# apple/ml-stable-diffusion

Measured on AMD Instinct MI355X. Metric: diffusion iter/s (UNet steps/s), SD2.1-base 512x512 fp16, higher is better.
Workload: dtype fp16; 1 GPU; BASELINE config 2: SD2.1-base (865.9 M-parameter UNet), random-init, denoising iteration at 512x512 (64x64 latents), CFG batch 2 per prompt, DDIM, device-resident loop; unet=sd21-base, latent=64, attention=ORIGINAL, prompts_per_gpu=1, global_batch=2, hip_graph=True, parallelism=dp1 (independent prompts per rank, no data-path collective)

## Files before the change

include/sd_mi355x.h:

```cpp
#ifndef SD_MI355X_H
#define SD_MI355X_H

#include <stddef.h>
#include <stdint.h>

#ifdef __cplusplus
extern "C" {
#endif

typedef enum sd_status {
  SD_OK = 0,
  SD_ERR_INVALID_ARGUMENT = -1,
  SD_ERR_NOT_FOUND = -2,
  SD_ERR_HIP = -3,
  SD_ERR_UNSUPPORTED = -4,
  SD_ERR_INTERNAL = -5
} sd_status;

typedef enum sd_dtype { SD_F16 = 0, SD_F32 = 1 } sd_dtype;

typedef enum sd_attention_impl {
  SD_ATTN_ORIGINAL = 0,
  SD_ATTN_SPLIT_EINSUM = 1,
  SD_ATTN_SPLIT_EINSUM_V2 = 2
// ... 62 lines not shown
int sd_unet_set_attention(sd_unet* u, int impl);
int sd_unet_reload_weights(sd_unet* u, const sd_weights* w, const char* const* names, int n_names);
int sd_unet_num_residuals(const sd_unet* u);
size_t sd_unet_device_bytes(const sd_unet* u);
size_t sd_unet_arena_used_bytes(const sd_unet* u);
int sd_unet_palette_info(const sd_unet* u, int* n_palettized, int* n_streamed, size_t* stream_bytes);
int sd_unet_w8a8_info(const sd_unet* u, int* n_marked, int* n_applied, size_t* bytes);
int sd_unet_w8a8_layer(const sd_unet* u, int index, char* name, int name_bytes);
int sd_unet_activation_ranges(sd_unet* u, int index, char* name, int name_bytes, float* absmax);

#define SD_FLAG_DEVICE_PTRS 1

typedef struct sd_unet_io {
  const void* sample;
  const void* timestep;
  const void* encoder_hidden_states;
  const void* time_ids;
  const void* text_embeds;
  const void* controlnet_cond;
  const void* const* additional_residuals;
  int32_t num_additional_residuals;
  void* noise_pred;
  void* const* residual_outputs;
  int32_t flags;
  const float* step_noise;
} sd_unet_io;

int sd_unet_forward(sd_unet* u, const sd_unet_io* io);

int sd_unet_time_forward(sd_unet* u, int warmup, int iters, float* ms_per_iter);

int sd_unet_profile(sd_unet* u, int iters, int cap, float* ms, double* flop, char* labels, int label_bytes,
                    int* n_ops);

int sd_tune_set_candidate(int tile, int staging, int splitk);
int sd_tune_set_plan_table(const char* rows, sd_unet* u, int* n_plans);

int sd_unet_denoise_loop(sd_unet* u, const sd_unet_io* io, float* latents, int n_images, int n_steps,
                         const float* timesteps, const float* coef, const float* sample_scale, int history,
                         float guidance_scale, float* history_io, float* ms_per_step);

typedef int (*sd_progress_fn)(void* user, int step, int n_steps, const float* latents, const float* denoised);
int sd_unet_denoise_loop_progress(sd_unet* u, const sd_unet_io* io, float* latents, int n_images, int n_steps,
                                  const float* timesteps, const float* coef, const float* sample_scale, int history,
                                  float guidance_scale, float* history_io, float* ms_per_step,
                                  const float* pred , int every,
                                  sd_progress_fn fn, void* user, int* steps_done);

int sd_unet_attach_controlnets(sd_unet* u, sd_unet* const* controlnets, int n);
int sd_controlnet_set_cond(sd_unet* controlnet, const void* controlnet_cond, int flags);

int sd_vae_decoder_create(const sd_unet_config* cfg, const sd_weights* w, int device, sd_unet** out);
int sd_vae_decode(sd_unet* vae, const void* z, sd_dtype z_dtype, float* image, int flags);
int sd_vae_encoder_create(const sd_unet_config* cfg, const sd_weights* w, int device, sd_unet** out);
int sd_vae_encode(sd_unet* vae, const void* x, sd_dtype x_dtype, float* moments, int flags);
int sd_vae_encode_latents(sd_unet* vae_encoder, const void* x, sd_dtype x_dtype, const float* eps, const float* noise, int n_images,
                          float scale_factor, float sa, float sb, float* latents, int flags);
int sd_op_vae_attention(const void* q, const void* k, const void* v, void* out, int B, int S, int C, int iters, float* ms);

typedef struct sd_text_encoder_config {
  int32_t vocab_size, hidden_size, intermediate_size, num_hidden_layers, num_attention_heads;
  int32_t max_position_embeddings;
  int32_t hidden_act;
  int32_t projection_dim;
  float layer_norm_eps;
  int32_t use_graph;
} sd_text_encoder_config;
typedef struct sd_text_encoder sd_text_encoder;
int sd_text_encoder_create(const sd_text_encoder_config* cfg, const sd_weights* w, int device, sd_text_encoder** out);
void sd_text_encoder_destroy(sd_text_encoder* t);
size_t sd_text_encoder_device_bytes(const sd_text_encoder* t);
int sd_text_encoder_encode(sd_text_encoder* t, const int32_t* input_ids, int eos_index, float* last_hidden_state,
                           float* hidden_embeds, float* pooled);

int sd_op_attention(int impl, const void* q, const void* k, const void* v, void* out, int B, int heads, int d,
                    int Sq, int Sk, int variant, int iters, float* ms);
int sd_op_layernorm(const void* x, const float* weight, const float* bias, void* out, int B, int C, int S, float eps,
                    int iters, float* ms);
int sd_op_groupnorm(const void* x, const float* weight, const float* bias, void* out, int B, int C, int H, int W,
                    int groups, float eps, int silu, int iters, float* ms);
int sd_op_groupnorm_shortcut(const void* x0, const void* x1, const float* gn_weight, const float* gn_bias, const void* w, const float* bias,
                             void* out_gn, void* out_sc, int B, int C0, int C1, int H, int W, int N, int groups, float eps, int silu,
                             int side, int iters, float* ms);
int sd_op_conv2d(const void* x, const void* w, const float* bias, const void* res, void* out, int B, int Cin, int H,
                 int W, int Cout, int ksize, int stride, int upsample, int tile, int splitk, int force_generic,
                 int iters, float* ms);
int sd_op_conv2d_ex(const void* x, const void* x1, const void* w, const float* bias, const float* temb, const void* res, void* out, int B,
                    int Cin, int C1, int H, int W, int Cout, int ksize, int stride, int upsample, int pad_mode, int twin_groups,
                    const float* twin_gamma, const float* twin_beta, float twin_eps, int twin_silu, void* out_twin, int tile, int splitk,
                    int force_generic, int* plan_out, int iters, float* ms);
int sd_op_conv2d_palettized(const void* x, const void* x1, const void* lut, int nbits, const uint8_t* indices, const float* bias,
                            const void* res, void* out, int B, int Cin, int C1, int H, int W, int Cout, int ksize, int upsample, int nw,
                            int* plan_out, int iters, float* ms);
int sd_op_palette_pack(const uint8_t* indices, int Cout, int Ctot, int ksize, int nbits, uint8_t* stream, size_t* bytes);
int sd_op_conv2d_w8a8(const void* x, const void* x1, const int8_t* wq, const float* w_scale, float act_absmax, const float* bias,
                      const void* res, void* out, int B, int Cin, int C1, int H, int W, int Cout, int ksize, int upsample, int nw,
                      int* plan_out, int iters, float* ms);
int sd_op_w8a8_pack(const int8_t* wq, int Cout, int Ctot, int ksize, int8_t* stream, size_t* bytes);
int sd_op_conv2d_w8a8_halo(const void* x, const void* x1, const int8_t* wq, const float* w_scale, float act_absmax, const float* bias,
                           const float* temb, const void* res, void* out, int B, int Cin, int C1, int H, int W, int Cout, int upsample,
                           int staging, int splitk, int* plan_out, int iters, float* ms);
int sd_op_w8a8_pack_halo(const int8_t* wq, int Cout, int Ctot, int8_t* packed, size_t* bytes);
int sd_op_subpixel_fold(const void* w, int w_f32, int Cout, int Cin, void* folded, size_t* halves);
int sd_op_subpixel_refusal(int ksize, int stride, int up, int C0, int C1, int N, int B, int Hi, int Wi, int out_mode, char* text, int text_bytes);
int sd_op_conv2d_subpixel(const void* x, const void* w, const float* bias, const void* res, void* out, int B, int Cin, int H, int W, int Cout,
                          int splitk, int staging, int* plan_out, int iters, float* ms);
int sd_op_gemm_w8a8(const void* x, const int8_t* wq, const float* w_scale, float act_absmax, const float* bias, const void* res, void* out, int B,
                    int Cin, int H, int W, int Cout, int bm, int* plan_out, int iters, float* ms);
int sd_op_w8a8_pack_gemm(const int8_t* wq, int Cout, int K, int8_t* packed, size_t* bytes);
int sd_op_layernorm_q8(const void* x, const float* ln_weight, const float* ln_bias, float act_absmax, float eps, int8_t* xq, int M, int C,
                       int iters, float* ms);
int sd_op_geglu_w8a8(const int8_t* xq, const int8_t* wq, const float* w_scale, float act_absmax, const float* bias, void* out, int M, int C,
                     int N2, int bm, int* plan_out, int iters, float* ms);
int sd_op_w8a8_pack_geglu(const int8_t* wq, int N2, int K, int8_t* packed, size_t* bytes);
int sd_op_geglu_w8a8_q8(const int8_t* xq, const int8_t* wq, const float* w_scale, float act_absmax, const float* bias, float out_absmax,
                        int8_t* out_q, int M, int C, int N2, int bm, int* plan_out, int iters, float* ms);
int sd_op_gemm_q8(const int8_t* xq, const int8_t* wq, const float* w_scale, float act_absmax, const float* bias, const void* res, void* out,
                  int M, int K, int N, int bm, int* plan_out, int iters, float* ms);
int sd_op_qkv_w8a8(const int8_t* xq, const int8_t* wq, const float* w_scale, float act_absmax, const float* bias, void* out_qk, void* out_vt,
                   int B, int HW, int C, float q_scale, int vt_perm, int bm, int* plan_out, int iters, float* ms);
int sd_op_w8a8_pack_qkv(const int8_t* wq, int C, int8_t* packed, size_t* bytes);
int sd_op_quantize_weight(const float* w, int Cout, size_t per_row, int8_t* q, float* w_scale, double* sq_err);
int sd_op_absmax(const void* x, size_t n, float* absmax);
int sd_op_gemm_palettized(const void* x, const void* lut, int nbits, const uint8_t* indices, const float* bias, const void* res, void* out,
                          int B, int Cin, int H, int W, int Cout, int bm, int* plan_out, int iters, float* ms);
int sd_op_palette_pack_gemm(const uint8_t* indices, int Cout, int K, int nbits, uint8_t* stream, size_t* bytes);
int sd_op_geglu_palettized(const void* x, const float* ln_weight, const float* ln_bias, const void* lut, int nbits, const uint8_t* indices,
                           const float* bias, void* out, int M, int C, int N2, float eps, int bm, int* plan_out, int iters, float* ms);
int sd_op_palette_pack_geglu(const uint8_t* indices, int N2, int K, int nbits, uint8_t* stream, size_t* bytes);
int sd_op_conv2d_groupnorm(const void* x, const void* w, const float* bias, const void* res, const float* gn_weight,
                           const float* gn_bias, void* conv_out, void* out, int B, int Cin, int H, int W, int Cout, int ksize,
                           int groups, float eps, int silu, int tile, int producer_stats, int* entries, int iters, float* ms);
int sd_op_conv2d_groupnorm_proj(const void* x, const void* w, const float* bias, const void* res, const float* gn_weight,
                                const float* gn_bias, const void* proj_w, const float* proj_bias, void* conv_out, void* out, int B,
                                int Cin, int H, int W, int Cout, int ksize, int Nproj, int groups, float eps, int fold, int tile,
                                int* entries, int iters, float* ms);
int sd_op_conv2d_groupnorm_conv3x3(const void* x, const void* w, const float* bias, const void* res, const float* gn_weight,
                                   const float* gn_bias, const void* w2, const float* bias2, const void* res2, void* conv_out, void* out,
                                   int B, int Cin, int H, int W, int Cout, int ksize, int N2, int groups, float eps, int silu, int fold,
                                   int tile, int staging2, int* entries, int iters, float* ms);
int sd_op_ffn_out_proj(const void* g, const void* w1, const float* b1, const void* res1, const void* w2, const float* b2, const void* res2,
                       void* out, float* gn_sums, int B, int C, int S, int groups, int fused, int iters, float* ms);
int sd_op_fold_linear(const void* wp, const float* bp, const void* w2, const float* b2, void* wm_out, float* bm_out, int N, int J, int K);
int sd_op_cross_attention_fused(const void* x, const float* ln_weight, const float* ln_bias, const void* wq, const void* k,
                                const void* v, void* out, int B, int heads, int Sq, int Sk, float eps, int nst, int iters,
                                float* ms);
int sd_op_cross_attention_block(const void* x, const float* ln_weight, const float* ln_bias, const void* wq, const void* k, const void* v,
                                const void* wo, const float* bo, const void* a1, const void* wo1, const float* bo1, void* out, int B, int heads,
                                int Sq, int Sk, float eps, int fused, int iters, float* ms);
int sd_op_geglu(const void* x, const void* w, const float* bias, void* out, int M, int C, int N2, int iters, float* ms);
int sd_op_geglu_ln(const void* x, const float* ln_weight, const float* ln_bias, const void* w, const float* bias, void* out, int M, int C,
                   int N2, float eps, int kernel, int iters, float* ms);
int sd_op_qkv_ln(const void* x, const float* ln_weight, const float* ln_bias, const void* w, void* out_qk, void* out_vt, int B, int HW, int C,
                 float eps, float q_scale, int vt_perm, int kernel, int iters, float* ms);
int sd_op_gn_proj_qkv(const void* x_in, const void* conv_w, const float* gn_weight, const float* gn_bias, const void* proj_w,
                      const float* proj_bias, const float* ln_weight, const float* ln_bias, const void* wqkv, void* out_h, void* out_qk,
                      void* out_vt, int B, int H, int W, int C, int groups, float gn_eps, float ln_eps, float q_scale, int vt_perm, int fused,
                      int* entries, int iters, float* ms);
int sd_op_timestep_embedding(const float* t, float* out, int n, int dim, int flip_sin_to_cos, float freq_shift);
int sd_op_posterior_noise(const float* moments, const float* eps, const float* noise, float* out, int Cz, int h, int w, int n_images,
                          float scale_factor, float sa, float sb, int iters, float* ms);
int sd_op_sched_step(const float* noise_pred, float* latents, float* hist, const float* coef, const float* pred, const float* step_noise,
                     float guidance, int cfg, int history, int n_images, int n, float* denoised, int* step_after);
int sd_op_conv_plan(int ksize, int stride, int up, int C0, int C1, int N, int B, int Ho, int Wo, int out_mode, int flags, int n_trans,
                    int n_twins, int gnf_groups, int tile, int staging, int splitk, int copies, int* plan, unsigned long long* workspace_bytes);
int sd_op_conv_plan_kernel(int ksize, int stride, int up, int C0, int C1, int N, int B, int Ho, int Wo, int out_mode, int flags, int n_trans,
// ... 58 lines not shown
```

ml-stable-diffusion_amd/csrc/capi_ops.cpp:

```cpp
#include <algorithm>
#include <climits>
#include <cmath>
#include <cstring>
#include <initializer_list>

#include "capi_util.h"
#include "conv_plan.h"
#include "weight_prep.h"

namespace sd {
namespace {

const half_t* f16(const void* p) { return reinterpret_cast<const half_t*>(p); }

half_t* upload_nhwc(Scratch& sc, const void* x, int B, int C, int H, int W) {
  const half_t* src = f16(x);
  std::vector<half_t> t((size_t)B * C * H * W);
  for (int b = 0; b < B; ++b)
    for (int c = 0; c < C; ++c)
      for (int p = 0; p < H * W; ++p) t[((size_t)b * H * W + p) * C + c] = src[((size_t)b * C + c) * H * W + p];
  return sc.dev<half_t>(t.size(), t.data());
}
half_t* upload_tokens(Scratch& sc, const void* x, int B, int C, int S) { return upload_nhwc(sc, x, B, C, 1, S); }

// ... 326 lines not shown
      a.variant = 0;
      a.sk_force = 1;
      a.sk_upw = variant - 100;
    }
    {
      size_t pb = 0;
      int nc = 0;
      if (perm && attention8_sk_scratch(a, &pb, &nc)) {
        a.sk_part = reinterpret_cast<float*>(sc.out<char>(pb, "sk_part"));
        a.sk_part_bytes = pb;
        a.sk_cnt = sc.zeroed<unsigned>(nc, "sk_cnt");
        a.sk_cnt_n = nc;
      } else {
        SD_REQUIRE(variant < 100, kInvalidArgument, "attention variant %d: the balanced form cannot run this shape", variant);
      }
    }
    sc.timed(iters, ms, [&] { launch_attention(a, sc.stream); });
    download_tokens(o, out, B, C, Sq);
  });
}

int sd_op_layernorm(const void* x, const float* weight, const float* bias, void* out, int B, int C, int S, float eps,
                    int iters, float* ms) {
  return guarded([&] {
    SD_REQUIRE(x && weight && bias && out, kInvalidArgument, "NULL argument");
    Scratch sc("layernorm");
    half_t* dx = upload_tokens(sc, x, B, C, S);
    half_t* dy = sc.out<half_t>((size_t)B * S * C, "out");
    float* dw = sc.dev<float>(C, weight);
    float* db = sc.dev<float>(C, bias);
    sc.timed(iters, ms, [&] { launch_layernorm(dx, dw, db, dy, B * S, C, eps, sc.stream); });
    download_tokens(dy, out, B, C, S);
  });
}

int sd_op_groupnorm(const void* x, const float* weight, const float* bias, void* out, int B, int C, int H, int W,
                    int groups, float eps, int silu, int iters, float* ms) {
  return guarded([&] {
    SD_REQUIRE(x && weight && bias && out, kInvalidArgument, "NULL argument");
    Scratch sc("groupnorm");
    half_t* dx = upload_nhwc(sc, x, B, C, H, W);
    half_t* dy = sc.out<half_t>((size_t)B * H * W * C, "out");
    float* dw = sc.dev<float>(C, weight);
    float* db = sc.dev<float>(C, bias);
    float* partial = poisoned_gn_partial(sc, B, H * W, groups);
    sc.timed(iters, ms, [&] {
      launch_groupnorm(dx, C, nullptr, 0, partial, dw, db, dy, B, H * W, groups, eps, silu, sc.stream);
    });
    download_nchw(dy, out, B, C, H, W);
  });
}

int sd_op_groupnorm_shortcut(const void* x0, const void* x1, const float* gn_weight, const float* gn_bias, const void* w, const float* bias,
                             void* out_gn, void* out_sc, int B, int C0, int C1, int H, int W, int N, int groups, float eps, int silu,
                             int side, int iters, float* ms) {
  return guarded([&] {
    SD_REQUIRE(x0 && gn_weight && gn_bias && w && out_gn && out_sc, kInvalidArgument, "NULL argument");
    if (!x1) C1 = 0;
    const int C = C0 + C1;
    Scratch sc("groupnorm_shortcut");
    half_t* d0 = upload_nhwc(sc, x0, B, C0, H, W);
    half_t* d1 = x1 ? upload_nhwc(sc, x1, B, C1, H, W) : nullptr;
    half_t* dy = sc.out<half_t>((size_t)B * H * W * C, "out_gn");
    half_t* ds = sc.out<half_t>((size_t)B * H * W * N, "out_sc");
    float* dgw = sc.dev<float>(C, gn_weight);
    float* dgb = sc.dev<float>(C, gn_bias);
    float* partial = poisoned_gn_partial(sc, B, H * W, groups);
    ConvDesc d = conv_desc(d0, C0, sc.dev<half_t>((size_t)N * C, f16(w)), bias ? sc.dev<float>(N, bias) : nullptr, nullptr, ds, B, H, W, N);
    d.x1 = d1;
    d.C1 = C1;
    SD_REQUIRE(conv_fast_path_ok(d), kInvalidArgument, "groupnorm_shortcut: C0=%d C1=%d N=%d not MFMA-tileable", C0, C1, N);
    SD_REQUIRE(!side || gn_side_gemm_ok(d), kUnsupported, "groupnorm_shortcut: the GEMM cannot ride in the GroupNorm launch (M=%d)", B * H * W);
    ConvWorkspace ws = workspace_for(sc, {d});
    sc.timed(iters, ms, [&] {
      if (side) {
        launch_groupnorm(d0, C0, d1, C1, partial, dgw, dgb, dy, B, H * W, groups, eps, silu, sc.stream, 0, &d);
      } else {
        launch_groupnorm(d0, C0, d1, C1, partial, dgw, dgb, dy, B, H * W, groups, eps, silu, sc.stream);
        launch_conv(d, ws, sc.stream);
      }
    });
    download_nchw(dy, out_gn, B, C, H, W);
    download_nchw(ds, out_sc, B, N, H, W);
  });
}

int sd_op_conv2d(const void* x, const void* w, const float* bias, const void* res, void* out, int B, int Cin, int H,
                 int W, int Cout, int ksize, int stride, int upsample, int tile, int splitk, int force_generic,
                 int iters, float* ms) {
  return guarded([&] { conv2d_op(x, w, bias, res, out, B, Cin, H, W, Cout, ksize, stride, upsample, tile, splitk, force_generic, iters, ms, ConvOpExtra{}); });
}

int sd_op_conv2d_ex(const void* x, const void* x1, const void* w, const float* bias, const float* temb, const void* res, void* out, int B,
                    int Cin, int C1, int H, int W, int Cout, int ksize, int stride, int upsample, int pad_mode, int twin_groups,
                    const float* twin_gamma, const float* twin_beta, float twin_eps, int twin_silu, void* out_twin, int tile, int splitk,
                    int force_generic, int* plan_out, int iters, float* ms) {
  return guarded([&] {
    SD_REQUIRE(plan_out, kInvalidArgument, "NULL argument");
    ConvOpExtra e;
    e.entry = "conv2d_ex";
    e.x1 = x1; e.C1 = C1; e.temb = temb; e.pad_mode = pad_mode;
    e.twin_groups = twin_groups; e.twin_gamma = twin_gamma; e.twin_beta = twin_beta; e.twin_eps = twin_eps; e.twin_silu = twin_silu;
    e.out_twin = out_twin;
    e.plan_out = plan_out;
    conv2d_op(x, w, bias, res, out, B, Cin, H, W, Cout, ksize, stride, upsample, tile, splitk, force_generic, iters, ms, e);
  });
}

int sd_op_conv2d_palettized(const void* x, const void* x1, const void* lut, int nbits, const uint8_t* indices, const float* bias,
                            const void* res, void* out, int B, int Cin, int C1, int H, int W, int Cout, int ksize, int upsample, int nw,
                            int* plan_out, int iters, float* ms) {
  return guarded([&] {
    SD_REQUIRE(lut && indices, kInvalidArgument, "NULL argument");
    SD_REQUIRE(palette_bits_ok(nbits), kInvalidArgument, "conv2d_palettized: nbits = %d, not one of 1, 2, 4, 6, 8", nbits);
    SD_REQUIRE(nw == 0 || nw == 4 || nw == 8, kInvalidArgument, "conv2d_palettized: nw = %d, not 0, 4 or 8", nw);
    SD_REQUIRE(B > 0 && Cin > 0 && C1 >= 0 && Cout > 0 && H > 0 && W > 0, kInvalidArgument, "conv2d_palettized: empty problem");
    ConvOpExtra e;
    e.entry = "conv2d_palettized";
    e.x1 = x1; e.C1 = C1;
    e.plan_out = plan_out;
    e.cw.kind = WeightSource::PalWstream; e.cw.lut = lut; e.cw.indices = indices; e.cw.bits = nbits;
    e.nw = nw;
    conv2d_op(x, nullptr, bias, res, out, B, Cin, H, W, Cout, ksize, 1, upsample, 0, 0, 0, iters, ms, e);
  });
}

int sd_op_conv2d_w8a8(const void* x, const void* x1, const int8_t* wq, const float* w_scale, float act_absmax, const float* bias,
                      const void* res, void* out, int B, int Cin, int C1, int H, int W, int Cout, int ksize, int upsample, int nw,
                      int* plan_out, int iters, float* ms) {
  return guarded([&] {
    SD_REQUIRE(x && wq && w_scale && out, kInvalidArgument, "NULL argument");
    SD_REQUIRE(nw == 0 || nw == 4 || nw == 8, kInvalidArgument, "conv2d_w8a8: nw = %d, not 0, 4 or 8", nw);
    SD_REQUIRE(B > 0 && Cin > 0 && C1 >= 0 && Cout > 0 && H > 0 && W > 0 && (C1 == 0 || x1), kInvalidArgument, "conv2d_w8a8: empty problem");
    SD_REQUIRE((ksize == 1 || ksize == 3) && (upsample == 0 || upsample == 1), kInvalidArgument, "conv2d_w8a8: ksize %d upsample %d", ksize, upsample);
    ConvDesc d;
    d.C0 = Cin;
    if (C1 > 0) d.x1 = f16(x1), d.C1 = C1;
    d.B = B; d.Hi = H; d.Wi = W; d.Ho = H * (upsample ? 2 : 1); d.Wo = W * (upsample ? 2 : 1);
    d.ksize = ksize; d.up = upsample ? 2 : 1; d.N = Cout;
    SD_REQUIRE(conv_fast_path_ok(d) && wstream_shape_ok(d), kInvalidArgument,
               "conv2d_w8a8: shape not eligible for plan tile 17 (wstream.hip: k=%d C0=%d C1=%d N=%d %dx%d)", ksize, Cin, C1, Cout, d.Ho, d.Wo);
    (void)w8a8_host_copy("conv2d_w8a8", wq, w_scale, act_absmax, Cout, Cin + C1, ksize);
    ConvOpExtra e;
    e.entry = "conv2d_w8a8";
    e.x1 = x1; e.C1 = C1;
    e.plan_out = plan_out;
    e.cw.kind = WeightSource::I8Wstream; e.cw.q = wq; e.cw.w_scale = w_scale; e.cw.act_absmax = act_absmax;
    e.nw = nw;
    conv2d_op(x, nullptr, bias, res, out, B, Cin, H, W, Cout, ksize, 1, upsample, 0, 0, 0, iters, ms, e);
  });
}

int sd_op_conv2d_w8a8_halo(const void* x, const void* x1, const int8_t* wq, const float* w_scale, float act_absmax, const float* bias, const float* temb,
                           const void* res, void* out, int B, int Cin, int C1, int H, int W, int Cout, int upsample, int staging, int splitk, int* plan_out,
                           int iters, float* ms) {
  return guarded([&] {
    SD_REQUIRE(x && wq && w_scale && out, kInvalidArgument, "NULL argument");
    SD_REQUIRE(B > 0 && Cin > 0 && C1 >= 0 && Cout > 0 && H > 0 && W > 0 && (C1 == 0 || x1), kInvalidArgument, "conv2d_w8a8_halo: empty problem");
    SD_REQUIRE((upsample == 0 || upsample == 1) && staging >= 0 && staging <= 5 && staging != 1 && splitk >= 0, kInvalidArgument,
               "conv2d_w8a8_halo: upsample %d staging %d (plan tile 7's ring codes 0, 2-5) splitk %d", upsample, staging, splitk);
    ConvDesc d;
    d.C0 = Cin;
    if (C1 > 0) d.x1 = f16(x1), d.C1 = C1;
    d.B = B; d.Hi = H; d.Wi = W; d.Ho = H * (upsample ? 2 : 1); d.Wo = W * (upsample ? 2 : 1);
    d.ksize = 3; d.up = upsample ? 2 : 1; d.N = Cout;
    SD_REQUIRE(conv_fast_path_ok(d) && halo_ks_ok(d), kInvalidArgument,
// ... 1506 lines not shown
```

ml-stable-diffusion_amd/csrc/conv_plan.cpp:

```cpp
#include "conv_plan.h"

#include <algorithm>
#include <cstring>

namespace sd {

namespace {

constexpr int BK = kConvBK;

struct Dims {
  int Ctot, M, N, K, HoWo, nk_total, tiles_x, tiles_y;
};
Dims dims_of(const ConvDesc& d) {
  Dims a;
  a.Ctot = d.C0 + (d.x1 ? d.C1 : 0);
  a.M = d.B * d.Ho * d.Wo;
  a.N = d.N;
  a.K = d.ksize * d.ksize * a.Ctot;
  a.HoWo = d.Ho * d.Wo;
  a.nk_total = a.K / BK;
  a.tiles_x = cdiv(d.Wo, 16);
  a.tiles_y = cdiv(d.Ho, 8);
  return a;
// ... 317 lines not shown
    r.workspace_bytes = slab_bytes(a, r.splitk, r.slab);
    return r;
  }
  if (!conv_fast_path_ok(d)) return ConvPlan{-1, 0, 1, false, 0};
  switch (cw.kind) {
    case WeightSource::Fp16: break;
    case WeightSource::PalWstream:
    case WeightSource::I8Wstream: {
      const bool i8 = i8_stream(d);
      SD_REQUIRE(cw.stream && (i8 ? cw.scale != nullptr : cw.lut != nullptr) && can_split(d) && wstream_shape_ok(d), kInvalidArgument, "%s",
                 i8 ? "plan tile 17 (wstream.hip, int8) needs the int8 stream, the scales and a shape of the weight stream"
                    : "plan tile 14 (wstream.hip, palettized) needs the index stream, the LUT and a shape of the weight stream");
      ConvPlan r{i8 ? 17 : 14, d.staging, 1, true, 0};
      r.splitk = wstream_splits(d, wstream_waves(d.staging));
      r.workspace_bytes = slab_bytes(dims_of(d), r.splitk, true);
      return r;
    }
    case WeightSource::I8Halo: {
      const Dims a = dims_of(d);
      const Plan p = choose_plan(d, a);
      ConvPlan r{18, p.staging, 1, true, 0};
      const int steps = a.Ctot / BK;
      r.splitk = cdiv(steps, cdiv(steps, p.splitk));
      r.slab = r.splitk > 1 || d.n_twins > 0;
      r.workspace_bytes = slab_bytes(a, r.splitk, r.slab);
      return r;
    }
    case WeightSource::PalGemm:
      SD_REQUIRE(cw.stream && cw.lut && palette_bits_ok(cw.bits) && !d.x1 && d.staging >= 0 && d.staging <= 2 && smgemm_shape_ok(d, d.staging), kInvalidArgument,
                 "plan tile 15 (smgemm.hip, palettized) needs the index stream, the LUT and a single-source shape of the small-M GEMM");
      return ConvPlan{15, smgemm_bm(d, d.staging) == 32 ? 1 : 2, 1, false, 0};
    case WeightSource::I8Gemm:
      return ConvPlan{19, smgemm_bm(d, d.staging) == 32 ? 1 : 2, 1, false, 0};
    case WeightSource::PalGeglu:
      SD_REQUIRE(cw.stream && cw.lut && palette_bits_ok(cw.bits) && (cw.ln_gamma != nullptr) == (d.ln_colsum != nullptr) && smgeglu_pal_shape_ok(d, d.staging),
                 kInvalidArgument,
                 "plan tile 16 (smgeglu.hip, palettized) needs the index stream, the LUT, the norm weight with the LayerNorm fold and a shape of "
                 "the GEGLU kernel with 128-row tiles");
      return ConvPlan{16, 1, 1, false, 0};
    case WeightSource::I8Geglu:
      return ConvPlan{20, smgeglu_bm(d, d.staging) == 128 ? 1 : 2, 1, false, 0};
    case WeightSource::I8Qkv:
      return ConvPlan{22, smqkv_i8_bm(d, d.staging) == 128 ? 1 : 2, 1, false, 0};
    case WeightSource::I8GemmQ:
      return ConvPlan{24, smgemm_bm(d, d.staging) == 32 ? 1 : 2, 1, false, 0};
  }
  const Switches& sw = switches();
  const bool free_choice = d.tile == 0 && d.splitk == 0 && d.staging == 0 && g_tune.tile == 0;
  if (d.w_ws && wsgemm_shape_ok(d) && (d.tile == 10 || (sw.wsgemm && free_choice && wsgemm_wanted(d)))) return ConvPlan{10, 0, 1, false, 0};
  SD_REQUIRE(d.tile != 10, kInvalidArgument, "plan tile 10 (wsgemm.hip) needs the pre-tiled weights and an eligible GEGLU shape");
  if (sw.bvgemm && d.w_bv && free_choice && bvgemm_wanted(d)) return ConvPlan{11, 0, 1, false, 0};
  if (d.tile == 11) {
    SD_REQUIRE(d.w_bv && bvgemm_shape_ok(d), kInvalidArgument, "plan tile 11 (bvgemm.hip) needs the pre-tiled weights and an eligible 1x1 shape");
    return ConvPlan{11, d.staging, 1, false, 0};
  }
  if (d.tile == 12 || (sw.smgemm && free_choice && smgemm_wanted(d))) return ConvPlan{12, d.tile == 12 ? d.staging : 0, 1, false, 0};
  if (d.tile == 13 || (sw.smgeglu && free_choice && smgeglu_wanted(d))) return ConvPlan{13, d.tile == 13 ? d.staging : 0, 1, false, 0};

  const Dims a = dims_of(d);
  Plan p = choose_plan(d, a);
  const bool twins = d.n_twins > 0;
  if (d.gnf_partial && d.ksize == 3) {
    SD_REQUIRE(conv_gn_loader_ok(d) && d.gnf_silu == 1 && d.gnf_gamma && d.gnf_beta && d.gnf_entries >= 1 && d.gnf_entries <= 128 && !twins, kInvalidArgument,
               "GroupNorm in the conv loader: Ctot=%d groups=%d entries=%d up=%d", a.Ctot, d.gnf_groups, d.gnf_entries, d.up);
    p.tile = 7;
    if (p.staging != 2 && p.staging != 3) p.staging = 3;
    p.splitk = 1;
  } else if (d.gnf_partial) {
    SD_REQUIRE(d.ksize == 1 && d.stride == 1 && !d.x1 && d.out_mode == kOutHalf && !d.ln_colsum && !d.out_t && !twins &&
                   gemm_pipe_ok(d.ksize, d.stride, d.up, a.M, a.N, a.K, d.C0, 0) &&
                   d.gnf_gamma && d.gnf_beta && d.gnf_groups >= 1 && d.gnf_groups <= 32 && a.K % d.gnf_groups == 0 && a.K <= 2048 &&
                   d.gnf_entries >= 1 && d.gnf_entries <= 128 && a.HoWo % 64 == 0,
               kInvalidArgument, "GroupNorm fold: K=%d groups=%d entries=%d HoWo=%d", a.K, d.gnf_groups, d.gnf_entries, a.HoWo);
    p.tile = 3;
    if (p.staging != 6 && p.staging != 7 && p.staging != 8) p.staging = 6;
    p.splitk = 1;
  }
  ConvPlan r{p.tile, p.staging, 1, true, 0};
  if (p.tile == 9) {
    r.splitk = wstream_splits(d, wstream_waves(p.staging));
  } else {
    const int steps = p.tile == 7 ? a.Ctot / BK : a.nk_total;
    r.splitk = cdiv(steps, cdiv(steps, p.splitk));
    r.slab = r.splitk > 1 || twins;
  }
  r.workspace_bytes = slab_bytes(a, r.splitk, r.slab);
  return r;
}

void decode_plan(const ConvDesc& d, ConvPlan& p) {
  const Dims a = dims_of(d);
  int code = p.staging;
  switch (p.tile) {
    case -1: p.kernel = ConvKernel::Generic; return;
    case 9: case 14: case 17:
      p.kernel = p.tile == 9 ? ConvKernel::Wstream : p.tile == 14 ? ConvKernel::WstreamPal : ConvKernel::WstreamI8;
      p.waves = wstream_waves(code);
      return;
    case 10: p.kernel = ConvKernel::Wsgemm; return;
    case 11:
      p.kernel = ConvKernel::Bvgemm;
      p.variant = code >= 1 && code <= 6 ? code : bvgemm_auto_variant(d);
      return;
    case 12: case 15: case 19: case 24:
      p.kernel = p.tile == 12 ? ConvKernel::Smgemm : p.tile == 15 ? ConvKernel::SmgemmPal : p.tile == 19 ? ConvKernel::SmgemmI8 : ConvKernel::SmgemmQ8;
      p.bm = code >= 0 && code <= 2 ? smgemm_bm(d, code) : 0;
      return;
    case 13: case 16: case 20:
      p.kernel = p.tile == 13 ? ConvKernel::Smgeglu : p.tile == 16 ? ConvKernel::SmgegluPal : ConvKernel::SmgegluI8;
      p.bm = code >= 0 && code <= 2 ? smgeglu_bm(d, code) : 0;
      return;
    case 22:
      p.kernel = ConvKernel::SmqkvI8;
      p.bm = code >= 0 && code <= 2 ? smqkv_i8_bm(d, code) : 0;
      return;
    default: break;
  }
  if (p.tile == 18) {
    tile_dims(7, p.bm, p.bn);
    p.kernel = ConvKernel::HaloI8;
    p.stages = code >= 3 ? 4 : code == 2 ? 3 : 2;
    return;
  }
  if (p.tile == 21) {
    tile_dims(7, p.bm, p.bn);
    p.kernel = ConvKernel::HaloSubpix;
    p.stages = code == 2 ? 3 : 4;
    return;
  }
  tile_dims(p.tile, p.bm, p.bn);
  if (p.tile == 7) {
    p.kernel = ConvKernel::HaloKs;
    if (d.gnf_partial) p.stages = code >= 3 && halo_gnl_lds_bytes(4, a.Ctot) <= kLdsBudget ? 4 : 3;
    else p.stages = code >= 5 ? 8 : code == 4 ? 6 : code == 3 ? 4 : code == 2 ? 3 : 2;
    return;
  }
  p.kernel = ConvKernel::Igemm;
  p.stages = 2;
  const bool lnf = d.ln_colsum != nullptr;
  auto fits = [&](int nst, int kgroups = 1) { return ring_fits(p.bm, p.bn, nst, kgroups); };
  if (lnf && code == 1) code = 0;
  if (code == 1) {
    p.reg_staged = true;
    return;
  }
  if (!lnf && d.out_mode == kOutHalfT) {
    if (code >= 2) p.stages = 3;
    return;
  }
  if (code == 12 || code == 13) {
    const bool two_groups = !lnf && cdiv(a.nk_total, p.splitk) >= 4;
    if (two_groups && code == 13 && fits(4, 2)) p.stages = 4, p.kgroups = 2;
    else if (two_groups && fits(3, 2)) p.stages = 3, p.kgroups = 2;
    if (p.kgroups == 2) return;
    code -= 10;
  }
  if (code >= 6 && code <= 8 && gemm_pipe_ok(d.ksize, d.stride, d.up, a.M, a.N, a.K, d.C0, d.x1 ? d.C1 : 0)) {
    p.kernel = ConvKernel::GemmPipe;
    p.stages = code == 8 ? 2 : (code == 7 && fits(4)) ? 4 : 3;
    return;
  }
  if (code >= 6) code = 3;
  const int asked = code >= 5 ? 8 : code == 4 ? 6 : code == 3 ? 4 : code == 2 ? 3 : 2;
  for (int nst : {8, 6, 4, 3, 2})
    if (nst <= asked && fits(nst)) {
      p.stages = nst;
      return;
    }
}

}

ConvPlan conv_plan(const ConvDesc& d) {
  ConvPlan p = plan_codes(d);
  decode_plan(d, p);
  return p;
}

std::string conv_plan_kernel_name(const ConvPlan& p) {
  const std::string tile = std::to_string(p.bm) + "x" + std::to_string(p.bn), ring = " ring" + std::to_string(p.stages);
  switch (p.kernel) {
    case ConvKernel::Igemm: return "igemm " + tile + ring + (p.kgroups == 2 ? " kg2" : "") + (p.reg_staged ? " regs" : "");
    case ConvKernel::GemmPipe: return "gemm_pipe " + tile + ring;
    case ConvKernel::HaloKs: return "halo_ks" + ring;
    case ConvKernel::HaloI8: return "halo_i8" + ring;
    case ConvKernel::HaloSubpix: return "conv3x3_halo_sp" + ring;
    case ConvKernel::Wstream: return "wstream waves" + std::to_string(p.waves);
    case ConvKernel::WstreamPal: return "wstream_pal waves" + std::to_string(p.waves);
    case ConvKernel::WstreamI8: return "wstream_i8 waves" + std::to_string(p.waves);
    case ConvKernel::Wsgemm: return "wsgemm";
    case ConvKernel::Bvgemm: return "bvgemm v" + std::to_string(p.variant);
    case ConvKernel::Smgemm: return "smgemm bm" + std::to_string(p.bm);
    case ConvKernel::SmgemmPal: return "smgemm_pal bm" + std::to_string(p.bm);
    case ConvKernel::SmgemmI8: return "smgemm_i8 bm" + std::to_string(p.bm);
    case ConvKernel::SmgemmQ8: return "smgemm_q8 bm" + std::to_string(p.bm);
    case ConvKernel::Smgeglu: return "smgeglu bm" + std::to_string(p.bm);
    case ConvKernel::SmgegluPal: return "smgeglu_pal bm" + std::to_string(p.bm);
    case ConvKernel::SmgegluI8: return "smgeglu_i8 bm" + std::to_string(p.bm);
    case ConvKernel::SmqkvI8: return "smqkv_i8 bm" + std::to_string(p.bm);
    default: return "generic";
  }
}

size_t conv_workspace_bytes(const ConvDesc& d) {
  if (!conv_fast_path_ok(d) || pal_gemm(d) || pal_geglu(d) || i8_gemm(d) || i8_geglu(d) || i8_qkv(d) || i8_gemm_q(d)) return 0;
  const Dims a = dims_of(d);
  if (d.subpix) return halo_sp_ok(d) ? slab_bytes(a, subpix_splits(d, a), false) : 0;
  const Plan p = choose_plan(d, a);
  int splits = (switches().tuning && can_split(d)) ? std::max(p.splitk, 16) : p.splitk;
  const bool stream = can_stream(d) || ((pal_stream(d) || i8_stream(d)) && can_split(d) && wstream_shape_ok(d));
  if (stream) splits = std::max(splits, wstream_splits(d, 4));
  return slab_bytes(a, splits, d.n_twins > 0 || stream);
}

ConvWeightCopies conv_plan_copies(const ConvDesc& d0) {
  ConvWeightCopies c{false, false, false};
  if (!conv_fast_path_ok(d0) || d0.subpix) return c;
  ConvDesc d = d0;
  d.w_tiled = d.w_ws = d.w_bv = nullptr;
  const Switches& sw = switches();
  const int k = d.ksize, M = d.B * d.Ho * d.Wo;
  const bool ws_candidate = sw.tuning ? ((k == 3 && M <= 512) || (k == 1 && M <= 128)) : plan_is_wstream(d);
  c.wstream = sw.wstream && wstream_shape_ok(d) && ws_candidate;
  c.wsgemm = sw.wsgemm && wsgemm_wanted(d);
  c.bvgemm = sw.bvgemm && !c.wsgemm && bvgemm_wanted(d);
  return c;
}

namespace {
ConvPlan fp16_plan(const ConvDesc& d0, const ConvWeightCopies& c) {
  static const half_t present = 0;
  ConvDesc d = d0;
  d.cw = CompressedWeights{};
  d.w_tiled = c.wstream ? &present : nullptr;
  d.w_ws = c.wsgemm ? &present : nullptr;
  d.w_bv = c.bvgemm ? &present : nullptr;
  return conv_plan(d);
}
}

WeightPin conv_plan_pin(WeightSource kind, int n) {
  switch (kind) {
    case WeightSource::PalWstream: return {kind, 14, n == 4 ? 4 : 0};
    case WeightSource::I8Wstream: return {kind, 17, n == 4 ? 4 : 0};
    case WeightSource::I8Halo: return {kind, 18, n};
    case WeightSource::PalGemm: return {kind, 15, n == 32 ? 1 : n == 64 ? 2 : 0};
    case WeightSource::I8Gemm: return {kind, 19, n == 32 ? 1 : n == 64 ? 2 : 0};
    case WeightSource::PalGeglu: return {kind, 16, n == 128 ? 1 : n == 256 ? 2 : 0};
    case WeightSource::I8Geglu: return {kind, 20, n == 128 ? 1 : n == 256 ? 2 : 0};
    case WeightSource::I8Qkv: return {kind, 22, n == 128 ? 1 : n == 256 ? 2 : 0};
    case WeightSource::I8GemmQ: return {kind, 24, n == 32 ? 1 : n == 64 ? 2 : 0};
    default: return {};
  }
}

WeightPin conv_plan_weights(const ConvDesc& d, StoredWeights held, bool opt_in) {
  if (held == StoredWeights::Fp16 || !conv_fast_path_ok(d)) return {};
  const Switches& sw = switches();
  const bool palette = held == StoredWeights::Palette, one_by_one = opt_in && palette && d.ksize == 1 && !d.x1;
  if (one_by_one && d.out_mode == kOutGeglu && sw.smgeglu) {
    const ConvPlan p = fp16_plan(d, conv_plan_copies(d));
    if (p.kernel == ConvKernel::Smgeglu && smgeglu_pal_shape_ok(d, 0)) return conv_plan_pin(WeightSource::PalGeglu, p.bm);
  }
  if (opt_in && held == StoredWeights::W8A8 && d.ksize == 1 && !d.x1 && d.out_mode == kOutGeglu && sw.smgeglu) {
    const ConvPlan p = fp16_plan(d, conv_plan_copies(d));
    ConvDesc plain = d;
    plain.ln_colsum = nullptr;
    if (p.kernel == ConvKernel::Smgeglu && smgeglu_i8_shape_ok(plain, p.bm == 128 ? 1 : 2)) return conv_plan_pin(WeightSource::I8Geglu, p.bm);
  }
  if (opt_in && held == StoredWeights::W8A8 && d.ksize == 1 && !d.x1 && d.out_mode == kOutHalf && d.n_trans == 0 && d.x0_i8) {
    if (sw.smgemm && !d.ln_colsum && smgemm_q8_wanted(d)) return conv_plan_pin(WeightSource::I8GemmQ, smgemm_bm(d, 0));
    return {};
  }
  if (opt_in && held == StoredWeights::W8A8 && d.ksize == 1 && !d.x1 && d.out_mode == kOutHalf && d.n_trans > 0 && sw.qkv_i8) {
    ConvDesc plain = d;
    plain.ln_colsum = nullptr;
    if (smqkv_i8_shape_ok(plain, 0)) return conv_plan_pin(WeightSource::I8Qkv, smqkv_i8_bm(plain, 0));
    return {};
  }
  if (sw.wstream && !d.ln_colsum && plan_is_wstream(d)) {
    const ConvPlan p = fp16_plan(d, {true, false, false});
    if (p.kernel == ConvKernel::Wstream) return conv_plan_pin(palette ? WeightSource::PalWstream : WeightSource::I8Wstream, p.waves);
  }
  if (one_by_one && d.out_mode == kOutHalf && sw.smgemm && !d.ln_colsum) {
    const ConvPlan p = fp16_plan(d, conv_plan_copies(d));
    if (p.kernel == ConvKernel::Smgemm) return conv_plan_pin(WeightSource::PalGemm, p.bm);
  }
  if (opt_in && held == StoredWeights::W8A8 && d.ksize == 1 && !d.x1 && d.out_mode == kOutHalf && sw.smgemm && !d.ln_colsum) {
    const ConvPlan p = fp16_plan(d, conv_plan_copies(d));
    if (p.kernel == ConvKernel::Smgemm && smgemm_i8_shape_ok(d, 0)) return conv_plan_pin(WeightSource::I8Gemm, p.bm);
  }
  if (held == StoredWeights::W8A8 && halo_i8_ok(d)) {
    const ConvPlan p = fp16_plan(d, conv_plan_copies(d));
    if (p.kernel == ConvKernel::HaloKs) {
      WeightPin pin = conv_plan_pin(WeightSource::I8Halo, p.staging);
// ... 79 lines not shown
```

ml-stable-diffusion_amd/csrc/conv_plan.h:

```cpp
#pragma once
#include <string>

#include "kernels.h"

namespace sd {

enum class ConvKernel { Generic, Igemm, GemmPipe, HaloKs, HaloI8, HaloSubpix, Wstream, WstreamPal, WstreamI8, Wsgemm, Bvgemm, Smgemm, SmgemmPal, SmgemmI8, Smgeglu, SmgegluPal, SmgegluI8, SmqkvI8, SmgemmQ8 };

struct ConvPlan {
  int tile;
  int staging;
  int splitk;
  bool slab;
  size_t workspace_bytes;
  ConvKernel kernel = ConvKernel::Generic;
  int bm = 0, bn = 0;
  int stages = 0;
  int kgroups = 1;
  bool reg_staged = false;
  int waves = 0;
  int variant = 0;
};
ConvPlan conv_plan(const ConvDesc& d);

struct ConvWeightCopies {
  bool wstream, wsgemm, bvgemm;
};
ConvWeightCopies conv_plan_copies(const ConvDesc& d);

enum class StoredWeights { Fp16, Palette, W8A8 };
struct WeightPin {
  WeightSource kind = WeightSource::Fp16;
  int tile = 0, staging = 0;
  int splitk = 0;
};
WeightPin conv_plan_weights(const ConvDesc& d, StoredWeights held, bool opt_in);
WeightPin conv_plan_pin(WeightSource kind, int n);

void conv_plan_log(const ConvDesc& d, const ConvPlan& p, int n_fast = 0);

std::string conv_plan_kernel_name(const ConvPlan& p);

bool choose_tile_order(double a_bytes, double w_bytes, double nbm, double nbn, bool ab_switch);

bool conv_reduce_stats_on();

constexpr int kConvBK = 64;
bool halo_ks_ok(const ConvDesc& d);
const char* halo_sp_refusal(const ConvDesc& d);
inline bool halo_sp_ok(const ConvDesc& d) { return halo_sp_refusal(d) == nullptr; }
bool subpixel_wanted(const ConvDesc& d);
bool gemm_pipe_ok(int ksize, int stride, int up, int M, int N, int K, int C0, int C1);

constexpr size_t kLdsBudget = 160 * 1024;
constexpr size_t ring_bytes(int bm, int bn, int nst) { return (size_t)nst * (bm + bn) * kConvBK * sizeof(half_t); }
constexpr bool ring_fits(int bm, int bn, int nst, int kgroups = 1) { return kgroups * ring_bytes(bm, bn, nst) + 2 * bn * sizeof(float) <= kLdsBudget; }
constexpr int kHaloLdsRows = 184;
constexpr size_t halo_lds_bytes(int bn, int d) {
  return ((size_t)2 * kHaloLdsRows * kConvBK + (size_t)d * bn * kConvBK) * sizeof(half_t) + bn * sizeof(float);
}
constexpr size_t halo_gnl_lds_bytes(int d, int ctot) {
  const size_t k_loop = halo_lds_bytes(64, d) - 64 * sizeof(float) + (((size_t)6 * ctot + 15) & ~(size_t)15);
  const size_t epilogue = 32 * 1024 + 128 * (64 + 8) * 2 + 64 * sizeof(float);
  return k_loop > epilogue ? k_loop : epilogue;
}
constexpr int kHaloI8Pitch = 20, kHaloI8Rows = 204;
constexpr size_t halo_i8_lds_bytes(int d) {
  return (size_t)kHaloLdsRows * kConvBK * sizeof(half_t) + (size_t)2 * kHaloI8Rows * kConvBK + (size_t)d * 64 * kConvBK + 2 * 64 * sizeof(float);
}
constexpr int kHaloI8MaxCtot = 14784;
static_assert(127LL * 127 * 9 * kHaloI8MaxCtot < (1LL << 31) && 127LL * 127 * 9 * (kHaloI8MaxCtot + 64) >= (1LL << 31), "int32 bound of plan tile 18");
constexpr int kSmI8MaxK = 133120;
static_assert(127LL * 127 * kSmI8MaxK < (1LL << 31) && 127LL * 127 * (kSmI8MaxK + 64) >= (1LL << 31), "int32 bound of plan tile 19");

bool smgemm_q8_wanted(const ConvDesc& d);
constexpr int kSmQkvCols = 160;
bool smqkv_i8_shape_ok(const ConvDesc& d, int variant);
bool smqkv_i8_tiles(const ConvDesc& d, int variant);
int smqkv_i8_bm(const ConvDesc& d, int variant);

}
```

ml-stable-diffusion_amd/csrc/igemm.hip:

```cpp
#include "igemm_device.h"

namespace sd {

namespace {

template <int BM, int BN, int WGM, int WGN, bool TRANS_OUT, bool GLDS, int NST, int DBG = 0, bool LNF = false, int KG = 1>
__global__ __launch_bounds__(256 * KG) void igemm_kernel(IgemmArgs a) {
  static_assert(WGM * WGN == 4, "4 waves");
  static_assert(KG == 1 || (KG == 2 && GLDS && NST >= 3 && !LNF && !TRANS_OUT && DBG == 0), "in-workgroup split-K: ring variants of the plain epilogue");
  static_assert(!(LNF && TRANS_OUT), "LayerNorm fold uses the in-lane row layout of the non-transposed tile");
  constexpr int TM = BM / WGM / 32;
  constexpr int TN = BN / WGN / 32;
  constexpr int XR = BM / 32;
  constexpr int WR = BN / 32;
  constexpr int ROW = GLDS ? BK : LDS_ROW;

  const bool prof = (DBG & 4) && blockIdx.x == 0 && blockIdx.y == 0 && threadIdx.x == 0;
  long long prof_t[4];
  long long prof_w0 = 0;
  if (prof) { prof_t[0] = clock64(); prof_w0 = wall_clock64(); }
  extern __shared__ __attribute__((aligned(16))) char smem[];
  const int kg = KG > 1 ? __builtin_amdgcn_readfirstlane((int)threadIdx.x >> 8) : 0;
  half_t* Xs = reinterpret_cast<half_t*>(smem) + (size_t)kg * NST * (BM + BN) * ROW;
  half_t* Ws = Xs + NST * BM * ROW;
// ... 618 lines not shown
  int rd_stage = 0;
  auto body = [&](Frags& cur, Frags& nxt, auto last) {
    constexpr bool LAST = decltype(last)::value;
    if constexpr (LAST) {
      asm volatile("s_waitcnt lgkmcnt(0)" ::: "memory");
      mfma_step(cur);
    } else {
      asm volatile("s_waitcnt lgkmcnt(0)" ::: "memory");
      wait_vmcnt_barrier<(D - 2) * PER>();
      const int nstage = (rd_stage + 1 == D) ? 0 : rd_stage + 1;
      read_step(nxt, nstage);
      issue_tile();
      mfma_step(cur);
      rd_stage = nstage;
      if constexpr (!LNF && !GNF) {
        constexpr int NM = KK * TM * TN, NR = KK * (TM + TN);
        constexpr int RPM = (NR + NM / 2 - 1) / (NM / 2);
#pragma unroll
        for (int g = 0; g < NM / 2; ++g) {
          __builtin_amdgcn_sched_group_barrier(0x008, 1, 0);
          __builtin_amdgcn_sched_group_barrier(0x100, RPM, 0);
        }
#pragma unroll
        for (int g = 0; g < NM - NM / 2; ++g) {
          __builtin_amdgcn_sched_group_barrier(0x008, 1, 0);
          __builtin_amdgcn_sched_group_barrier(0x010, (PER + NM - NM / 2 - 1) / (NM - NM / 2), 0);
        }
      }
    }
    __builtin_amdgcn_sched_barrier(0);
  };
  {
    using Tt = std::true_type;
    using Ff = std::false_type;
    int st = 0;
    for (; st + 2 < T; st += 2) {
      body(fA, fB, Ff{});
      body(fB, fA, Ff{});
    }
    if (T - st == 2) {
      body(fA, fB, Ff{});
      body(fB, fA, Tt{});
    } else {
      body(fA, fB, Tt{});
    }
  }
  asm volatile("s_waitcnt vmcnt(0) lgkmcnt(0)" ::: "memory");

  float ln_a[TM] = {}, ln_b[TM] = {};
  if constexpr (LNF) {
    const float inv_k = 1.0f / (float)a.K;
#pragma unroll
    for (int i = 0; i < TM; ++i) {
      const float s1 = xor32_sum(ln_s1[i]), s2 = xor32_sum(ln_s2[i]);
      const float mean = s1 * inv_k;
      const float var = fmaxf(s2 * inv_k - mean * mean, 0.f);
      ln_a[i] = rsqrtf(var + a.ln_eps);
      ln_b[i] = -ln_a[i] * mean;
    }
  }
  tile_epilogue<BM, BN, WGM, WGN, TM, TN, LNF, (RES_PRE ? RIT : 0)>(a, acc, ln_a, ln_b, smem, sconst, const_b, const_t, const_c, m_blk,
                                                                    n_blk, wave, split, temb_uniform, resv, use_resv);
}

template <int BM, int BN, int WGM, int WGN, int D, bool LNF, int DBG = 0, bool GNF = false>
__global__ __launch_bounds__(256, D == 2 ? 2 : 1) void gemm_pipe_kernel(IgemmArgs a) {
  gemm_pipe_body<BM, BN, WGM, WGN, D, LNF, DBG, GNF>(a, blockIdx.x, blockIdx.y);
}

struct GnSideArgs {
  const half_t* x0;
  const half_t* x1;
  int C0, C1;
  const float* partial;
  int slabs;
  const float* gamma;
  const float* beta;
  half_t* y;
  int HW, G;
  float eps;
  int silu, pix_per_block;
  int gx, gy;
  int n_gn_pad;
};

template <int D>
__global__ __launch_bounds__(256) void gn_apply_side_kernel(GnSideArgs g, IgemmArgs a) {
  const int v = blockIdx.x;
  if (v < g.gx * g.gy) {
    groupnorm_apply_body(g.x0, g.C0, g.x1, g.C1, g.partial, g.slabs, g.gamma, g.beta, g.y, g.HW, g.G, g.eps, g.silu, g.pix_per_block,
                         v % g.gx, v / g.gx);
  } else if (v >= g.n_gn_pad) {
    gemm_pipe_body<64, 64, 2, 2, D, false>(a, v - g.n_gn_pad, 0);
  }
}

template <int VW, int D>
__global__ __launch_bounds__(256) void gn_fused_side_kernel(GnSideArgs g, IgemmArgs a) {
  const int v = blockIdx.x;
  if (v < g.gx * g.gy) {
    groupnorm_fused_body<VW, 256>(g.x0, g.C0, g.x1, g.C1, g.gamma, g.beta, g.y, g.HW, g.G, g.eps, g.silu, v % g.gx, v / g.gx);
  } else if (v >= g.n_gn_pad) {
    gemm_pipe_body<64, 64, 2, 2, D, false>(a, v - g.n_gn_pad, 0);
  }
}

__global__ __launch_bounds__(256) void splitk_reduce_kernel(IgemmArgs a) {
  constexpr int SB = 8;
  const size_t total4 = (size_t)a.M * a.N / 4;
  const size_t slab = (size_t)a.M * a.N;
  const floatx4 z4 = {0.f, 0.f, 0.f, 0.f};
  for (size_t idx = (size_t)blockIdx.x * blockDim.x + threadIdx.x; idx < total4;
       idx += (size_t)gridDim.x * blockDim.x) {
    const size_t e0 = idx * 4;
    const int m = (int)(e0 / a.N);
    const int n = (int)(e0 - (size_t)m * a.N);
    floatx4 p[SB];
#pragma unroll
    for (int z = 0; z < SB; ++z) p[z] = (z < a.splitk) ? *reinterpret_cast<const floatx4*>(a.partial + (size_t)z * slab + e0) : z4;
    const floatx4 bv = a.bias ? *reinterpret_cast<const floatx4*>(a.bias + n) : z4;
    const floatx4 tv = a.temb ? *reinterpret_cast<const floatx4*>(a.temb + (size_t)(m / a.HoWo) * a.temb_stride + n) : z4;
    const half4 hz = {0, 0, 0, 0};
    const half4 rr = a.res ? *reinterpret_cast<const half4*>(a.res + e0) : hz;
    floatx4 s = z4;
#pragma unroll
    for (int z = 0; z < SB; ++z)
      if (z < a.splitk) s += p[z];
    for (int z = SB; z < a.splitk; ++z) s += *reinterpret_cast<const floatx4*>(a.partial + (size_t)z * slab + e0);
    if (a.bias) s += bv;
    if (a.temb) s += tv;
    if (a.res) {
      s[0] += (float)rr[0];
      s[1] += (float)rr[1];
      s[2] += (float)rr[2];
      s[3] += (float)rr[3];
    }
    half4 o = {(half_t)s[0], (half_t)s[1], (half_t)s[2], (half_t)s[3]};
    out_store(reinterpret_cast<half4*>(a.out + e0), o);
  }
}

__global__ __launch_bounds__(256) void splitk_reduce_stats_kernel(IgemmArgs a, int ppb) {
  extern __shared__ __attribute__((aligned(16))) char smem[];
  float* qs = reinterpret_cast<float*>(smem);
  const int NQ = a.N >> 2, t = threadIdx.x, b = blockIdx.y;
  const int p0 = blockIdx.x * ppb;
  const int items = ppb * NQ;
  for (int id = t; id < items; id += 256) {
    const int pl = id / NQ, qd = id - pl * NQ;
    const int p = p0 + pl;
    float fs = 0.f, fq = 0.f;
    if (p < a.HoWo) {
      const int m = b * a.HoWo + p, n = 4 * qd;
      const size_t e0 = (size_t)m * a.N + n;
      floatx4 s = {0.f, 0.f, 0.f, 0.f};
      for (int z = 0; z < a.splitk; ++z) s += *reinterpret_cast<const floatx4*>(a.partial + (size_t)z * a.M * a.N + e0);
      if (a.bias) s += *reinterpret_cast<const floatx4*>(a.bias + n);
      if (a.temb) s += *reinterpret_cast<const floatx4*>(a.temb + (size_t)b * a.temb_stride + n);
      if (a.res) {
        const half4 rr = *reinterpret_cast<const half4*>(a.res + e0);
        s[0] += (float)rr[0];
        s[1] += (float)rr[1];
        s[2] += (float)rr[2];
        s[3] += (float)rr[3];
      }
      const half4 o = {(half_t)s[0], (half_t)s[1], (half_t)s[2], (half_t)s[3]};
      out_store(reinterpret_cast<half4*>(a.out + e0), o);
      const float f0 = (float)o[0], f1 = (float)o[1], f2 = (float)o[2], f3 = (float)o[3];
      fs = (f0 + f1) + (f2 + f3);
      fq = fmaf(f0, f0, fmaf(f1, f1, fmaf(f2, f2, f3 * f3)));
    }
    qs[2 * id] = fs;
    qs[2 * id + 1] = fq;
  }
  __syncthreads();
  if (t < a.gn_G) {
    const int q0 = t * (a.gn_cpg >> 2), q1 = q0 + (a.gn_cpg >> 2);
    float s = 0.f, q = 0.f;
    for (int pl = 0; pl < ppb; ++pl)
      for (int qd = q0; qd < q1; ++qd) {
        s += qs[2 * (pl * NQ + qd)];
        q += qs[2 * (pl * NQ + qd) + 1];
      }
    float* dst = a.gn_partial + (((size_t)b * a.gn_G + t) * kGnMaxSlabs + blockIdx.x) * 2;
    dst[0] = s;
    dst[1] = q;
  }
}


template <int BM, int BN, int WGM, int WGN, bool TRANS, bool GLDS, int NST, bool LNF = false, int KG = 1>
void launch_variant(const IgemmArgs& a, hipStream_t s) {
  const size_t lds = (size_t)KG * NST * (BM + BN) * (GLDS ? BK : LDS_ROW) * sizeof(half_t) + 2 * BN * sizeof(float);
  static_assert(ring_fits(BM, BN, NST, KG), "LDS");
  static_assert((size_t)BN * (BM + 8) <= (size_t)NST * (BM + BN) * (GLDS ? BK : LDS_ROW), "transposed staging fits");
  static_assert((size_t)BM * (BN + 8) * 2 + 16 + (kGnScratchFloats + 2 * BN) * sizeof(float) <=
                    (size_t)NST * (BM + BN) * (GLDS ? BK : LDS_ROW) * sizeof(half_t),
                "GroupNorm statistics scratch fits behind the staged tile");
  dim3 grid(cdiv(a.M, BM) * cdiv(a.N, BN), a.splitk);
  auto k = igemm_kernel<BM, BN, WGM, WGN, TRANS, GLDS, NST, 0, LNF, KG>;
  static DynLdsOnce once;
  once.set(k, lds);
  hipLaunchKernelGGL(k, grid, dim3(256 * KG), lds, s, a);
}

template <int BM, int BN, int DBG>
void launch_debug(const IgemmArgs& a, hipStream_t s) {
  const size_t lds = (size_t)2 * (BM + BN) * BK * sizeof(half_t) + 2 * BN * sizeof(float);
  dim3 grid(cdiv(a.M, BM) * cdiv(a.N, BN), a.splitk);
  auto k = igemm_kernel<BM, BN, 2, 2, false, true, 2, DBG>;
  SD_HIP(hipFuncSetAttribute((const void*)k, hipFuncAttributeMaxDynamicSharedMemorySize, (int)lds));
  hipLaunchKernelGGL(k, grid, dim3(256), lds, s, a);
}
template <int BM, int BN>
bool launch_debug_mode(const IgemmArgs& a, int dbg, hipStream_t s) {
  switch (dbg) {
    case 4: launch_debug<BM, BN, 4>(a, s); return true;
    case 5: launch_debug<BM, BN, 5>(a, s); return true;
    case 6: launch_debug<BM, BN, 6>(a, s); return true;
    case 14: launch_debug<BM, BN, 14>(a, s); return true;
    case 22: launch_debug<BM, BN, 22>(a, s); return true;
    case 30: launch_debug<BM, BN, 30>(a, s); return true;
    default: return false;
  }
}

template <int BM, int BN, int WGM, int WGN, int D, bool LNF>
void launch_pipe_dbg(const IgemmArgs& a, hipStream_t s) {
  constexpr size_t lds = (size_t)D * (BM + BN) * BK * sizeof(half_t) + 2 * BN * sizeof(float);
  dim3 grid(cdiv(a.M, BM) * cdiv(a.N, BN), a.splitk);
  if (a.debug == 65) {
    auto k = gemm_pipe_kernel<BM, BN, WGM, WGN, D, LNF, 1>;
    SD_HIP(hipFuncSetAttribute((const void*)k, hipFuncAttributeMaxDynamicSharedMemorySize, (int)lds));
    hipLaunchKernelGGL(k, grid, dim3(256), lds, s, a);
  } else {
    auto k = gemm_pipe_kernel<BM, BN, WGM, WGN, D, LNF, 2>;
    SD_HIP(hipFuncSetAttribute((const void*)k, hipFuncAttributeMaxDynamicSharedMemorySize, (int)lds));
    hipLaunchKernelGGL(k, grid, dim3(256), lds, s, a);
  }
// ... 37 lines not shown
      if constexpr (!LNF && (NST == 3 || NST == 4) && ring_fits(BM, BN, NST, 2)) { launch_variant<BM, BN, 2, 2, false, true, NST, false, 2>(a, s); return true; }
    } else {
      launch_variant<BM, BN, 2, 2, false, true, NST, LNF>(a, s);
      return true;
    }
  }
  return false;
}
template <int BM, int BN, bool LNF>
bool launch_ring(const IgemmArgs& a, const ConvPlan& p, hipStream_t s) {
  switch (p.stages) {
    case 2: return launch_ring_depth<BM, BN, LNF, 2>(a, p, s);
    case 3: return launch_ring_depth<BM, BN, LNF, 3>(a, p, s);
    case 4: return launch_ring_depth<BM, BN, LNF, 4>(a, p, s);
    case 6: return launch_ring_depth<BM, BN, LNF, 6>(a, p, s);
    case 8: return launch_ring_depth<BM, BN, LNF, 8>(a, p, s);
    default: return false;
  }
}

template <int BM, int BN>
void launch_tile(const IgemmArgs& a, const ConvPlan& p, bool trans, hipStream_t s) {
  bool ok = true;
  if (a.ln_colsum) ok = !p.reg_staged && launch_ring<BM, BN, true>(a, p, s);
  else if (trans && p.reg_staged) launch_variant<BM, BN, 2, 2, true, false, 2>(a, s);
  else if (trans && p.stages == 3) launch_variant<BM, BN, 2, 2, true, true, 3>(a, s);
  else if (trans) launch_variant<BM, BN, 2, 2, true, true, 2>(a, s);
  else if (p.reg_staged) launch_variant<BM, BN, 2, 2, false, false, 2>(a, s);
  else ok = launch_ring<BM, BN, false>(a, p, s);
  SD_REQUIRE(ok, kInternal, "no %dx%d kernel for plan '%s'", BM, BN, conv_plan_kernel_name(p).c_str());
}

int launch_slab_combine(const ConvDesc& d, IgemmArgs& a, hipStream_t s) {
  a.gn_partial = nullptr;
  if (conv_reduce_stats_on() && d.gn_partial && d.gn_groups >= 1 && d.gn_groups <= 256 && a.N % d.gn_groups == 0 && (a.N / d.gn_groups) % 4 == 0 &&
      a.HoWo <= 256 && d.out_mode == kOutHalf && !d.out_t) {
    int ppb = std::max(1, a.B * a.HoWo / 512);
    const int slabs = cdiv(a.HoWo, ppb);
    const size_t lds = (size_t)ppb * (a.N / 4) * 2 * sizeof(float);
    if (slabs <= kGnMaxSlabs && lds <= 64 * 1024) {
      a.gn_partial = d.gn_partial;
      a.gn_G = d.gn_groups;
      a.gn_cpg = a.N / d.gn_groups;
      a.gn_T = slabs;
      hipLaunchKernelGGL(splitk_reduce_stats_kernel, dim3(slabs, a.B), dim3(256), lds, s, a, ppb);
      return slabs;
    }
  }
  const size_t total4 = (size_t)a.M * a.N / 4;
  const int blocks = (int)std::min<size_t>((total4 + 255) / 256, 2048);
  hipLaunchKernelGGL(splitk_reduce_kernel, dim3(blocks), dim3(256), 0, s, a);
  return 0;
}

half_t* g_zero_chunk = nullptr;

}

const half_t* device_zero_chunk() {
  if (!g_zero_chunk) {
    SD_HIP(hipMalloc(reinterpret_cast<void**>(&g_zero_chunk), 256));
    SD_HIP(hipMemset(g_zero_chunk, 0, 256));
    SD_HIP(hipDeviceSynchronize());
  }
  return g_zero_chunk;
}

const half_t* zero_chunk() {
  SD_REQUIRE(g_zero_chunk, kInternal, "conv launch before any handle allocated the zero chunk (device_zero_chunk)");
  return g_zero_chunk;
}

int launch_conv(const ConvDesc& d, const ConvWorkspace& ws, hipStream_t s) {
  SD_REQUIRE(conv_fast_path_ok(d), kInvalidArgument, "launch_conv: shape not MFMA-tileable (C0=%d C1=%d N=%d k=%d)",
             d.C0, d.C1, d.N, d.ksize);
  SD_REQUIRE(!d.ln_colsum || (d.ksize == 1 && !d.x1 && d.bias && d.out_mode != kOutHalfT), kInvalidArgument,
             "LayerNorm fold needs a 1x1 single-source GEMM with a (folded) bias");
  SD_REQUIRE(!d.out_t || (d.out_mode == kOutHalf && d.n_trans % 64 == 0 && d.n_trans < d.N && (d.Ho * d.Wo) % 8 == 0 &&
                          d.ldT % 8 == 0 && !d.res && !d.temb),
             kInvalidArgument, "fused q|k|v: n_trans %d N %d HoWo %d ldT %d", d.n_trans, d.N, d.Ho * d.Wo, d.ldT);
  SD_REQUIRE(!d.vt_perm || (d.out_t && (d.Ho * d.Wo) % 16 == 0), kInvalidArgument, "permuted V^T needs the fused q|k|v epilogue and HoWo %% 16 == 0");
  SD_REQUIRE(d.q_cols == 0 || (d.out_t && d.q_cols % 4 == 0 && d.q_cols <= d.n_trans), kInvalidArgument, "pre-scaled queries need the fused q|k|v epilogue (q_cols %d)", d.q_cols);
  const ConvPlan p = conv_plan(d);
  switch (p.kernel) {
    case ConvKernel::Wsgemm: launch_wsgemm(d, s); return 0;
    case ConvKernel::Bvgemm: launch_bvgemm(d, p, s); return 0;
    case ConvKernel::Smgemm: launch_smgemm(d, p, s); return 0;
    case ConvKernel::Smgeglu: launch_smgeglu(d, p, s); return 0;
    case ConvKernel::SmgegluPal: launch_smgeglu_pal(d, p, s); return 0;
    case ConvKernel::SmgemmPal: launch_smgemm_pal(d, p, s); return 0;
    case ConvKernel::SmgemmI8: launch_smgemm_i8(d, p, s); return 0;
    case ConvKernel::SmgegluI8: launch_smgeglu_i8(d, p, s); return 0;
    case ConvKernel::SmgemmQ8: launch_smgemm_q8(d, p, s); return 0;
    case ConvKernel::SmqkvI8: launch_smqkv_i8(d, p, s); return 0;
    default: break;
  }
  IgemmArgs a = planned_args(d, p, ws.partial);
  const bool twins = d.n_twins > 0;
  SD_REQUIRE(!twins || (d.out_mode == kOutHalf && !d.ln_colsum && !d.out_t && !d.debug && reduce_twin_ok(a.HoWo, a.N, d.n_twins, d.twin)),
             kInvalidArgument, "GroupNorm twins need a plain fp16 output and whole (sample, group) slices (HoWo=%d N=%d)", a.HoWo, a.N);
  const bool have_ws = !p.slab || (ws.partial && ws.partial_bytes >= p.workspace_bytes);
  if (p.kernel == ConvKernel::Wstream || p.kernel == ConvKernel::WstreamPal || p.kernel == ConvKernel::WstreamI8) SD_REQUIRE(have_ws, kInternal, "wstream workspace too small (%zu < %zu)", ws.partial_bytes, p.workspace_bytes);
  SD_REQUIRE(have_ws, kInternal, "split-K workspace too small (%zu < %zu)", ws.partial_bytes, p.workspace_bytes);
  conv_plan_log(d, p);
  int gn_entries = 0;
  switch (p.kernel) {
    case ConvKernel::Wstream:
      launch_wstream(d, ws.partial, p.waves, s);
      break;
    case ConvKernel::WstreamPal:
      launch_wstream_pal(d, ws.partial, p.waves, s);
      break;
    case ConvKernel::WstreamI8:
      launch_wstream_i8(d, ws.partial, p.waves, s);
      break;
    case ConvKernel::HaloKs: gn_entries = launch_halo_ks(d, p, ws.partial, s); break;
    case ConvKernel::HaloI8: gn_entries = launch_halo_i8(d, p, ws.partial, s); break;
    case ConvKernel::HaloSubpix: gn_entries = launch_halo_sp(d, p, ws.partial, s); break;
    case ConvKernel::Igemm:
    case ConvKernel::GemmPipe: {
      const bool trans = d.out_mode == kOutHalfT;
      set_tile_order(a, p.bm, p.bn);
      if (d.debug && d.debug < 64) {
        const bool ok = p.bm == 128 && p.bn == 128 ? launch_debug_mode<128, 128>(a, d.debug, s) : launch_debug_mode<64, 64>(a, d.debug, s);
        SD_REQUIRE(ok && !trans, kInvalidArgument, "no ablation kernel for debug mode %d", d.debug);
        return 0;
      }
      if (!trans) gn_entries = setup_gn_stats(d, a, p.bm);
      if (p.bm == 128 && p.bn == 128) launch_tile<128, 128>(a, p, trans, s);
      else if (p.bm == 128) launch_tile<128, 64>(a, p, trans, s);
      else if (p.bn == 64) launch_tile<64, 64>(a, p, trans, s);
      else launch_tile<64, 128>(a, p, trans, s);
      break;
    }
    default: SD_REQUIRE(false, kInternal, "launch_conv: plan '%s' has no launcher here", conv_plan_kernel_name(p).c_str());
  }
  if (twins) {
    launch_reduce_twin(a.partial, a.splitk, a.M, a.N, a.HoWo, a.bias, a.temb, a.temb_stride, a.res, a.out, d.n_twins, d.twin, s);
  } else if (a.slab) {
    gn_entries = launch_slab_combine(d, a, s);
  }
  SD_HIP(hipGetLastError());
  return gn_entries;
}

bool gn_side_gemm_ok(const ConvDesc& d) {
  if (!(d.ksize == 1 && d.stride == 1 && d.up == 1 && d.out_mode == kOutHalf && !d.ln_colsum && !d.out_t && d.n_twins == 0 && !d.gnf_partial &&
        !d.gn_partial && !d.temb && !d.debug && conv_fast_path_ok(d)))
    return false;
  const int M = d.B * d.Ho * d.Wo, c1 = d.x1 ? d.C1 : 0;
  return gemm_pipe_ok(d.ksize, d.stride, d.up, M, d.N, d.C0 + c1, d.C0, c1) && M >= 256;
}

namespace {
constexpr int kSideD = 4;
IgemmArgs side_args(const ConvDesc& d) {
  SD_REQUIRE(gn_side_gemm_ok(d), kInvalidArgument, "side GEMM: not a plain 1x1 GEMM of the pipelined kernel (C0=%d C1=%d N=%d)", d.C0, d.C1, d.N);
  IgemmArgs a = make_args(d);
  a.splitk = 1;
  a.slab = 0;
  set_tile_order(a, 64, 64);
  return a;
}
constexpr size_t kSideLds = (size_t)kSideD * (64 + 64) * BK * sizeof(half_t) + 2 * 64 * sizeof(float);
}

void launch_gn_apply_side(const half_t* x0, int C0, const half_t* x1, int C1, const float* partial, int entries, const float* gamma,
                          const float* beta, half_t* y, int B, int HW, int G, float eps, int silu, int slabs, int ppb, const ConvDesc& side,
                          hipStream_t s) {
  IgemmArgs a = side_args(side);
  GnSideArgs g{x0, x1, C0, x1 ? C1 : 0, partial, entries, gamma, beta, y, HW, G, eps, silu, ppb, slabs, B, 0};
  g.n_gn_pad = (slabs * B + 7) / 8 * 8;
  auto k = gn_apply_side_kernel<kSideD>;
  static DynLdsOnce once;
  once.set(k, kSideLds);
  hipLaunchKernelGGL(k, dim3(g.n_gn_pad + cdiv(a.M, 64) * cdiv(a.N, 64)), dim3(256), kSideLds, s, g, a);
  SD_HIP(hipGetLastError());
}

void launch_gn_fused_side(int vw, const half_t* x0, int C0, const half_t* x1, int C1, const float* gamma, const float* beta, half_t* y, int B,
                          int HW, int G, float eps, int silu, const ConvDesc& side, hipStream_t s) {
  IgemmArgs a = side_args(side);
  GnSideArgs g{x0, x1, C0, x1 ? C1 : 0, nullptr, 0, gamma, beta, y, HW, G, eps, silu, 0, G, B, 0};
  g.n_gn_pad = (G * B + 7) / 8 * 8;
  const dim3 grid(g.n_gn_pad + cdiv(a.M, 64) * cdiv(a.N, 64));
  static DynLdsOnce o8, o4, o2;
  if (vw == 8) {
    auto k = gn_fused_side_kernel<8, kSideD>;
    o8.set(k, kSideLds);
    hipLaunchKernelGGL(k, grid, dim3(256), kSideLds, s, g, a);
  } else if (vw == 4) {
    auto k = gn_fused_side_kernel<4, kSideD>;
    o4.set(k, kSideLds);
    hipLaunchKernelGGL(k, grid, dim3(256), kSideLds, s, g, a);
  } else {
    auto k = gn_fused_side_kernel<2, kSideD>;
    o2.set(k, kSideLds);
    hipLaunchKernelGGL(k, grid, dim3(256), kSideLds, s, g, a);
  }
  SD_HIP(hipGetLastError());
}

}
```

ml-stable-diffusion_amd/csrc/igemm_device.h:

```cpp
#pragma once
#include <cstdio>
#include <cstdlib>
#include <cstring>
#include <string>
#include <type_traits>

#include "conv_plan.h"

namespace sd {

const half_t* zero_chunk();

int launch_halo_ks(const ConvDesc& d, const ConvPlan& p, float* partial, hipStream_t s);
int launch_halo_i8(const ConvDesc& d, const ConvPlan& p, float* partial, hipStream_t s);
int launch_halo_sp(const ConvDesc& d, const ConvPlan& p, float* partial, hipStream_t s);

namespace {

constexpr int BK = kConvBK;
constexpr int LDS_ROW = BK + 8;

struct IgemmArgs {
  const half_t* x0;
  const half_t* x1;
  const half_t* w;
  const float* bias;
  const float* temb;
  const half_t* res;
  half_t* out;
  float* partial;
  int C0, C1, Ctot;
  int B, Hi, Wi, Ho, Wo, HoWo;
  int ksize, stride, up, pad;
  int M, N, K;
  int temb_stride;
  int nk_total, nk_per_split, splitk;
  int slab;
  int out_mode, ldT;
  int debug;
  long long* prof;
  const half_t* zeros;
  int tiles_x, tiles_y;
  const float* ln_colsum;
  float ln_eps;
  int n_trans, ldo;
  half_t* out_t;
  int vt_perm;
  int res_pre;
  float* gn_partial;
  int gn_G, gn_cpg, gn_T;
  int n_fast;
  const float* gnf_partial;
  const float* gnf_gamma;
  const float* gnf_beta;
  float gnf_eps;
  int gnf_G, gnf_entries;
  float q_scale;
  int q_cols;
};

constexpr int kGnScratchFloats = 256 * 17;

template <int BN>
__device__ __forceinline__ void tile_gn_stats(const IgemmArgs& a, float* scratch, const float (&fs)[8], const float (&fq)[8],
                                              int n_blk, int b, int mt) {
  constexpr int OWC = BN / 8;
  const int tid = threadIdx.x;
  float* chan = scratch + kGnScratchFloats;
#pragma unroll
  for (int e = 0; e < 8; ++e) {
    scratch[tid * 17 + e] = fs[e];
    scratch[tid * 17 + 8 + e] = fq[e];
  }
  __syncthreads();
  for (int cc = tid; cc < 2 * BN; cc += 256) {
    const int which = cc / BN, ch = cc - which * BN;
    const int cl = ch >> 3, e = ch & 7;
    float s = 0.f;
#pragma unroll 4
    for (int k = 0; k < 256 / OWC; ++k) s += scratch[(k * OWC + cl) * 17 + which * 8 + e];
    chan[cc] = s;
  }
  __syncthreads();
  const int g0 = n_blk / a.gn_cpg;
  const int g = g0 + tid;
  const int n_end = min(n_blk + BN, a.N);
  if (tid < BN && g < a.gn_G && g * a.gn_cpg < n_end) {
    const int gs = g * a.gn_cpg, ge = gs + a.gn_cpg;
    const int lo = max(gs, n_blk), hi = min(ge, n_end);
    float s = 0.f, q = 0.f;
    for (int c = lo; c < hi; ++c) {
      s += chan[c - n_blk];
      q += chan[BN + c - n_blk];
    }
    float* dst = a.gn_partial + (((size_t)b * a.gn_G + g) * kGnMaxSlabs + (size_t)mt * 2) * 2;
    if (gs < n_blk) {
      dst[2] = s;
      dst[3] = q;
    } else {
      dst[0] = s;
      dst[1] = q;
      if (ge <= n_end) {
        dst[2] = 0.f;
        dst[3] = 0.f;
      }
    }
  }
}

__device__ __forceinline__ float gelu_erf(float x) {
  const float z = x * 0.70710678118654752f;
  const float az = fabsf(z);
  const float t = __builtin_amdgcn_rcpf(fmaf(0.3275911f, az, 1.0f));
  float p = 1.061405429f;
  p = fmaf(p, t, -1.453152027f);
  p = fmaf(p, t, 1.421413741f);
  p = fmaf(p, t, -0.284496736f);
  p = fmaf(p, t, 0.254829592f);
  const float e = __builtin_amdgcn_exp2f(-az * az * 1.4426950408889634f);
  const float erf_abs = fmaf(-p * t, e, 1.0f);
  return 0.5f * x * (1.0f + copysignf(erf_abs, z));
}

__device__ __forceinline__ float xor32_sum(float v) {
  const unsigned u = __float_as_uint(v);
  const auto r = __builtin_amdgcn_permlane32_swap(u, u, false, false);
  const unsigned r0 = r[0], r1 = r[1];
  return __uint_as_float(r0) + __uint_as_float(r1);
}

__device__ __forceinline__ float wave_sum(float v) {
#pragma unroll
  for (int o = 32; o > 0; o >>= 1) v += __shfl_xor(v, o);
  return v;
}
#include "gn_body.inc"

__device__ __forceinline__ void dma16_to_lds(const __amdgpu_buffer_rsrc_t& rs, char* lds, unsigned voffset, int soffset) {
#if defined(__HIP_DEVICE_COMPILE__)
  __builtin_amdgcn_raw_ptr_buffer_load_lds(rs, (__attribute__((address_space(3))) void*)lds, 16, voffset, soffset, 0, 0);
#endif
// ... 309 lines not shown
```

ml-stable-diffusion_amd/csrc/kernels.h:

```cpp
#pragma once
#include "sd_common.h"

namespace sd {

enum OutMode : int {
  kOutHalf = 0,
  kOutHalfT = 1,
  kOutGeglu = 2,
};

struct GnTwin {
  half_t* y = nullptr;
  int ld = 0, c_off = 0;
  int cpg = 0;
  const float* gamma = nullptr;
  const float* beta = nullptr;
  float eps = 1e-5f;
  int silu = 0;
};

enum class WeightSource { Fp16, PalWstream, PalGemm, PalGeglu, I8Wstream, I8Halo, I8Gemm, I8Geglu, I8Qkv, I8GemmQ };
struct CompressedWeights {
  WeightSource kind = WeightSource::Fp16;
  const void* stream = nullptr;
  const half_t* lut = nullptr;
  int bits = 0;
  const float* ln_gamma = nullptr;
  const float* scale = nullptr;
  float inv_s = 0.f;
  bool palettized() const { return kind == WeightSource::PalWstream || kind == WeightSource::PalGemm || kind == WeightSource::PalGeglu; }
  const uint8_t* pal() const { return palettized() ? static_cast<const uint8_t*>(stream) : nullptr; }
  bool int8() const { return kind == WeightSource::I8Wstream || kind == WeightSource::I8Halo || kind == WeightSource::I8Gemm || kind == WeightSource::I8Geglu || kind == WeightSource::I8Qkv || kind == WeightSource::I8GemmQ; }
  const int8_t* i8() const { return int8() ? static_cast<const int8_t*>(stream) : nullptr; }
};

struct ConvDesc {
  const half_t* x0 = nullptr;
  const half_t* x1 = nullptr;
  const int8_t* x0_i8 = nullptr;
  int C0 = 0, C1 = 0;
  const half_t* w = nullptr;
  const float* bias = nullptr;
  const float* temb = nullptr;
  int temb_stride = 0;
  const half_t* res = nullptr;
  half_t* out = nullptr;
  int8_t* out_q8 = nullptr;
  float out_inv_s = 0.f;
  int B = 1, Hi = 1, Wi = 1;
  int Ho = 1, Wo = 1;
  int ksize = 1, stride = 1, up = 1;
  int pad = -1;
  int N = 0;
  int out_mode = kOutHalf;
  int ldT = 0;
  int tile = 0;
  int splitk = 0;
  long long* prof = nullptr;
  int debug = 0;
  int staging = 0;
  const float* ln_colsum = nullptr;
  float ln_eps = 1e-5f;
  half_t* out_t = nullptr;
  int n_trans = 0;
  int vt_perm = 0;
  float q_scale = 1.f;
  int q_cols = 0;
  float* gn_partial = nullptr;
  int gn_groups = 0;
  const float* gnf_partial = nullptr;
  const float* gnf_gamma = nullptr;
  const float* gnf_beta = nullptr;
  float gnf_eps = 1e-6f;
  int gnf_groups = 0, gnf_entries = 0;
  int gnf_silu = 0;
  const half_t* w_tiled = nullptr;
  CompressedWeights cw;
  const half_t* w_ws = nullptr;
  const half_t* w_bv = nullptr;
  GnTwin twin[2];
  int n_twins = 0;
  bool subpix = false;
};

constexpr int kGnMaxSlabs = 256;

struct ConvWorkspace {
  float* partial = nullptr;
  size_t partial_bytes = 0;
};

size_t conv_workspace_bytes(const ConvDesc& d);
const half_t* device_zero_chunk();
int launch_conv(const ConvDesc& d, const ConvWorkspace& ws, hipStream_t s);
struct ConvPlan;
bool conv_fast_path_ok(const ConvDesc& d);
bool conv_gn_loader_ok(const ConvDesc& d);
void conv_tune_set_candidate(int tile, int staging, int splitk);
bool conv_plan_is_tuned(const ConvDesc& d);
int conv_plan_table_set(const char* text);

bool wstream_shape_ok(const ConvDesc& d);
int wstream_splits(const ConvDesc& d, int nw);
size_t wstream_tiled_halves(int N, int Ctot, int ksize);
void launch_wstream_retile(const half_t* w, half_t* wt, int N, int Ctot, int ksize, hipStream_t s);
int launch_wstream(const ConvDesc& d, float* partial, int nw, hipStream_t s);
int launch_wstream_pal(const ConvDesc& d, float* partial, int nw, hipStream_t s);
int launch_wstream_i8(const ConvDesc& d, float* partial, int nw, hipStream_t s);
bool reduce_twin_ok(int HW, int N, int n_twins, const GnTwin* tw);
void launch_reduce_twin(const float* partial, int S, int M, int N, int HW, const float* bias, const float* temb, int temb_stride,
                        const half_t* res, half_t* out, int n_twins, const GnTwin* tw, hipStream_t s);

bool wsgemm_shape_ok(const ConvDesc& d);
bool wsgemm_wanted(const ConvDesc& d);
size_t wsgemm_tiled_halves(int N);
void launch_wsgemm_retile(const half_t* w, half_t* wt, int N, bool geglu, hipStream_t s);
void launch_wsgemm(const ConvDesc& d, hipStream_t s);

bool bvgemm_shape_ok(const ConvDesc& d);
size_t bvgemm_tiled_halves(int N, int K);
void launch_bvgemm_retile(const half_t* w, half_t* wt, int N, int K, bool geglu, hipStream_t s);
void launch_bvgemm(const ConvDesc& d, const ConvPlan& p, hipStream_t s);
int bvgemm_auto_variant(const ConvDesc& d);
bool bvgemm_wanted(const ConvDesc& d);

bool smgemm_shape_ok(const ConvDesc& d, int variant);
bool smgemm_wanted(const ConvDesc& d);
void launch_smgemm(const ConvDesc& d, const ConvPlan& p, hipStream_t s);
int smgemm_bm(const ConvDesc& d, int variant);
void launch_smgemm_pal(const ConvDesc& d, const ConvPlan& p, hipStream_t s);
bool smgemm_i8_shape_ok(const ConvDesc& d, int variant);
void launch_smgemm_i8(const ConvDesc& d, const ConvPlan& p, hipStream_t s);
bool smgemm_q8_shape_ok(const ConvDesc& d, int variant);
void launch_smgemm_q8(const ConvDesc& d, const ConvPlan& p, hipStream_t s);

void launch_wfold(const half_t* wp, const float* bp, const half_t* w2, const float* b2, half_t* merged, float* bm, int N, int J, int K,
                  hipStream_t s);

bool smgeglu_shape_ok(const ConvDesc& d, int variant);
bool smgeglu_wanted(const ConvDesc& d);
int smgeglu_bm(const ConvDesc& d, int variant);
void launch_smgeglu(const ConvDesc& d, const ConvPlan& p, hipStream_t s);
size_t smgeglu_prof_entries(const ConvDesc& d, int variant);
bool smgeglu_pal_shape_ok(const ConvDesc& d, int variant);
void launch_smgeglu_pal(const ConvDesc& d, const ConvPlan& p, hipStream_t s);
bool smgeglu_i8_shape_ok(const ConvDesc& d, int variant);
void launch_smgeglu_i8(const ConvDesc& d, const ConvPlan& p, hipStream_t s);
void launch_smqkv_i8(const ConvDesc& d, const ConvPlan& p, hipStream_t s);

void run_calibration(int device, float* out);

int launch_conv_generic(const ConvDesc& d, int act_silu_out, hipStream_t s);

void launch_conv_small_n(const ConvDesc& d, float* out_nchw_f32, hipStream_t s);

enum AttnImpl : int { kAttnOriginal = 0, kAttnSplitEinsum = 1, kAttnSplitEinsumV2 = 2 };

struct AttnDesc {
  const half_t* q = nullptr;
  const half_t* k = nullptr;
  const half_t* vt = nullptr;
  half_t* out = nullptr;
  int B = 1, heads = 1, d = 64, Sq = 0, Sk = 0;
  int ldq = 0, ldk = 0, ldv = 0, ldo = 0;
  int impl = kAttnOriginal;
// ... 202 lines not shown
```

ml-stable-diffusion_amd/csrc/net.cpp:

```cpp
#include "net.h"

#include <algorithm>
#include <type_traits>

#include "conv_plan.h"
#include "weight_prep.h"

namespace sd {

Net::Net(const sd_unet_config& cfg, const WeightStore& ws, int device)
    : cfg_(cfg), ws_(&ws), f32_(cfg.compute_fp32 != 0), pal_tensors_((int)ws.palettes()), i8_marked_((int)ws.w8a8_marks()),
      observing_(ws.observe() != 0) {
  SD_REQUIRE(cfg.n_levels >= 1 && cfg.n_levels <= SD_MAX_LEVELS, kInvalidArgument, "n_levels=%d", cfg.n_levels);
  SD_REQUIRE(cfg.batch >= 1 && cfg.height >= 1 && cfg.width >= 1, kInvalidArgument, "bad batch/size");
  SD_REQUIRE(cfg.norm_num_groups >= 1 && cfg.norm_num_groups <= 64, kUnsupported, "norm_num_groups=%d",
             cfg.norm_num_groups);
  open(device);
}

void Net::seal() {
  ll_.seal();
  ws_ = nullptr;
}

// ... 40 lines not shown
  refill({name + ".weight"}, d, [=](const WeightStore& ws) {
    const HostTensor& t = ws.get(name + ".weight");
    SD_REQUIRE(t.numel() == expect, kInvalidArgument, "%s.weight has %zu elements, expected %zu (%d,%d,%d,%d)", name.c_str(), t.numel(), expect,
               cout, cin, k, k);
    std::vector<float> host(expect);
    retile_ohwi(t.data.data(), cout, cin, k, false, host.data());
    SD_HIP(hipMemcpy(d, host.data(), expect * sizeof(float), hipMemcpyHostToDevice));
  });
  return d;
}

float* Net::upload_vec(const std::string& name, int n, bool geglu) {
  SD_REQUIRE((int)ws_->get(name).numel() == n, kInvalidArgument, "%s has %zu elements, expected %d", name.c_str(), ws_->get(name).numel(), n);
  float* d = ll_.arena.alloc_n<float>(n);
  refill({name}, d, [=](const WeightStore& ws) {
    const HostTensor& t = ws.get(name);
    SD_REQUIRE((int)t.numel() == n, kInvalidArgument, "%s has %zu elements, expected %d", name.c_str(), t.numel(), n);
    std::vector<float> host(t.data);
    if (geglu)
      for (int o = 0; o < n; ++o) host[geglu_row(o, n)] = t.data[o];
    SD_HIP(hipMemcpy(d, host.data(), (size_t)n * sizeof(float), hipMemcpyHostToDevice));
  });
  return d;
}

void Net::refill(const std::vector<std::string>& sources, const void* made, Fill fill) {
  for (const std::string& s : sources) source_shape_[s] = ws_->get(s).shape;
  fill(*ws_);
  if (made) made_from_[made] = sources;
  refills_.push_back({sources, std::move(fill)});
}

void Net::derive(const void* from, std::function<void()> launch) {
  auto it = made_from_.find(from);
  SD_REQUIRE(it != made_from_.end(), kInternal, "a derived weight copy of a matrix no refill record made");
  launch();
  refills_.push_back({it->second, [launch](const WeightStore&) { launch(); }});
}

void Net::reload_weights(const WeightStore& ws, const std::vector<std::string>& names) {
  SD_REQUIRE(!observing_, kUnsupported, "reload_weights: the handle was built from an observing store (its observers' ranges belong to the weights it was built with)");
  const std::set<std::string> wanted(names.begin(), names.end());
  for (const std::string& n : wanted) {
    const HostTensor* t = ws.find(n);
    if (!t) fail(kNotFound, "reload_weights: the store has no tensor '%s'", n.c_str());
    SD_REQUIRE(!compressed_.count(n), kUnsupported, "reload_weights: the handle holds '%s' compressed on the device (a palette stream or int8); only fp16 / fp32 tensors reload",
               n.c_str());
  }
  std::vector<const Refill*> run;
  for (const Refill& r : refills_)
    if (std::any_of(r.sources.begin(), r.sources.end(), [&](const std::string& s) { return wanted.count(s) != 0; })) run.push_back(&r);
  for (const Refill* r : run)
    for (const std::string& s : r->sources) {
      const HostTensor* t = ws.find(s);
      if (!t) fail(kNotFound, "reload_weights: the store has no tensor '%s' (read together with a named one)", s.c_str());
      SD_REQUIRE(t->shape == source_shape_.at(s), kInvalidArgument, "reload_weights: '%s' has another shape than the tensor the handle was built with", s.c_str());
    }
  if (run.empty()) return;
  SD_HIP(hipSetDevice(ll_.device));
  SD_HIP(hipStreamSynchronize(ll_.stream));
  for (const Refill* r : run) r->fill(ws);
  after_reload();
  SD_HIP(hipStreamSynchronize(ll_.stream));
}

namespace {
struct ConvGeom {
  int Ho, Wo, pad;
};
ConvGeom conv_geom(const std::string& name, const Tensor& x, const ConvArgs& a) {
  const int Hup = x.H * a.up, Wup = x.W * a.up, pad = a.k / 2;
  if (a.pad >= 0) {
    SD_REQUIRE(a.pad == 0 && a.stride == 2 && a.k == 3, kUnsupported, "%s: explicit padding %d", name.c_str(), a.pad);
    return {(Hup + 1 - a.k) / a.stride + 1, (Wup + 1 - a.k) / a.stride + 1, 0};
  }
  return {(Hup + 2 * pad - a.k) / a.stride + 1, (Wup + 2 * pad - a.k) / a.stride + 1, -1};
}
}

Tensor Net::conv(std::vector<Op>& ops, const std::string& name, const Tensor& x, const ConvArgs& a) {
  if (f32_) return conv_f32(ops, name, x, a);
  const int cin = x.C + (a.x2 ? a.x2->C : 0);
  const bool geglu = a.out_mode == kOutGeglu;
  const float* b = a.bias ? upload_vec(name + ".bias", a.cout, geglu) : nullptr;
  const WeightPin pin = weight_plan(name, x, a, false);
  const WeightSource could = ws_->observe() && !ws_->palette(name + ".weight") && !a.silu_out
                                 ? conv_plan_weights(conv_shape(name, x, a), StoredWeights::W8A8, ws_->observe_gemms() && a.keep_compressed).kind
                                 : WeightSource::Fp16;
  if (could == WeightSource::I8Wstream || (could == WeightSource::I8Halo && ws_->observe() >= 2) || could == WeightSource::I8Gemm) {
    float* slot = ll_.arena.alloc_n<float>(1);
    observed_.push_back({name + ".weight", slot});
    const half_t *p0 = x.p, *p1 = a.x2 ? a.x2->p : nullptr;
    const size_t n0 = x.numel(), n1 = a.x2 ? a.x2->numel() : 0;
    ops.push_back([=](hipStream_t s) { launch_absmax_half(p0, n0, p1, n1, slot, s); });
    ops.back().label = "absmax " + name;
  }
  if (pin.kind != WeightSource::Fp16) return conv_w(ops, name, upload_compressed(name, pin, cin, a), b, x, a);
  if (a.subpix && !a.silu_out && subpixel_wanted(conv_shape(name, x, a))) return conv_w(ops, name, ConvWeights(upload_subpixel_weight(name, a.cout, cin), true), b, x, a);
  return conv_w(ops, name, upload_conv_weight(name, a.cout, cin, a.k, geglu), b, x, a);
}

WeightPin Net::weight_plan(const std::string& name, const Tensor& x, const ConvArgs& a, bool ln) const {
  if (f32_ || a.silu_out) return {};
  const StoredWeights held = ws_->palette(name + ".weight") ? StoredWeights::Palette
                             : ws_->w8a8(name + ".weight")  ? StoredWeights::W8A8
                                                            : StoredWeights::Fp16;
  ConvDesc d = conv_shape(name, x, a);
  static const float present = 0.f;
  if (ln) d.ln_colsum = d.bias = &present;
  return conv_plan_weights(d, held, a.keep_compressed);
}

bool Net::observes_geglu(const std::string& name, const Tensor& x, const ConvArgs& a, bool ln) const {
  if (f32_ || !ws_->observe() || !ws_->observe_geglus() || ws_->palette(name + ".weight") || a.out_mode != kOutGeglu) return false;
  ConvDesc d = conv_shape(name, x, a);
  static const float present = 0.f;
  if (ln) d.ln_colsum = d.bias = &present;
  return conv_plan_weights(d, StoredWeights::W8A8, a.keep_compressed).kind == WeightSource::I8Geglu;
}

bool Net::observes_tail(const std::string& name, const Tensor& x, const ConvArgs& a) const {
  if (f32_ || !ws_->observe() || !ws_->observe_tails() || ws_->palette(name + ".weight") || a.out_mode != kOutHalf) return false;
  const WeightSource could = conv_plan_weights(conv_shape(name, x, a), StoredWeights::W8A8, a.keep_compressed).kind;
  return could == (a.x_i8 ? WeightSource::I8GemmQ : WeightSource::I8Gemm);
}

void Net::observe_tensor(std::vector<Op>& ops, const std::string& name, const Tensor& t, const std::vector<std::string>& report_as) {
  float* slot = ll_.arena.alloc_n<float>(1);
  if (report_as.empty()) observed_.push_back({name + ".weight", slot});
  for (const std::string& n : report_as) observed_.push_back({n + ".weight", slot});
  const half_t* p0 = t.p;
  const size_t n0 = t.numel();
  ops.push_back([=](hipStream_t s) { launch_absmax_half(p0, n0, nullptr, 0, slot, s); });
  ops.back().label = "absmax " + name;
}

ConvDesc Net::qkv_shape(const std::string& name, const Tensor& x, const ConvArgs& a) const {
  ConvArgs plain = a;
  plain.ln_colsum = nullptr;
  plain.x_i8 = nullptr;
  ConvDesc d = conv_shape(name, x, plain);
  static const half_t present = 0;
  d.out_t = const_cast<half_t*>(&present);
  d.n_trans = a.n_trans;
  d.vt_perm = a.vt_perm ? 1 : 0;
  d.q_scale = a.q_scale;
  d.q_cols = a.q_cols;
  return d;
}

WeightPin Net::qkv_plan(const std::string& name, const std::vector<std::string>& parts, const Tensor& x, const ConvArgs& a) const {
  if (f32_ || a.silu_out || parts.empty()) return {};
  const W8A8Mark* first = nullptr;
  for (const std::string& p : parts) {
    const W8A8Mark* m = ws_->w8a8(p + ".weight");
    if (!m || ws_->palette(p + ".weight")) return {};
    if (!first) first = m;
    if (m->act_absmax != first->act_absmax) return {};
  }
  return conv_plan_weights(qkv_shape(name, x, a), StoredWeights::W8A8, true);
}

bool Net::observes_qkv(const std::string& name, const std::vector<std::string>& parts, const Tensor& x, const ConvArgs& a) const {
  if (f32_ || !ws_->observe() || !ws_->observe_qkv()) return false;
  for (const std::string& p : parts)
    if (ws_->palette(p + ".weight")) return false;
  return conv_plan_weights(qkv_shape(name, x, a), StoredWeights::W8A8, true).kind == WeightSource::I8Qkv;
}

ConvWeights Net::upload_qkv_i8(const std::vector<std::string>& parts, const WeightPin& pin, int cin, int cout_each) {
  const size_t per = (size_t)cout_each * cin;
  std::vector<int8_t> q(parts.size() * per);
  std::vector<float> w_scale(parts.size() * cout_each);
  float act_absmax = 0.f;
  for (size_t i = 0; i < parts.size(); ++i) {
    const std::string wname = parts[i] + ".weight";
    const W8A8Mark* i8 = ws_->w8a8(wname);
    SD_REQUIRE(i8 && ws_->get(wname).numel() == per && i8->q.size() == per && i8->w_scale.size() == (size_t)cout_each, kInvalidArgument,
               "%s: expected %zu W8A8 values (%d,%d,1,1)", wname.c_str(), per, cout_each, cin);
    std::copy(i8->q.begin(), i8->q.end(), q.begin() + i * per);
    std::copy(i8->w_scale.begin(), i8->w_scale.end(), w_scale.begin() + i * cout_each);
    act_absmax = i8->act_absmax;
// ... 29 lines not shown
               "%s: expected %zu W8A8 values (%d,%d,%d,%d)", wname.c_str(), expect, a.cout, cin, a.k, a.k);
    cw = upload_w8a8(up, pin.kind, wname.c_str(), i8->q.data(), i8->w_scale.data(), i8->act_absmax, a.cout, cin, a.k, &bytes);
    ++i8_applied_;
    i8_bytes_ += bytes;
    i8_names_.push_back(wname);
  } else {
    const Palette* pal = ws_->palette(wname);
    SD_REQUIRE(pal && ws_->get(wname).numel() == expect && pal->indices.size() == expect, kInvalidArgument,
               "%s has %zu elements, expected %zu (%d,%d,%d,%d)", wname.c_str(), ws_->get(wname).numel(), expect, a.cout, cin, a.k, a.k);
    SD_REQUIRE(palette_bits_ok(pal->nbits) && pal->lut.size() == (size_t)1 << pal->nbits, kInternal, "%s: a palette of %zu entries for %d bits",
               wname.c_str(), pal->lut.size(), pal->nbits);
    cw = upload_palettized(up, pin.kind, wname.c_str(), reinterpret_cast<const half_t*>(pal->lut.data()), pal->nbits, pal->indices.data(), a.cout,
                           cin, a.k, &bytes);
    if (!ln_name.empty()) cw.ln_gamma = upload_vec(ln_name + ".weight", cin);
    ++pal_streamed_;
    pal_stream_bytes_ += bytes;
  }
  holds_compressed(wname);
  return ConvWeights(cw, pin);
}

int Net::activation_range(int index, std::string* name, float* absmax) {
  if (index < 0 || index >= (int)observed_.size()) return (int)observed_.size();
  SD_HIP(hipSetDevice(ll_.device));
  SD_HIP(hipStreamSynchronize(ll_.stream));
  SD_HIP(hipMemcpy(absmax, observed_[(size_t)index].second, sizeof(float), hipMemcpyDeviceToHost));
  *name = observed_[(size_t)index].first;
  return (int)observed_.size();
}

Tensor Net::conv_f32(std::vector<Op>& ops, const std::string& name, const Tensor& x, const ConvArgs& a) {
  const int cout = a.cout, k = a.k;
  const float* b = a.bias ? upload_vec(name + ".bias", cout) : nullptr;
  SD_REQUIRE(!a.x2 && !a.temb && !a.ln_colsum && a.out_mode == kOutHalf && !a.silu_out, kInternal, "%s: not a VAE conv", name.c_str());
  const float* w = upload_conv_weight_f32(name, cout, x.C, k);
  const ConvGeom g = conv_geom(name, x, a);
  Tensor out = new_tensor(x.B, g.Ho, g.Wo, cout);
  ConvF32Desc fd;
  fd.x = x.f();
  fd.w = w;
  fd.w_kind = 1;
  fd.bias = b;
  fd.res = reinterpret_cast<const float*>(a.res);
  fd.out = out.f();
  fd.B = x.B; fd.Hi = x.H; fd.Wi = x.W; fd.Cin = x.C; fd.Ho = g.Ho; fd.Wo = g.Wo; fd.N = cout;
  fd.ksize = k; fd.stride = a.stride; fd.up = a.up; fd.pad = g.pad;
  ops.push_back([fd](hipStream_t s) { launch_conv_f32(fd, s); });
  char buf[256];
  snprintf(buf, sizeof(buf), "conv%dx%d fp32 %d->%d @%dx%d %s", k, k, x.C, cout, g.Ho, g.Wo, name.c_str());
  ops.back().label = buf;
  ops.back().flop = 2.0 * x.B * g.Ho * g.Wo * (double)cout * x.C * k * k;
  return out;
}

ConvDesc Net::conv_shape(const std::string& name, const Tensor& x, const ConvArgs& a) const {
  const Tensor* x2 = a.x2;
  const bool ln = a.ln_colsum != nullptr;
  ConvDesc d;
  d.x0 = x.p;
  d.C0 = x.C;
  if (x2) {
    SD_REQUIRE(x2->B == x.B && x2->H == x.H && x2->W == x.W, kInternal, "%s: concat shape mismatch", name.c_str());
    d.x1 = x2->p;
    d.C1 = x2->C;
  }
  d.temb = a.temb;
  d.temb_stride = kTembCap;
  d.res = a.res;
  d.B = x.B;
  d.Hi = x.H;
  d.Wi = x.W;
  const ConvGeom g = conv_geom(name, x, a);
  d.Ho = g.Ho;
  d.Wo = g.Wo;
  d.pad = g.pad;
  d.ksize = a.k;
  d.stride = a.stride;
  d.up = a.up;
  d.N = a.cout;
  d.out_mode = a.out_mode;
  d.ldT = a.ldT;
  d.ln_colsum = a.ln_colsum;
  d.x0_i8 = a.x_i8;
  if (ln || a.x_i8) {
    d.vt_perm = a.vt_perm ? 1 : 0;
    d.q_scale = a.q_scale;
    d.q_cols = a.q_cols;
  }
  return d;
}

Tensor Net::conv_w(std::vector<Op>& ops, const std::string& name, const ConvWeights& weights, const float* bias, const Tensor& x, const ConvArgs& a) {
  const Tensor* x2 = a.x2;
  const int cout = a.cout, k = a.k;
  const bool geglu = a.out_mode == kOutGeglu, ln = a.ln_colsum != nullptr;
  const half_t* w = weights.w;
  ConvDesc d = conv_shape(name, x, a);
  d.w = w;
  d.bias = bias;
  d.cw = weights.cw;
  d.tile = weights.pin.tile;
  d.staging = weights.pin.staging;
  d.splitk = weights.pin.splitk;
  d.subpix = weights.subpix;
  Tensor out;
  const bool qkv = (ln || a.x_i8) && a.n_trans > 0;
  if (qkv) {
    out = new_tensor(x.B, d.Ho, d.Wo, a.n_trans);
    *a.vt_out = ll_.arena.alloc_n<half_t>((size_t)x.B * (cout - a.n_trans) * a.ldT);
    d.out_t = *a.vt_out;
    d.n_trans = a.n_trans;
  } else if (a.out_mode == kOutHalfT) {
    out.B = x.B; out.H = 1; out.W = a.ldT; out.C = cout;
    out.p = ll_.arena.alloc_n<half_t>((size_t)x.B * cout * a.ldT);
  } else if (a.out_q8) {
    SD_REQUIRE(geglu && d.cw.kind == WeightSource::I8Geglu && a.out_inv_s > 0.f, kInternal, "%s: an int8 output needs the int8 GEGLU kernel", name.c_str());
    out.B = x.B; out.H = d.Ho; out.W = d.Wo; out.C = cout / 2;
    d.out_q8 = a.out_q8;
    d.out_inv_s = a.out_inv_s;
  } else {
    out = new_tensor(x.B, d.Ho, d.Wo, geglu ? cout / 2 : cout);
  }
  d.out = out.p;
  SD_REQUIRE(!ln || (conv_fast_path_ok(d) && !a.silu_out), kInternal, "%s: LayerNorm fold / fused q|k|v off the MFMA path",
             name.c_str());
  std::shared_ptr<GnHook> hook;
  if (a.out_mode == kOutHalf && !qkv) {
    hook = std::make_shared<GnHook>();
    out.gn = hook;
    hook->ops_pos = (int)ops.size();
    hook->ops_list = &ops;
  }
  auto with_hook = [hook](const ConvDesc& d0) {
    ConvDesc dd = d0;
    if (hook) {
      dd.gn_partial = hook->partial;
      dd.gn_groups = hook->groups;
    }
    return dd;
  };
  const int cin = x.C + (x2 ? x2->C : 0);
  if (conv_fast_path_ok(d) && !a.silu_out) {
    const ConvWeightCopies copies = d.cw.kind != WeightSource::Fp16 ? ConvWeightCopies{false, false, false} : conv_plan_copies(d);
    if (copies.wstream && !ln) {
      half_t* wt = ll_.arena.alloc_n<half_t>(wstream_tiled_halves(cout, cin, k));
      derive(w, [=] { launch_wstream_retile(w, wt, cout, cin, k, ll_.stream); });
      d.w_tiled = wt;
    }
    if (copies.wsgemm) {
      half_t* wt = ll_.arena.alloc_n<half_t>(wsgemm_tiled_halves(cout));
      derive(w, [=] { launch_wsgemm_retile(w, wt, cout, geglu, ll_.stream); });
      d.w_ws = wt;
    }
    if (copies.bvgemm) {
      half_t* wt = ll_.arena.alloc_n<half_t>(bvgemm_tiled_halves(cout, x.C));
      const int c0 = x.C;
      derive(w, [=] { launch_bvgemm_retile(w, wt, cout, c0, geglu, ll_.stream); });
      d.w_bv = wt;
    }
    ll_.ws_need = std::max(ll_.ws_need, conv_workspace_bytes(d));
    ops.push_back([this, d, hook, with_hook](hipStream_t s) {
      const int n = launch_conv(with_hook(d), ll_.ws_conv, s);
      if (hook) hook->produced(n);
    });
  } else {
    const int so = a.silu_out ? 1 : 0;
    ops.push_back([d, so, hook, with_hook](hipStream_t s) {
      const int n = launch_conv_generic(with_hook(d), so, s);
      if (hook) hook->produced(n);
    });
  }
  char buf[320];
  const int kind = d.out_t ? 3 : (geglu ? 2 : (ln ? 1 : 0));
  const WeightSource src = d.cw.kind;
  const std::string lnmark = ln ? "+ln" : "", palmark = "+pal" + std::to_string(d.cw.bits);
  const std::string mark = d.subpix ? "+subpix" : src == WeightSource::PalGeglu ? palmark + lnmark : lnmark + (d.cw.i8() ? (d.out_q8 ? "+q8out+w8a8" : "+w8a8") : src != WeightSource::Fp16 ? palmark : "");
  snprintf(buf, sizeof(buf), "%s%s %d->%d @%dx%d M=%d K=%d %s #%d,%d,%d,%d,%d,%d,%d",
           k == 3 ? "conv3x3" : (geglu ? (src == WeightSource::PalGeglu ? "geglu" : "geglu1x1") : "gemm1x1"), mark.c_str(), cin, cout, d.Ho, d.Wo,
           x.B * d.Ho * d.Wo, cin * k * k, name.c_str(), kind, k, a.stride, a.up, cin, cout, x.B * d.Ho * d.Wo);
  ops.back().label = buf;
  ops.back().flop = 2.0 * x.B * d.Ho * d.Wo * (double)cout * cin * k * k;
  return out;
}

void Net::conv_small_n(std::vector<Op>& ops, const std::string& name, const Tensor& x, int cout, half_t* out_nhwc, float* out_nchw) {
  if (f32_) {
    ConvF32Desc fd;
    fd.x = x.f(); fd.w = upload_conv_weight_f32(name, cout, x.C, 3); fd.w_kind = 1; fd.bias = upload_vec(name + ".bias", cout);
    fd.out = out_nhwc ? reinterpret_cast<float*>(out_nhwc) : new_tensor(x.B, x.H, x.W, cout).f();
    fd.B = x.B; fd.Hi = x.H; fd.Wi = x.W; fd.Cin = x.C; fd.Ho = x.H; fd.Wo = x.W; fd.N = cout; fd.ksize = 3;
    ops.push_back([=](hipStream_t s) {
      launch_conv_f32(fd, s);
      if (out_nchw) launch_nhwc_to_nchw_f32f32(fd.out, out_nchw, fd.B, fd.N, fd.Ho, fd.Wo, s);
    });
  } else {
    ConvDesc d;
    d.x0 = x.p;
    d.C0 = x.C;
    d.w = upload_conv_weight(name, cout, x.C, 3, false);
    d.bias = upload_vec(name + ".bias", cout);
    d.out = out_nhwc;
    d.B = x.B; d.Hi = x.H; d.Wi = x.W; d.Ho = x.H; d.Wo = x.W;
    d.ksize = 3; d.stride = 1; d.up = 1; d.N = cout;
    ops.push_back([=](hipStream_t s) { launch_conv_small_n(d, out_nchw, s); });
  }
  ops.back().label = "conv3x3 small-N " + name + (out_nchw ? " -> fp32 NCHW" : "");
  ops.back().flop = 2.0 * x.M() * (double)cout * x.C * 9;
}

Tensor Net::group_norm_f32(std::vector<Op>& ops, const std::string& name, const Tensor& x, float eps, bool silu) {
  const int C = x.C, G = cfg_.norm_num_groups;
  void* scratch = ll_.arena.alloc(groupnorm_f32_scratch_bytes(x.B, G));
  const float* gamma = upload_vec(name + ".weight", C);
  const float* beta = upload_vec(name + ".bias", C);
  Tensor y = new_tensor(x.B, x.H, x.W, C);
  const float* xp = x.f();
  float* yp = y.f();
  const int B = x.B, HW = x.H * x.W, si = silu ? 1 : 0;
  ops.push_back([=](hipStream_t s) { launch_groupnorm_f32(xp, scratch, gamma, beta, yp, B, HW, C, G, eps, si, s); });
  ops.back().label = "groupnorm fp32 C=" + std::to_string(C) + " @" + std::to_string(x.H) + "x" + std::to_string(x.W) + " " + name;
  return y;
}

Tensor Net::group_norm(std::vector<Op>& ops, const std::string& name, const Tensor& x, const Tensor* x2, float eps,
                       bool silu, const ConvDesc* side, const std::string& side_label, double side_flop) {
  SD_REQUIRE(!side || !f32_, kInternal, "%s: side GEMM on the fp32 path", name.c_str());
  const int C = x.C + (x2 ? x2->C : 0);
  const int G = cfg_.norm_num_groups;
  SD_REQUIRE(C % G == 0, kUnsupported, "%s: %d channels not divisible by %d groups", name.c_str(), C, G);
  if (f32_) {
    SD_REQUIRE(!x2, kInternal, "%s: concat GroupNorm on the fp32 path", name.c_str());
    return group_norm_f32(ops, name, x, eps, silu);
  }
  const float* gamma = upload_vec(name + ".weight", C);
  const float* beta = upload_vec(name + ".bias", C);
  Tensor y = new_tensor(x.B, x.H, x.W, C);
  float* partial = ll_.arena.alloc_n<float>(groupnorm_scratch_floats(x.B, x.H * x.W, G));
  const half_t* p0 = x.p;
  const half_t* p1 = x2 ? x2->p : nullptr;
  const int C0 = x.C, C1 = x2 ? x2->C : 0, B = x.B, HW = x.H * x.W, si = silu ? 1 : 0;
  half_t* yp = y.p;
  std::shared_ptr<GnHook> hook;
  if (!x2 && x.gn && !x.gn->partial && groupnorm_wants_producer_stats(HW, C, G)) {
    SD_REQUIRE(x.gn->ops_list == &ops && x.gn->ops_pos >= 0 && x.gn->ops_pos < (int)ops.size(), kInternal,
               "%s: GroupNorm producer statistics need the producing op earlier in the same launch list", name.c_str());
    hook = x.gn;
    hook->partial = partial;
    hook->groups = G;
  }
  const std::string label = "groupnorm C=" + std::to_string(C) + " @" + std::to_string(x.H) + "x" + std::to_string(x.W) + " " + name;
  if (side) {
    const ConvDesc sd = *side;
    ops.push_back([=](hipStream_t s) {
      launch_groupnorm(p0, C0, p1, C1, partial, gamma, beta, yp, B, HW, G, eps, si, s, hook ? hook->consume() : 0, &sd);
    });
    ops.back().label = label + " || " + side_label;
    ops.back().flop = side_flop;
    return y;
  }
  ops.push_back([=](hipStream_t s) {
    launch_groupnorm(p0, C0, p1, C1, partial, gamma, beta, yp, B, HW, G, eps, si, s, hook ? hook->consume() : 0);
  });
  ops.back().label = label;
  return y;
}

Tensor Net::resnet(std::vector<Op>& ops, const std::string& p, const Tensor& x, const Tensor* x2, int cout, const float* temb) {
  const int cin = x.C + (x2 ? x2->C : 0);
  static const int side_mode = tune_env_int("SD_GN_SIDE", 1);
  const half_t* side_out = nullptr;
  Tensor t0;
  if (cin != cout && side_mode != 0 && !f32_) {
    ConvDesc sd;
    sd.x0 = x.p;
    sd.C0 = x.C;
    if (x2) {
      sd.x1 = x2->p;
      sd.C1 = x2->C;
    }
    sd.B = x.B;
    sd.Hi = sd.Ho = x.H;
    sd.Wi = sd.Wo = x.W;
    sd.N = cout;
    if (gn_side_gemm_ok(sd)) {
      sd.w = upload_conv_weight(p + ".conv_shortcut", cout, cin, 1, false);
      sd.bias = upload_vec(p + ".conv_shortcut.bias", cout);
      Tensor sc = new_tensor(x.B, x.H, x.W, cout);
      sd.out = sc.p;
      side_out = sc.p;
      char buf[256];
      snprintf(buf, sizeof(buf), "gemm1x1 %d->%d @%dx%d M=%d K=%d %s.conv_shortcut", cin, cout, x.H, x.W, x.M(), cin, p.c_str());
      t0 = group_norm(ops, p + ".norm1", x, x2, cfg_.norm_eps, true, &sd, buf, 2.0 * x.M() * (double)cout * cin);
    }
  }
  if (!side_out) t0 = group_norm(ops, p + ".norm1", x, x2, cfg_.norm_eps, true);
  Tensor h = conv(ops, p + ".conv1", t0, {.cout = cout, .k = 3, .temb = temb});
  Tensor t1 = group_norm(ops, p + ".norm2", h, nullptr, cfg_.norm_eps, true);
  const half_t* shortcut;
  if (side_out) {
    shortcut = side_out;
  } else if (cin != cout) {
    shortcut = conv(ops, p + ".conv_shortcut", x, {.x2 = x2, .cout = cout}).p;
  } else {
    SD_REQUIRE(x2 == nullptr, kInternal, "%s: concat input with identity shortcut", p.c_str());
    shortcut = x.p;
  }
  return conv(ops, p + ".conv2", t1, {.cout = cout, .k = 3, .res = shortcut});
}

void Net::invalidate_graphs() {
  if (ll_.graph) { (void)hipGraphExecDestroy(ll_.graph); ll_.graph = nullptr; }
}

void Net::set_attention(int impl) {
  SD_REQUIRE(impl >= 0 && impl <= 2, kInvalidArgument, "attention impl %d", impl);
  if (impl != cfg_.attention_impl) {
    cfg_.attention_impl = impl;
    invalidate_graphs();
  }
}

void Net::run_ops_on(const std::vector<Op>& ops, hipStream_t s) {
  static const bool trace = tune_env_set("SD_NAN_TRACE");
  if (trace) {
    hipStreamCaptureStatus cs = hipStreamCaptureStatusNone;
    if (hipStreamIsCapturing(s, &cs) == hipSuccess && cs == hipStreamCaptureStatusNone) {
      unsigned long long* d = nullptr;
      SD_HIP(hipMalloc(&d, sizeof(unsigned long long)));
      auto scan = [&]() {
        SD_HIP(hipMemsetAsync(d, 0, sizeof(unsigned long long), s));
        const Arena& ar = ll_.arena;
        for (size_t i = 0; i < ar.chunks().size(); ++i) launch_count_nonfinite_half(ar.chunks()[i], ar.chunk_bytes()[i], d, s);
        unsigned long long h = 0;
        SD_HIP(hipMemcpyAsync(&h, d, sizeof(h), hipMemcpyDeviceToHost, s));
        SD_HIP(hipStreamSynchronize(s));
        return h;
      };
      unsigned long long last = scan();
      fprintf(stderr, "nan-trace: %llu non-finite fp16 patterns in the arena before the list\n", last);
      for (auto& op : ops) {
        op(s);
        const unsigned long long now = scan();
        if (now != last) fprintf(stderr, "nan-trace: %llu -> %llu after  %s\n", last, now, op.label.c_str());
        last = now;
      }
      (void)hipFree(d);
      return;
    }
  }
  static const bool poison = tune_env_set("SD_POISON_LDS");
  for (auto& op : ops) {
    if (poison) launch_lds_poison(s);
    op(s);
  }
}

void Net::run_forward() {
  if (!cfg_.use_graph) return run_eager();
  if (!ll_.graph) {
    run_eager();
    SD_HIP(hipStreamSynchronize(ll_.stream));
    ll_.graph = capture_graph(ll_.stream, [&] { run_eager(); });
  }
  SD_HIP(hipGraphLaunch(ll_.graph, ll_.stream));
}

// ... 47 lines not shown
```

ml-stable-diffusion_amd/csrc/net.h:

```cpp
#pragma once
#include "../../include/sd_mi355x.h"
#include "conv_plan.h"
#include "launch_list.h"

#include <functional>
#include <map>
#include <set>

namespace sd {

constexpr int kTembCap = 65536;
inline int round_up(int x, int a) { return (x + a - 1) / a * a; }

struct GnHook {
  float* partial = nullptr;
  int groups = 0;
  int entries = 0;
  bool fresh = false;
  void produced(int n) {
    entries = n;
    fresh = true;
  }
  int consume() {
    const int n = fresh ? entries : 0;
    fresh = false;
    return n;
  }
  int ops_pos = -1;
  const void* ops_list = nullptr;
};

struct Tensor {
  half_t* p = nullptr;
  int B = 0, H = 0, W = 0, C = 0;
  std::shared_ptr<GnHook> gn;
  int M() const { return B * H * W; }
  size_t numel() const { return (size_t)B * H * W * C; }
  float* f() const { return reinterpret_cast<float*>(p); }
};

struct OpTime {
  std::string label;
  double flop;
  float ms;
};

struct ConvArgs {
  const Tensor* x2 = nullptr;
  int cout = 0;
  int k = 1, stride = 1, up = 1;
  bool bias = true;
  const float* temb = nullptr;
  const half_t* res = nullptr;
  int out_mode = kOutHalf;
  int ldT = 0;
  bool silu_out = false;
  int pad = -1;
  const float* ln_colsum = nullptr;
  int n_trans = 0;
  half_t** vt_out = nullptr;
  bool vt_perm = false;
  float q_scale = 1.f;
  int q_cols = 0;
  bool keep_compressed = false;
  bool subpix = false;
  const int8_t* x_i8 = nullptr;
  int8_t* out_q8 = nullptr;
  float out_inv_s = 0.f;
};

struct ConvWeights {
  const half_t* w = nullptr;
  CompressedWeights cw;
  WeightPin pin;
  bool subpix = false;
  ConvWeights(const half_t* fp16, bool folded = false) : w(fp16), subpix(folded) {}
  ConvWeights(const CompressedWeights& c, const WeightPin& p) : cw(c), pin(p) {}
};

class Net {
 public:
  virtual ~Net() { close(); }
  Net(const Net&) = delete;
  float time_forward(int warmup, int iters);
  std::vector<OpTime> profile(int iters);
  virtual void set_attention(int impl);
  void drop_graphs() { invalidate_graphs(); }
  size_t device_bytes() const { return ll_.arena.bytes(); }
  size_t arena_used_bytes() const { return ll_.arena.used(); }
  void palette_info(int* n_palettized, int* n_streamed, size_t* stream_bytes) const {
    *n_palettized = pal_tensors_;
    *n_streamed = pal_streamed_;
    *stream_bytes = pal_stream_bytes_;
  }
  void w8a8_info(int* n_marked, int* n_applied, size_t* bytes) const {
    *n_marked = i8_marked_;
    *n_applied = i8_applied_;
    *bytes = i8_bytes_;
  }
  int activation_range(int index, std::string* name, float* absmax);
  const std::vector<std::string>& w8a8_applied() const { return i8_names_; }
  const sd_unet_config& config() const { return cfg_; }
  virtual void reload_weights(const WeightStore& ws, const std::vector<std::string>& names);

 protected:
  Net(const sd_unet_config& cfg, const WeightStore& ws, int device);
  void open(int device) { ll_.open(device); }
  void seal();
  void close() { ll_.close(); }

  Tensor new_tensor(int B, int H, int W, int C);
  half_t* upload_conv_weight(const std::string& name, int cout, int cin, int k, bool geglu);
  float* upload_conv_weight_f32(const std::string& name, int cout, int cin, int k);
  half_t* upload_subpixel_weight(const std::string& name, int cout, int cin);
  float* upload_vec(const std::string& name, int n, bool geglu = false);
  Tensor conv(std::vector<Op>& ops, const std::string& name, const Tensor& x, const ConvArgs& a);
  Tensor conv_w(std::vector<Op>& ops, const std::string& name, const ConvWeights& w, const float* bias, const Tensor& x, const ConvArgs& a);
  WeightPin weight_plan(const std::string& name, const Tensor& x, const ConvArgs& a, bool ln) const;
  ConvWeights upload_compressed(const std::string& name, const WeightPin& pin, int cin, const ConvArgs& a, const std::string& ln_name = std::string());
  bool observes_geglu(const std::string& name, const Tensor& x, const ConvArgs& a, bool ln) const;
  bool observes_tail(const std::string& name, const Tensor& x, const ConvArgs& a) const;
  void observe_tensor(std::vector<Op>& ops, const std::string& name, const Tensor& t, const std::vector<std::string>& report_as = {});
  WeightPin qkv_plan(const std::string& name, const std::vector<std::string>& parts, const Tensor& x, const ConvArgs& a) const;
  bool observes_qkv(const std::string& name, const std::vector<std::string>& parts, const Tensor& x, const ConvArgs& a) const;
  ConvWeights upload_qkv_i8(const std::vector<std::string>& parts, const WeightPin& pin, int cin, int cout_each);
  void conv_small_n(std::vector<Op>& ops, const std::string& name, const Tensor& x, int cout, half_t* out_nhwc, float* out_nchw);
  Tensor group_norm(std::vector<Op>& ops, const std::string& name, const Tensor& x, const Tensor* x2, float eps,
                    bool silu, const ConvDesc* side = nullptr, const std::string& side_label = std::string(), double side_flop = 0);
  Tensor resnet(std::vector<Op>& ops, const std::string& p, const Tensor& x, const Tensor* x2, int cout, const float* temb);

  using Fill = std::function<void(const WeightStore&)>;
  void refill(const std::vector<std::string>& sources, const void* made, Fill fill);
  void derive(const void* from, std::function<void()> launch);
  void holds_compressed(const std::string& wname) { compressed_.insert(wname); }
  virtual void after_reload() {}

  void run_ops(const std::vector<Op>& ops) { run_ops_on(ops, ll_.stream); }
  void run_ops_on(const std::vector<Op>& ops, hipStream_t s);
  virtual void run_eager() { run_ops(ll_.ops); }
  void run_forward();
  virtual void invalidate_graphs();
  virtual std::vector<const std::vector<Op>*> forward_lists() const { return {&ll_.ops}; }

  sd_unet_config cfg_;
  const WeightStore* ws_ = nullptr;
  bool f32_ = false;
  LaunchList ll_;
  bool have_inputs_ = false;

 private:
  ConvDesc conv_shape(const std::string& name, const Tensor& x, const ConvArgs& a) const;
  ConvDesc qkv_shape(const std::string& name, const Tensor& x, const ConvArgs& a) const;
  int pal_tensors_ = 0, pal_streamed_ = 0;
  size_t pal_stream_bytes_ = 0;
  int i8_marked_ = 0, i8_applied_ = 0;
  size_t i8_bytes_ = 0;
  std::vector<std::pair<std::string, float*>> observed_;
  std::vector<std::string> i8_names_;
  struct Refill {
    std::vector<std::string> sources;
    Fill fill;
  };
  std::vector<Refill> refills_;
  std::map<std::string, std::vector<int64_t>> source_shape_;
  std::map<const void*, std::vector<std::string>> made_from_;
  std::set<std::string> compressed_;
  bool observing_ = false;
  Tensor conv_f32(std::vector<Op>& ops, const std::string& name, const Tensor& x, const ConvArgs& a);
  Tensor group_norm_f32(std::vector<Op>& ops, const std::string& name, const Tensor& x, float eps, bool silu);
};

struct EventList {
  std::vector<hipEvent_t> ev;
  explicit EventList(size_t n) {
    ev.reserve(n);
    for (size_t i = 0; i < n; ++i) {
      hipEvent_t e = nullptr;
      SD_HIP(hipEventCreate(&e));
      ev.push_back(e);
    }
  }
  ~EventList() {
    for (hipEvent_t e : ev) (void)hipEventDestroy(e);
  }
  hipEvent_t operator[](size_t i) const { return ev[i]; }
};

}

struct sd_unet {
  std::unique_ptr<sd::Net> impl;
};
```

ml-stable-diffusion_amd/csrc/weight_prep.h:

```cpp
#pragma once
#include <algorithm>
#include <cmath>
#include <cstddef>
#include <cstdint>
#include <vector>

#include "kernels.h"

namespace sd {

inline int geglu_row(int o, int n) {
  const int half_n = n / 2;
  const bool gate = o >= half_n;
  const int j = gate ? o - half_n : o;
  return (j / 32) * 64 + (gate ? 32 : 0) + (j % 32);
}

template <typename S, typename D>
void retile_ohwi(const S* src, int cout, int cin, int k, bool geglu, D* dst) {
  const int kk = k * k;
  for (int o = 0; o < cout; ++o) {
    const int dst_o = geglu ? geglu_row(o, cout) : o;
    for (int c = 0; c < cin; ++c)
      for (int t = 0; t < kk; ++t) dst[((size_t)dst_o * kk + t) * cin + c] = (D)src[((size_t)o * cin + c) * kk + t];
  }
}

inline size_t subpixel_fold_halves(int cout, int cin) { return (size_t)16 * cout * cin; }
inline int subpixel_first(int phase_bit, int d) { return phase_bit == 0 ? d : 2 * d; }
inline int subpixel_count(int phase_bit, int d) { return (phase_bit == 0) == (d == 0) ? 1 : 2; }
template <typename S>
void subpixel_fold(const S* src, int cout, int cin, half_t* dst) {
  SD_REQUIRE(src && dst && cout > 0 && cin > 0, kInvalidArgument, "subpixel_fold: Cout %d Cin %d", cout, cin);
  for (int p = 0; p < 4; ++p) {
    const int a = p >> 1, b = p & 1;
    for (int o = 0; o < cout; ++o)
      for (int t = 0; t < 4; ++t) {
        const int dy = t >> 1, dx = t & 1;
        const int ky0 = subpixel_first(a, dy), nky = subpixel_count(a, dy), kx0 = subpixel_first(b, dx), nkx = subpixel_count(b, dx);
        half_t* row = dst + (((size_t)p * cout + o) * 4 + t) * cin;
        for (int c = 0; c < cin; ++c) {
          const S* w9 = src + ((size_t)o * cin + c) * 9;
          float s = 0.f;
          for (int ky = ky0; ky < ky0 + nky; ++ky)
            for (int kx = kx0; kx < kx0 + nkx; ++kx) s += (float)w9[ky * 3 + kx];
          SD_REQUIRE(std::fabs(s) <= 65504.0f, kInvalidArgument, "subpixel_fold: the folded weight of output %d input %d phase %d tap %d is %g, outside fp16",
                     o, c, p, t, (double)s);
          row[c] = (half_t)s;
        }
      }
  }
}

template <typename W>
void fold_layernorm_rows(const W* w, const float* bias, const float* gamma, const float* beta, int cout, int cin, int row0,
                         bool geglu, half_t* w_out, float* colsum, float* bias_out) {
  for (int o = 0; o < cout; ++o) {
    const int dst = geglu ? geglu_row(o, cout) : row0 + o;
    double cs = 0.0, bb = bias ? (double)bias[o] : 0.0;
    for (int c = 0; c < cin; ++c) {
      const float wv = (float)w[(size_t)o * cin + c];
      const half_t h = gamma ? (half_t)(wv * gamma[c]) : (half_t)w[(size_t)o * cin + c];
      w_out[(size_t)dst * cin + c] = h;
      cs += (double)(float)h;
      if (beta) bb += (double)wv * (double)beta[c];
    }
    colsum[dst] = (float)cs;
    bias_out[dst] = (float)bb;
  }
}

struct PalLaneWriter {
  int nbits;
  std::vector<uint8_t> bytes;
  uint64_t window = 0;
  int held = 0;
  size_t at = 0;
  PalLaneWriter(int nbits_, int words) : nbits(nbits_), bytes((size_t)words * 16 + 8, (uint8_t)0) {}
  void put(uint64_t index) {
    window |= index << held;
    held += nbits;
    while (held >= 8) {
      bytes[at++] = (uint8_t)window;
      window >>= 8;
      held -= 8;
    }
  }
  void flush(uint8_t* wave_block, int lane) {
    if (held) bytes[at++] = (uint8_t)window;
    for (size_t q = 0; (q + 1) * 16 + 8 <= bytes.size(); ++q)
      std::copy(bytes.begin() + q * 16, bytes.begin() + (q + 1) * 16, wave_block + (q * 64 + lane) * 16);
    std::fill(bytes.begin(), bytes.end(), (uint8_t)0);
    window = 0;
    held = 0;
    at = 0;
  }
};

inline int wstream_pal_words(int taps, int nbits) { return (2 * taps * 8 * nbits + 127) / 128; }
inline size_t wstream_pal_bytes(int N, int Ctot, int ksize, int nbits) {
  return (size_t)(N / 32) * (Ctot / 32) * wstream_pal_words(ksize * ksize, nbits) * 64 * 16;
}
inline void wstream_pal_pack(const uint8_t* indices, int N, int Ctot, int ksize, int nbits, uint8_t* dst) {
  const int taps = ksize * ksize, nslices = Ctot / 32, Q = wstream_pal_words(taps, nbits), nf = 2 * taps;
  PalLaneWriter w(nbits, Q);
  for (int strip = 0; strip < N / 32; ++strip)
    for (int slice = 0; slice < nslices; ++slice)
      for (int lane = 0; lane < 64; ++lane) {
// ... 162 lines not shown
```

ml-stable-diffusion_amd/python_hip_stable_diffusion/_lib.py:

```python
import ctypes as C
import os

import numpy as np

_HERE = os.path.dirname(os.path.abspath(__file__))
LIB_PATH = os.environ.get("SD_MI355X_LIB", os.path.join(os.path.dirname(_HERE), "lib", "libsdmi355.so"))

SD_MAX_LEVELS = 6
SD_FLAG_DEVICE_PTRS = 1
ATTENTION_IMPLEMENTATIONS = {"ORIGINAL": 0, "SPLIT_EINSUM": 1, "SPLIT_EINSUM_V2": 2}


class LibraryNotBuilt(ImportError):
    pass


class UNetConfig(C.Structure):
    _fields_ = [
        ("batch", C.c_int32), ("in_channels", C.c_int32), ("out_channels", C.c_int32),
        ("height", C.c_int32), ("width", C.c_int32), ("n_levels", C.c_int32),
        ("block_out_channels", C.c_int32 * SD_MAX_LEVELS),
        ("down_cross_attn", C.c_int32 * SD_MAX_LEVELS),
        ("up_cross_attn", C.c_int32 * SD_MAX_LEVELS),
        ("layers_per_block", C.c_int32),
# ... 39 lines not shown

ACTS = {"quick_gelu": 0, "gelu": 1}

PROGRESS_FN = C.CFUNCTYPE(C.c_int, C.c_void_p, C.c_int, C.c_int, C.POINTER(C.c_float), C.POINTER(C.c_float))

_lib = None

_P, _I, _F = C.c_void_p, C.c_int, C.c_float
_FP = C.POINTER(C.c_float)
SYMBOLS = [
    ("sd_last_error", C.c_char_p, []),
    ("sd_version", C.c_char_p, []),
    ("sd_device_count", _I, []),
    ("sd_weights_create", _I, [C.POINTER(_P)]),
    ("sd_weights_add", _I, [_P, C.c_char_p, _P, _I, C.POINTER(C.c_int64), _I]),
    ("sd_weights_load_safetensors", _I, [_P, C.c_char_p, C.c_char_p]),
    ("sd_weights_count", _I, [_P]),
    ("sd_weights_destroy", None, [_P]),
    ("sd_weights_set_values", _I, [_P, C.c_char_p, _FP, C.c_size_t]),
    ("sd_weights_tensor_info", _I, [_P, _I, C.c_char_p, _I, C.POINTER(C.c_int64), C.POINTER(_I)]),
    ("sd_weights_palettize", _I, [_P, C.c_char_p, _I, C.POINTER(C.c_double)]),
    ("sd_weights_add_palettized", _I, [_P, C.c_char_p, _P, _I, _P, C.POINTER(C.c_int64), _I]),
    ("sd_weights_palette_bits", _I, [_P, C.c_char_p]),
    ("sd_weights_read_palette", _I, [_P, C.c_char_p, _P, _P, _FP]),
    ("sd_weights_quantize_w8a8", _I, [_P, C.c_char_p, _F, C.POINTER(C.c_double)]),
    ("sd_weights_w8a8_info", _I, [_P, C.c_char_p, _FP]),
    ("sd_weights_observe_activations", _I, [_P, _I]),
    ("sd_weights_observe_gemms", _I, [_P, _I]),
    ("sd_weights_observe_geglus", _I, [_P, _I]),
    ("sd_weights_observe_qkv", _I, [_P, _I]),
    ("sd_weights_observe_tails", _I, [_P, _I]),
    ("sd_unet_w8a8_info", _I, [_P, C.POINTER(_I), C.POINTER(_I), C.POINTER(C.c_size_t)]),
    ("sd_unet_w8a8_layer", _I, [_P, _I, C.c_char_p, _I]),
    ("sd_unet_activation_ranges", _I, [_P, _I, C.c_char_p, _I, _FP]),
    ("sd_op_conv2d_w8a8", _I, [_P, _P, _P, _FP, _F, _FP, _P, _P, _I, _I, _I, _I, _I, _I, _I, _I, _I, C.POINTER(_I), _I, _FP]),
    ("sd_op_w8a8_pack", _I, [_P, _I, _I, _I, _P, C.POINTER(C.c_size_t)]),
    ("sd_op_conv2d_w8a8_halo", _I, [_P, _P, _P, _FP, _F, _FP, _FP, _P, _P, _I, _I, _I, _I, _I, _I, _I, _I, _I, C.POINTER(_I), _I, _FP]),
    ("sd_op_w8a8_pack_halo", _I, [_P, _I, _I, _P, C.POINTER(C.c_size_t)]),
    ("sd_op_subpixel_fold", _I, [_P, _I, _I, _I, _P, C.POINTER(C.c_size_t)]),
    ("sd_op_subpixel_refusal", _I, [_I, _I, _I, _I, _I, _I, _I, _I, _I, _I, C.c_char_p, _I]),
    ("sd_op_conv2d_subpixel", _I, [_P, _P, _FP, _P, _P, _I, _I, _I, _I, _I, _I, _I, C.POINTER(_I), _I, _FP]),
    ("sd_op_gemm_w8a8", _I, [_P, _P, _FP, _F, _FP, _P, _P, _I, _I, _I, _I, _I, _I, C.POINTER(_I), _I, _FP]),
    ("sd_op_w8a8_pack_gemm", _I, [_P, _I, _I, _P, C.POINTER(C.c_size_t)]),
    ("sd_op_layernorm_q8", _I, [_P, _FP, _FP, _F, _F, _P, _I, _I, _I, _FP]),
    ("sd_op_geglu_w8a8", _I, [_P, _P, _FP, _F, _FP, _P, _I, _I, _I, _I, C.POINTER(_I), _I, _FP]),
    ("sd_op_w8a8_pack_geglu", _I, [_P, _I, _I, _P, C.POINTER(C.c_size_t)]),
    ("sd_op_geglu_w8a8_q8", _I, [_P, _P, _FP, _F, _FP, _F, _P, _I, _I, _I, _I, C.POINTER(_I), _I, _FP]),
    ("sd_op_gemm_q8", _I, [_P, _P, _FP, _F, _FP, _P, _P, _I, _I, _I, _I, C.POINTER(_I), _I, _FP]),
    ("sd_op_qkv_w8a8", _I, [_P, _P, _FP, _F, _FP, _P, _P, _I, _I, _I, _F, _I, _I, C.POINTER(_I), _I, _FP]),
    ("sd_op_w8a8_pack_qkv", _I, [_P, _I, _P, C.POINTER(C.c_size_t)]),
    ("sd_op_quantize_weight", _I, [_FP, _I, C.c_size_t, _P, _FP, C.POINTER(C.c_double)]),
    ("sd_op_absmax", _I, [_P, C.c_size_t, _FP]),
    ("sd_unet_create", _I, [C.POINTER(UNetConfig), _P, _I, C.POINTER(_P)]),
    ("sd_unet_destroy", None, [_P]),
    ("sd_unet_set_attention", _I, [_P, _I]),
    ("sd_unet_reload_weights", _I, [_P, _P, C.POINTER(C.c_char_p), _I]),
    ("sd_unet_num_residuals", _I, [_P]),
    ("sd_unet_device_bytes", C.c_size_t, [_P]),
    ("sd_unet_arena_used_bytes", C.c_size_t, [_P]),
    ("sd_unet_palette_info", _I, [_P, C.POINTER(_I), C.POINTER(_I), C.POINTER(C.c_size_t)]),
    ("sd_unet_forward", _I, [_P, C.POINTER(UNetIO)]),
    ("sd_unet_time_forward", _I, [_P, _I, _I, _FP]),
    ("sd_unet_denoise_loop", _I, [_P, C.POINTER(UNetIO), _FP, _I, _I, _FP, _FP, _FP, _I, _F, _FP, _FP]),
    ("sd_unet_denoise_loop_progress", _I, [_P, C.POINTER(UNetIO), _FP, _I, _I, _FP, _FP, _FP, _I, _F, _FP, _FP, _FP, _I, _P, _P,
                                           C.POINTER(_I)]),
    ("sd_tune_set_candidate", _I, [_I, _I, _I]),
    ("sd_tune_set_plan_table", _I, [C.c_char_p, C.c_void_p, C.POINTER(C.c_int)]),
    ("sd_unet_profile", _I, [_P, _I, _I, _FP, C.POINTER(C.c_double), C.c_char_p, _I, C.POINTER(_I)]),
    ("sd_unet_attach_controlnets", _I, [_P, C.POINTER(_P), _I]),
    ("sd_controlnet_set_cond", _I, [_P, _P, _I]),
    ("sd_vae_decoder_create", _I, [C.POINTER(UNetConfig), _P, _I, C.POINTER(_P)]),
    ("sd_vae_decode", _I, [_P, _P, _I, _FP, _I]),
    ("sd_vae_encoder_create", _I, [C.POINTER(UNetConfig), _P, _I, C.POINTER(_P)]),
    ("sd_vae_encode", _I, [_P, _P, _I, _FP, _I]),
    ("sd_vae_encode_latents", _I, [_P, _P, _I, _FP, _FP, _I, _F, _F, _F, _FP, _I]),
    ("sd_text_encoder_create", _I, [_P, _P, _I, C.POINTER(_P)]),
    ("sd_text_encoder_destroy", None, [_P]),
    ("sd_text_encoder_device_bytes", C.c_size_t, [_P]),
    ("sd_text_encoder_encode", _I, [_P, C.POINTER(C.c_int32), _I, _FP, _FP, _FP]),
    ("sd_op_attention", _I, [_I, _P, _P, _P, _P, _I, _I, _I, _I, _I, _I, _I, _FP]),
    ("sd_op_layernorm", _I, [_P, _FP, _FP, _P, _I, _I, _I, _F, _I, _FP]),
    ("sd_op_groupnorm", _I, [_P, _FP, _FP, _P, _I, _I, _I, _I, _I, _F, _I, _I, _FP]),
    ("sd_op_groupnorm_shortcut", _I, [_P, _P, _FP, _FP, _P, _FP, _P, _P, _I, _I, _I, _I, _I, _I, _I, _F, _I, _I, _I, _FP]),
    ("sd_op_conv2d", _I, [_P, _P, _FP, _P, _P, _I, _I, _I, _I, _I, _I, _I, _I, _I, _I, _I, _I, _FP]),
    ("sd_op_conv2d_ex", _I, [_P, _P, _P, _FP, _FP, _P, _P, _I, _I, _I, _I, _I, _I, _I, _I, _I, _I, _I, _FP, _FP, _F, _I, _P, _I, _I, _I,
                             C.POINTER(_I), _I, _FP]),
    ("sd_op_conv2d_palettized", _I, [_P, _P, _P, _I, _P, _FP, _P, _P, _I, _I, _I, _I, _I, _I, _I, _I, _I, C.POINTER(_I), _I, _FP]),
    ("sd_op_palette_pack", _I, [_P, _I, _I, _I, _I, _P, C.POINTER(C.c_size_t)]),
    ("sd_op_gemm_palettized", _I, [_P, _P, _I, _P, _FP, _P, _P, _I, _I, _I, _I, _I, _I, C.POINTER(_I), _I, _FP]),
    ("sd_op_palette_pack_gemm", _I, [_P, _I, _I, _I, _P, C.POINTER(C.c_size_t)]),
    ("sd_op_geglu_palettized", _I, [_P, _FP, _FP, _P, _I, _P, _FP, _P, _I, _I, _I, C.c_float, _I, C.POINTER(_I), _I, _FP]),
    ("sd_op_palette_pack_geglu", _I, [_P, _I, _I, _I, _P, C.POINTER(C.c_size_t)]),
    ("sd_op_conv2d_groupnorm", _I, [_P, _P, _FP, _P, _FP, _FP, _P, _P, _I, _I, _I, _I, _I, _I, _I, _F, _I, _I, _I, C.POINTER(_I), _I, _FP]),
    ("sd_op_conv2d_groupnorm_proj", _I, [_P, _P, _FP, _P, _FP, _FP, _P, _FP, _P, _P, _I, _I, _I, _I, _I, _I, _I, _I, _F, _I, _I, C.POINTER(_I), _I, _FP]),
    ("sd_op_conv2d_groupnorm_conv3x3", _I, [_P, _P, _FP, _P, _FP, _FP, _P, _FP, _P, _P, _P, _I, _I, _I, _I, _I, _I, _I, _I, _F, _I, _I, _I, _I,
                                            C.POINTER(_I), _I, _FP]),
    ("sd_op_cross_attention_fused", _I, [_P, _FP, _FP, _P, _P, _P, _P, _I, _I, _I, _I, _F, _I, _I, _FP]),
    ("sd_op_ffn_out_proj", _I, [_P, _P, _FP, _P, _P, _FP, _P, _P, _FP, _I, _I, _I, _I, _I, _I, _FP]),
    ("sd_op_fold_linear", _I, [_P, _FP, _P, _FP, _P, _FP, _I, _I, _I]),
    ("sd_op_cross_attention_block", _I, [_P, _FP, _FP, _P, _P, _P, _P, _FP, _P, _P, _FP, _P, _I, _I, _I, _I, _F, _I, _I, _FP]),
    ("sd_op_geglu", _I, [_P, _P, _FP, _P, _I, _I, _I, _I, _FP]),
    ("sd_op_geglu_ln", _I, [_P, _FP, _FP, _P, _FP, _P, _I, _I, _I, C.c_float, _I, _I, _FP]),
    ("sd_op_qkv_ln", _I, [_P, _FP, _FP, _P, _P, _P, _I, _I, _I, C.c_float, C.c_float, _I, _I, _I, _FP]),
    ("sd_op_gn_proj_qkv", _I, [_P, _P, _FP, _FP, _P, _FP, _FP, _FP, _P, _P, _P, _P, _I, _I, _I, _I, _I, C.c_float, C.c_float, C.c_float, _I, _I,
                               C.POINTER(C.c_int), _I, _FP]),
    ("sd_op_timestep_embedding", _I, [_FP, _FP, _I, _I, _I, _F]),
    ("sd_op_posterior_noise", _I, [_FP, _FP, _FP, _FP, _I, _I, _I, _I, _F, _F, _F, _I, _FP]),
    ("sd_op_sched_step", _I, [_FP, _FP, _FP, _FP, _FP, _FP, _F, _I, _I, _I, _I, _FP, C.POINTER(_I)]),
    ("sd_op_conv_plan", _I, [_I] * 18 + [C.POINTER(C.c_int), C.POINTER(C.c_ulonglong)]),
    ("sd_op_conv_plan_kernel", _I, [_I] * 18 + [C.c_char_p, _I]),
    ("sd_numpy_randn", _I, [C.c_uint32, C.POINTER(C.c_double), C.c_size_t]),
    ("sd_torch_randn", _I, [C.c_uint32, C.POINTER(C.c_double), C.c_size_t]),
    ("sd_philox_randn", _I, [C.c_uint64, C.c_uint32, C.POINTER(C.c_double), C.c_size_t]),
    ("sd_calibrate", _I, [_I, _FP]),
    ("sd_selftest_mfma", _I, []),
    ("sd_safety_checker_create", _I, [C.POINTER(SafetyCheckerConfig), _P, _I, C.POINTER(_P)]),
    ("sd_safety_checker_destroy", None, [_P]),
    ("sd_safety_checker_device_bytes", C.c_size_t, [_P]),
    ("sd_safety_checker_last_ms", C.c_float, [_P]),
    ("sd_safety_checker_run", _I, [_P, _P, _F, _FP, _FP, _FP, _FP, _I]),
    ("sd_op_vit_attention", _I, [_P, _P, _I, _I, _I, _I, _I, _FP]),
    ("sd_op_safety_head", _I, [_FP, _FP, _FP, _FP, _FP, _F, _I, _I, _I, _I, _FP, _FP]),
    ("sd_op_vae_attention", _I, [_P, _P, _P, _P, _I, _I, _I, _I, _FP]),
    ("sd_vae_decode_images", _I, [_P, _P, _I, _FP, _P, _P, C.POINTER(ImagePost), _F, _FP, _FP, _I]),
    ("sd_op_resample_coeffs", _I, [_I, _I, C.POINTER(_I), _P, _P]),
    ("sd_op_image_rgb8", _I, [_FP, _P, _I, _I, _I, _I, _FP]),
    ("sd_op_clip_input", _I, [_P, _P, _I, _I, _I, _I, _I, _I, _FP, _FP, _I, _FP]),
    ("sd_op_conv_f32", _I, [_FP, _P, _I, _FP, _FP, _FP, _I, _I, _I, _I, _I, _I, _I, _I, _I]),
    ("sd_op_groupnorm_f32", _I, [_FP, _FP, _FP, _FP, _I, _I, _I, _I, _I, _F, _I]),
    ("sd_op_row_softmax", _I, [_P, _I, _I, _F, _I]),
    ("sd_op_gemv", _I, [_P, _FP, _FP, _FP, _I, _I, _I, _I, _I, _I]),
    ("sd_op_clip_attention", _I, [_P, _P, _I, _I, _I]),
    ("sd_op_clip_embed", _I, [C.POINTER(C.c_int32), _P, _P, _P, _I, _I, _I]),
    ("sd_op_clip_act", _I, [_P, C.c_size_t, _I]),
    ("sd_op_layout", _I, [_I, _P, _P, _I, _I, _I, _I]),
    ("sd_op_sum_half", _I, [C.POINTER(_P), _I, _P, C.c_size_t, _I]),
    ("sd_op_vit_patch_rows", _I, [_P, _P, _I, _I, _I, _I]),
    ("sd_op_vit_tokens", _I, [_P, _P, _P, _P, _I, _I, _I]),
    ("sd_op_harness_selftest", _I, [_I, _P, _FP, C.c_size_t]),
]


def lib():
    global _lib
    if _lib is not None:
        return _lib
    if not os.path.exists(LIB_PATH):
        raise LibraryNotBuilt(
            f"{LIB_PATH} is missing - build it with `python -c 'import __graft_entry__ as g; g.build()'` "
            f"or `make -C ml-stable-diffusion_amd/csrc`. There is no CPU fallback.")
    if not os.environ.get("SD_MI355X_NO_TORCH"):
        try:
            import torch
        except Exception:
            pass
    handle = C.CDLL(LIB_PATH, mode=C.RTLD_GLOBAL)
    for name, restype, argtypes in SYMBOLS:
        fn = getattr(handle, name)
        fn.restype = restype
        fn.argtypes = argtypes
    _lib = handle
    return handle


_EXC = {-1: ValueError, -2: FileNotFoundError, -3: RuntimeError, -4: NotImplementedError, -5: RuntimeError}

# ... 563 lines not shown
    if x.ndim != 4 or indices.ndim != 2 or indices.shape[1] != x.shape[1]:
        raise ValueError("gemm_palettized: x must be (B, Cin, H, W) and indices (Cout, Cin)")
    B, Cin, H, W = x.shape
    Cout = indices.shape[0]
    if nbits in (1, 2, 4, 6, 8) and lut.shape != (1 << nbits,):
        raise ValueError("gemm_palettized: lut must hold 2 ** nbits entries")
    bias = None if bias is None else f32(bias)
    res = None if res is None else f16(res)
    if (bias is not None and bias.shape != (Cout,)) or (res is not None and res.shape != (B, Cout, H, W)):
        raise ValueError("gemm_palettized: bias must be (Cout,), res (B, Cout, H, W)")
    n = B * Cout * H * W
    if out is None:
        out = np.empty(n, np.float16)
    if out.dtype != np.float16 or not out.flags.c_contiguous or out.size < n:
        raise ValueError("gemm_palettized: out must be a C-contiguous float16 buffer of at least B * Cout * H * W elements")
    plan = (C.c_int * 4)()
    ms = C.c_float(0)
    check(lib().sd_op_gemm_palettized(ptr(x), ptr(lut), nbits, ptr(indices), fptr(bias), ptr(res), ptr(out), B, Cin, H, W, Cout, bm, plan,
                                      iters, C.byref(ms)))
    return out.reshape(-1)[:n].reshape(B, Cout, H, W), list(plan), ms.value


def palette_pack_gemm(indices, nbits):
    indices = np.ascontiguousarray(indices, dtype=np.uint8)
    if indices.ndim != 2:
        raise ValueError("palette_pack_gemm: indices must be (Cout, K)")
    Cout, K = indices.shape
    return _packed(lib().sd_op_palette_pack_gemm, ptr(indices), Cout, K, nbits).reshape(Cout // 16, -1, nbits, 64, 16)


def geglu_palettized(x, lut, indices, nbits, bias=None, ln_weight=None, ln_bias=None, eps=1e-5, bm=0, out=None, iters=1):
    x, lut = f16(x), f16(lut)
    indices = np.ascontiguousarray(indices, dtype=np.uint8)
    if x.ndim != 2 or indices.ndim != 2 or indices.shape[1] != x.shape[1]:
        raise ValueError("geglu_palettized: x must be (M, C) and indices (N2, C)")
    M, Cn = x.shape
    N2 = indices.shape[0]
    if nbits in (1, 2, 4, 6, 8) and lut.shape != (1 << nbits,):
        raise ValueError("geglu_palettized: lut must hold 2 ** nbits entries")
    bias = None if bias is None else f32(bias)
    ln_weight = None if ln_weight is None else f32(ln_weight)
    ln_bias = None if ln_bias is None else f32(ln_bias)
    if (bias is not None and bias.shape != (N2,)) or any(v is not None and v.shape != (Cn,) for v in (ln_weight, ln_bias)):
        raise ValueError("geglu_palettized: bias must be (N2,), ln_weight / ln_bias (C,)")
    n = M * (N2 // 2)
    if out is None:
        out = np.empty(n, np.float16)
    if out.dtype != np.float16 or not out.flags.c_contiguous or out.size < n:
        raise ValueError("geglu_palettized: out must be a C-contiguous float16 buffer of at least M * N2 / 2 elements")
    plan = (C.c_int * 4)()
    ms = C.c_float(0)
    check(lib().sd_op_geglu_palettized(ptr(x), fptr(ln_weight), fptr(ln_bias), ptr(lut), nbits, ptr(indices), fptr(bias), ptr(out), M, Cn,
                                       N2, eps, bm, plan, iters, C.byref(ms)))
    return out.reshape(-1)[:n].reshape(M, N2 // 2), list(plan), ms.value


def palette_pack_geglu(indices, nbits):
    indices = np.ascontiguousarray(indices, dtype=np.uint8)
    if indices.ndim != 2:
        raise ValueError("palette_pack_geglu: indices must be (N2, K)")
    N2, K = indices.shape
    return _packed(lib().sd_op_palette_pack_geglu, ptr(indices), N2, K, nbits).reshape(N2 // 16, -1, nbits, 64, 16)


def groupnorm_shortcut(x0, x1, gn_weight, gn_bias, w, bias=None, groups=32, eps=1e-5, silu=True, side=True, iters=1):
    x0, w = f16(x0), f16(w)
    x1 = None if x1 is None else f16(x1)
    B, C0, H, W = x0.shape
    C1 = 0 if x1 is None else x1.shape[1]
    N = w.shape[0]
    w = np.ascontiguousarray(w.reshape(N, -1))
    if w.shape[1] != C0 + C1 or (x1 is not None and x1.shape != (B, C1, H, W)):
        raise ValueError("groupnorm_shortcut: inconsistent shapes")
    gn_weight, gn_bias = f32(gn_weight), f32(gn_bias)
    bias = None if bias is None else f32(bias)
    out_gn = np.empty((B, C0 + C1, H, W), np.float16)
    out_sc = np.empty((B, N, H, W), np.float16)
    ms = C.c_float(0)
    check(lib().sd_op_groupnorm_shortcut(ptr(x0), ptr(x1), fptr(gn_weight), fptr(gn_bias), ptr(w), fptr(bias), ptr(out_gn), ptr(out_sc),
                                         B, C0, C1, H, W, N, groups, eps, int(silu), int(side), iters, C.byref(ms)))
    return out_gn, out_sc, ms.value


def conv2d_groupnorm(x, w, gn_weight, gn_bias, bias=None, res=None, groups=32, eps=1e-5, silu=False, tile=0,
                     producer_stats=True, iters=1):
    x, w = f16(x), f16(w)
    B, Cin, H, W = x.shape
    Cout, Cin2, k, k2 = w.shape
    if Cin2 != Cin or k != k2:
        raise ValueError("conv2d_groupnorm: weight shape does not match input")
    bias = None if bias is None else f32(bias)
    res = None if res is None else f16(res)
    gn_weight, gn_bias = f32(gn_weight), f32(gn_bias)
    conv_out = np.empty((B, Cout, H, W), np.float16)
    out = np.empty((B, Cout, H, W), np.float16)
    ms, entries = C.c_float(0), C.c_int(0)
    check(lib().sd_op_conv2d_groupnorm(ptr(x), ptr(w), fptr(bias), ptr(res), fptr(gn_weight), fptr(gn_bias), ptr(conv_out),
                                       ptr(out), B, Cin, H, W, Cout, k, groups, eps, int(silu), tile, int(producer_stats),
                                       C.byref(entries), iters, C.byref(ms)))
    return conv_out, out, entries.value, ms.value


def conv2d_groupnorm_proj(x, w, gn_weight, gn_bias, proj_w, proj_bias=None, bias=None, res=None, groups=32, eps=1e-6, fold=True,
                          tile=0, iters=1):
    x, w, proj_w = f16(x), f16(w), f16(proj_w)
    B, Cin, H, W = x.shape
    Cout, k = w.shape[0], w.shape[2]
    Np = proj_w.shape[0]
    if w.shape[1] != Cin or proj_w.reshape(Np, -1).shape[1] != Cout:
        raise ValueError("conv2d_groupnorm_proj: inconsistent shapes")
    proj_w = np.ascontiguousarray(proj_w.reshape(Np, Cout))
    gn_weight, gn_bias = f32(gn_weight), f32(gn_bias)
    bias = None if bias is None else f32(bias)
    proj_bias = None if proj_bias is None else f32(proj_bias)
    res = None if res is None else f16(res)
    conv_out = np.empty((B, Cout, H, W), np.float16)
    out = np.empty((B, Np, H, W), np.float16)
    ms, entries = C.c_float(0), C.c_int(0)
    check(lib().sd_op_conv2d_groupnorm_proj(ptr(x), ptr(w), fptr(bias), ptr(res), fptr(gn_weight), fptr(gn_bias), ptr(proj_w),
                                            fptr(proj_bias), ptr(conv_out), ptr(out), B, Cin, H, W, Cout, k, Np, groups, eps,
                                            int(fold), tile, C.byref(entries), iters, C.byref(ms)))
    return conv_out, out, entries.value, ms.value


def conv2d_groupnorm_conv3x3(x, w, gn_weight, gn_bias, w2, bias2=None, res2=None, bias=None, res=None, groups=32, eps=1e-5, silu=True,
                             fold=True, tile=0, staging2=0, iters=1):
    x, w, w2 = f16(x), f16(w), f16(w2)
    B, Cin, H, W = x.shape
    Cout, k = w.shape[0], w.shape[2]
    N2 = w2.shape[0]
    if w.shape[1] != Cin or w2.shape[1:] != (Cout, 3, 3):
        raise ValueError("conv2d_groupnorm_conv3x3: inconsistent shapes")
    gn_weight, gn_bias = f32(gn_weight), f32(gn_bias)
    bias = None if bias is None else f32(bias)
    bias2 = None if bias2 is None else f32(bias2)
    res = None if res is None else f16(res)
    res2 = None if res2 is None else f16(res2)
    conv_out = np.empty((B, Cout, H, W), np.float16)
    out = np.empty((B, N2, H, W), np.float16)
    ms, entries = C.c_float(0), C.c_int(0)
    check(lib().sd_op_conv2d_groupnorm_conv3x3(ptr(x), ptr(w), fptr(bias), ptr(res), fptr(gn_weight), fptr(gn_bias), ptr(w2), fptr(bias2),
                                               ptr(res2), ptr(conv_out), ptr(out), B, Cin, H, W, Cout, k, N2, groups, eps, int(silu),
                                               int(fold), tile, staging2, C.byref(entries), iters, C.byref(ms)))
    return conv_out, out, entries.value, ms.value


def cross_attention_block(x, ln_weight, ln_bias, wq, k, v, wo, bo, heads, eps=1e-5, fused=True, iters=1, a1=None, wo1=None, bo1=None):
    x, k, v, wq, wo = f16(x), f16(k), f16(v), f16(wq), f16(wo)
    B, Cn, _, Sq = x.shape
    Sk = k.shape[3]
    if Cn != heads * 64 or k.shape[1] != Cn or v.shape != k.shape or wq.shape != (Cn, Cn) or wo.shape != (Cn, Cn):
        raise ValueError("cross_attention_block: inconsistent shapes")
    ln_weight, ln_bias, bo = f32(ln_weight), f32(ln_bias), f32(bo)
    if a1 is not None:
        a1, wo1, bo1 = f16(a1), f16(wo1), f32(bo1)
        if a1.shape != x.shape or wo1.shape != (Cn, Cn):
            raise ValueError("cross_attention_block: inconsistent shapes of a1 / wo1")
    out = np.empty_like(x)
    ms = C.c_float(0)
    check(lib().sd_op_cross_attention_block(ptr(x), fptr(ln_weight), fptr(ln_bias), ptr(wq), ptr(k), ptr(v), ptr(wo), fptr(bo), ptr(a1), ptr(wo1),
                                            fptr(bo1), ptr(out), B, heads, Sq, Sk, eps, int(fused), iters, C.byref(ms)))
    return out, ms.value


def ffn_out_proj(g, w1, b1, res1, w2, b2, res2, groups=0, fused=True, iters=1):
    g, res1, res2, w1, w2 = f16(g), f16(res1), f16(res2), f16(w1), f16(w2)
# ... 334 lines not shown
```

Before: 248.0 it/s.

## Fold ResNet shortcut GEMM into norm2 launch as split-K slabs combined by conv2

In resnet blocks whose 1x1 shortcut could not ride in norm1's GroupNorm launch, the shortcut GEMM now runs as side work in norm2's GroupNorm launch. It writes fp32 partial slabs that conv2's split-K reduction sums in, with the two biases pre-summed. This removes the standalone shortcut kernel and the fp16 residual round trip, and fills idle CUs during the GroupNorm. The cost is extra fp32 slab workspace and more combine reads, and the feature is gated by a planner with several refusal conditions plus an env switch that defaults to on.

```diff
diff --git a/include/sd_mi355x.h b/include/sd_mi355x.h
--- a/include/sd_mi355x.h
+++ b/include/sd_mi355x.h
@@ -168,6 +168,12 @@
 int sd_op_groupnorm_shortcut(const void* x0, const void* x1, const float* gn_weight, const float* gn_bias, const void* w, const float* bias,
                              void* out_gn, void* out_sc, int B, int C0, int C1, int H, int W, int N, int groups, float eps, int silu,
                              int side, int iters, float* ms);
+int sd_op_resnet_tail(const void* h, const void* x0, const void* x1, const float* gn_weight, const float* gn_bias, const void* w2, const float* b2,
+                      const void* wsc, const float* bsc, void* out_gn, void* out, int B, int C, int C0, int C1, int H, int W, int groups, float eps,
+                      int silu, int slabs, int conv2_tile, int conv2_splitk, int stats_entries, int* plan_out, int iters, float* ms);
+int sd_op_shortcut_slabs_plan(int B, int H, int W, int C0, int C1, int N, int gn_blocks, int flags, int* plan, unsigned long long* bytes, char* text,
+                              int text_bytes);
+int sd_op_sum_bias(const float* b2, const float* bs, int n, float* dst);
 int sd_op_conv2d(const void* x, const void* w, const float* bias, const void* res, void* out, int B, int Cin, int H,
                  int W, int Cout, int ksize, int stride, int upsample, int tile, int splitk, int force_generic,
                  int iters, float* ms);
diff --git a/ml-stable-diffusion_amd/csrc/capi_ops.cpp b/ml-stable-diffusion_amd/csrc/capi_ops.cpp
--- a/ml-stable-diffusion_amd/csrc/capi_ops.cpp
+++ b/ml-stable-diffusion_amd/csrc/capi_ops.cpp
@@ -432,6 +432,128 @@
     });
     download_nchw(dy, out_gn, B, C, H, W);
     download_nchw(ds, out_sc, B, N, H, W);
+  });
+}
+
+int sd_op_resnet_tail(const void* h, const void* x0, const void* x1, const float* gn_weight, const float* gn_bias, const void* w2, const float* b2,
+                      const void* wsc, const float* bsc, void* out_gn, void* out, int B, int C, int C0, int C1, int H, int W, int groups, float eps,
+                      int silu, int slabs, int conv2_tile, int conv2_splitk, int stats_entries, int* plan_out, int iters, float* ms) {
+  return guarded([&] {
+    SD_REQUIRE(h && x0 && gn_weight && gn_bias && w2 && b2 && wsc && bsc && out_gn && out && plan_out, kInvalidArgument, "NULL argument");
+    SD_REQUIRE(B >= 1 && C >= 1 && C0 >= 1 && C1 >= 0 && H >= 1 && W >= 1 && groups >= 1 && C % groups == 0 && slabs <= 8 && conv2_splitk >= 0 &&
+                   (conv2_tile == 0 || conv2_tile == 7 || conv2_tile == 9) && stats_entries >= 0 && stats_entries <= kGnMaxSlabs && stats_entries <= H * W,
+               kInvalidArgument, "resnet_tail: bad arguments (conv2_tile is 0, 7 or 9; slabs <= 8; stats_entries <= min(%d, H W))", kGnMaxSlabs);
+    if (!x1) C1 = 0;
+    const int Cs = C0 + C1, HW = H * W, M = B * HW;
+    Scratch sc("resnet_tail");
+    half_t* dh = upload_nhwc(sc, h, B, C, H, W);
+    half_t* d0 = upload_nhwc(sc, x0, B, C0, H, W);
+    half_t* d1 = x1 ? upload_nhwc(sc, x1, B, C1, H, W) : nullptr;
+    half_t* dy = sc.out<half_t>((size_t)M * C, "out_gn");
+    half_t* dout = sc.out<half_t>((size_t)M * C, "out");
+    float* dgw = sc.dev<float>(C, gn_weight);
+    float* dgb = sc.dev<float>(C, gn_bias);
+    float* partial = nullptr;
+    if (stats_entries > 0) {
+      std::vector<float> st(groupnorm_scratch_floats(B, HW, groups), 1.0e30f);
+      const half_t* hh = f16(h);
+      const int cpg = C / groups;
+      for (int b = 0; b < B; ++b)
+        for (int g = 0; g < groups; ++g)
+          for (int e = 0; e < stats_entries; ++e) {
+            const int p0 = (int)((long)HW * e / stats_entries), p1 = (int)((long)HW * (e + 1) / stats_entries);
+            double s1 = 0, s2 = 0;
+            for (int c = g * cpg; c < (g + 1) * cpg; ++c)
+              for (int p = p0; p < p1; ++p) {
+                const double v = (double)(float)hh[((size_t)b * C + c) * HW + p];
+                s1 += v;
+                s2 += v * v;
+              }
+            float* dst = st.data() + (((size_t)b * groups + g) * kGnMaxSlabs + e) * 2;
+            dst[0] = (float)s1;
+            dst[1] = (float)s2;
+          }
+      partial = sc.dev<float>(st.size(), st.data(), "GroupNorm partials");
+    } else {
+      partial = poisoned_gn_partial(sc, B, HW, groups);
+    }
+    ConvDesc c2 = conv_desc(dy, C, upload_conv_weight(sc, w2, C, C, 3), nullptr, nullptr, dout, B, H, W, C, 3);
+    c2.tile = conv2_tile;
+    c2.splitk = conv2_splitk;
+    ConvDesc sd = conv_desc(d0, C0, sc.dev<half_t>((size_t)C * Cs, f16(wsc)), nullptr, nullptr, nullptr, B, H, W, C);
+    sd.x1 = d1;
+    sd.C1 = C1;
+    SD_REQUIRE(conv_fast_path_ok(c2) && conv_fast_path_ok(sd), kInvalidArgument, "resnet_tail: C=%d C0=%d C1=%d not MFMA-tileable", C, C0, C1);
+    if (slabs < 0) {
+      const ShortcutSlabs ss = shortcut_slabs_plan(c2, sd, stats_entries > 0 ? 512 : B * groups, true);
+      SD_REQUIRE(ss.splits > 0, kUnsupported, "resnet_tail: the shortcut does not ride as slabs: %s", ss.refusal);
+      slabs = ss.splits;
+    }
+    const bool pinned = conv2_tile != 0 || conv2_splitk != 0;
+    if (c2.tile == 9 || (!pinned && conv_plan_copies(c2).wstream)) tile_for_wstream(sc, c2, "resnet_tail: conv2's shape is not eligible for plan tile 9 (wstream.hip)");
+    const bool side = slabs > 0 || gn_side_gemm_ok(sd);
+    ConvWorkspace ws;
+    if (slabs > 0) {
+      std::vector<float> bsum((size_t)C);
+      sum_bias(b2, bsc, C, bsum.data());
+      c2.bias = sc.dev<float>(C, bsum.data());
+      float* xs = sc.out<float>((size_t)slabs * M * C, "shortcut slabs");
+      c2.xslabs = sd.xslabs = xs;
+      c2.n_xslabs = sd.n_xslabs = slabs;
+      SD_REQUIRE(gn_side_gemm_ok(sd), kUnsupported, "resnet_tail: the shortcut GEMM cannot ride as %d slabs (M=%d K=%d)", slabs, M, Cs);
+      ws = workspace_for(sc, {c2});
+    } else {
+      sd.bias = sc.dev<float>(C, bsc);
+      sd.out = sc.out<half_t>((size_t)M * C, "shortcut");
+      c2.bias = sc.dev<float>(C, b2);
+      c2.res = sd.out;
+      if (!side) {
+        const ConvWeightCopies cp = conv_plan_copies(sd);
+        if (cp.wstream) tile_for_wstream(sc, sd, "resnet_tail: shortcut not eligible for plan tile 9");
+        if (cp.bvgemm) tile_for_bvgemm(sc, sd, "resnet_tail: shortcut not eligible for plan tile 11");
+      }
+      ws = workspace_for(sc, {c2, sd});
+    }
+    const ConvPlan p = conv_plan(c2);
+    plan_out[0] = p.tile; plan_out[1] = p.staging; plan_out[2] = p.splitk; plan_out[3] = p.slab ? 1 : 0; plan_out[4] = slabs; plan_out[5] = side ? 1 : 0;
+    sc.timed(iters, ms, [&] {
+      if (side) {
+        launch_groupnorm(dh, C, nullptr, 0, partial, dgw, dgb, dy, B, HW, groups, eps, silu, sc.stream, stats_entries, &sd);
+      } else {
+        launch_groupnorm(dh, C, nullptr, 0, partial, dgw, dgb, dy, B, HW, groups, eps, silu, sc.stream, stats_entries);
+        launch_conv(sd, ws, sc.stream);
+      }
+      launch_conv(c2, ws, sc.stream);
+    });
+    download_nchw(dy, out_gn, B, C, H, W);
+    download_nchw(dout, out, B, C, H, W);
+  });
+}
+
+int sd_op_shortcut_slabs_plan(int B, int H, int W, int C0, int C1, int N, int gn_blocks, int flags, int* plan, unsigned long long* bytes, char* text,
+                              int text_bytes) {
+  return guarded([&] {
+    SD_REQUIRE(plan && bytes && text && text_bytes >= 1 && B >= 1 && H >= 1 && W >= 1 && C0 >= 1 && C1 >= 0 && N >= 1, kInvalidArgument, "bad shortcut_slabs_plan arguments");
+    static const float present[4] = {};
+    const half_t* ph = reinterpret_cast<const half_t*>(present);
+    ConvDesc c2 = conv_desc(ph, N, ph, present, nullptr, nullptr, B, H, W, N, 3);
+    ConvDesc sd = conv_desc(ph, C0, ph, present, nullptr, nullptr, B, H, W, N);
+    if (C1 > 0) sd.x1 = ph, sd.C1 = C1;
+    if (flags & 1) c2.cw.kind = WeightSource::I8Wstream;
+    if (flags & 16) c2.cw.kind = WeightSource::PalWstream;
+    if (flags & 2) sd.cw.kind = WeightSource::I8Gemm;
+    if (flags & 8) c2.temb = present;
+    const ShortcutSlabs ss = shortcut_slabs_plan(c2, sd, gn_blocks, (flags & 4) == 0);
+    plan[0] = ss.splits; plan[1] = ss.conv2_tile; plan[2] = ss.conv2_splits;
+    bytes[0] = ss.slab_bytes; bytes[1] = ss.slab_offset; bytes[2] = ss.workspace_bytes;
+    snprintf(text, (size_t)text_bytes, "%s", ss.refusal ? ss.refusal : "");
+  });
+}
+
+int sd_op_sum_bias(const float* b2, const float* bs, int n, float* dst) {
+  return guarded([&] {
+    SD_REQUIRE(b2 && bs && dst && n >= 0, kInvalidArgument, "bad sum_bias arguments");
+    sum_bias(b2, bs, n, dst);
   });
 }
 
diff --git a/ml-stable-diffusion_amd/csrc/conv_plan.cpp b/ml-stable-diffusion_amd/csrc/conv_plan.cpp
--- a/ml-stable-diffusion_amd/csrc/conv_plan.cpp
+++ b/ml-stable-diffusion_amd/csrc/conv_plan.cpp
@@ -423,7 +423,7 @@
   } else {
     const int steps = p.tile == 7 ? a.Ctot / BK : a.nk_total;
     r.splitk = cdiv(steps, cdiv(steps, p.splitk));
-    r.slab = r.splitk > 1 || twins;
+    r.slab = r.splitk > 1 || twins || d.n_xslabs > 0;
   }
   r.workspace_bytes = slab_bytes(a, r.splitk, r.slab);
   return r;
@@ -551,7 +551,61 @@
   int splits = (switches().tuning && can_split(d)) ? std::max(p.splitk, 16) : p.splitk;
   const bool stream = can_stream(d) || ((pal_stream(d) || i8_stream(d)) && can_split(d) && wstream_shape_ok(d));
   if (stream) splits = std::max(splits, wstream_splits(d, 4));
-  return slab_bytes(a, splits, d.n_twins > 0 || stream);
+  return slab_bytes(a, splits, d.n_twins > 0 || stream || d.n_xslabs > 0);
+}
+
+ShortcutSlabs shortcut_slabs_plan(const ConvDesc& conv2_in, const ConvDesc& sc_in, int gn_blocks, bool fp16_handle) {
+  ShortcutSlabs r{};
+  auto refuse = [&](const char* why) {
+    r = ShortcutSlabs{};
+    r.refusal = why;
+    return r;
+  };
+  if (!fp16_handle) return refuse("an fp32 handle");
+  if ((conv2_in.cw.kind != WeightSource::Fp16 && conv2_in.cw.kind != WeightSource::PalWstream) || sc_in.cw.kind != WeightSource::Fp16)
+    return refuse("a compressed weight source without the combine");
+  if (conv2_in.temb || sc_in.temb) return refuse("a timestep embedding");
+  ConvDesc c2 = conv2_in, sc = sc_in;
+  const int M = c2.B * c2.Ho * c2.Wo;
+  if (M < 128) return refuse("M < 128");
+  {
+    ConvDesc riding = sc;
+    riding.xslabs = nullptr;
+    riding.n_xslabs = 0;
+    if (gn_side_gemm_ok(riding)) return refuse("the shortcut already rides in norm1's launch");
+  }
+  if (sc.B * sc.Ho * sc.Wo != M || sc.N != c2.N || c2.ksize != 3 || c2.x1 || c2.n_twins > 0 || c2.out_mode != kOutHalf || c2.out_t || c2.ln_colsum ||
+      c2.gnf_partial || c2.subpix || c2.debug || !conv_fast_path_ok(c2))
+    return refuse("conv2 is not a plain single-source 3x3 conv of the shortcut's output shape");
+  static const half_t present = 0;
+  c2.res = nullptr;
+  c2.cw = CompressedWeights{};
+  c2.xslabs = nullptr;
+  c2.n_xslabs = 0;
+  c2.w_tiled = (c2.tile == 9 || conv_plan_copies(c2).wstream) ? &present : nullptr;
+  const ConvPlan p = conv_plan(c2);
+  if (!((p.kernel == ConvKernel::HaloKs && p.splitk > 1) || p.kernel == ConvKernel::Wstream)) return refuse("conv2's plan does not end in a slab combine");
+  r.conv2_tile = p.tile;
+  r.conv2_splits = p.splitk;
+  sc.out = nullptr;
+  sc.bias = nullptr;
+  sc.res = nullptr;
+  static float present_f = 0.f;
+  sc.xslabs = &present_f;
+  const int tiles = cdiv(M, 64) * cdiv(sc.N, 64), steps = (sc.C0 + (sc.x1 ? sc.C1 : 0)) / BK;
+  const int room = 2 * 256 - std::max(0, gn_blocks);
+  int s = std::min({std::max(room / std::max(tiles, 1), 1), 8 - r.conv2_splits, steps, 4});
+  for (; s >= 1; --s) {
+    sc.n_xslabs = s;
+    if (gn_side_gemm_ok(sc)) break;
+  }
+  if (s < 1) return refuse(8 - r.conv2_splits < 1 ? "conv2 fills the combine's eight slabs" : "the shortcut is no side GEMM of a GroupNorm launch");
+  r.splits = s;
+  r.slab_bytes = (size_t)s * M * sc.N * sizeof(float);
+  c2.n_xslabs = s;
+  r.slab_offset = conv_workspace_bytes(c2);
+  r.workspace_bytes = r.slab_offset + r.slab_bytes;
+  return r;
 }
 
 ConvWeightCopies conv_plan_copies(const ConvDesc& d0) {
diff --git a/ml-stable-diffusion_amd/csrc/conv_plan.h b/ml-stable-diffusion_amd/csrc/conv_plan.h
--- a/ml-stable-diffusion_amd/csrc/conv_plan.h
+++ b/ml-stable-diffusion_amd/csrc/conv_plan.h
@@ -43,6 +43,14 @@
 
 bool choose_tile_order(double a_bytes, double w_bytes, double nbm, double nbn, bool ab_switch);
 
+struct ShortcutSlabs {
+  int splits;
+  int conv2_tile, conv2_splits;
+  size_t slab_bytes, slab_offset, workspace_bytes;
+  const char* refusal;
+};
+ShortcutSlabs shortcut_slabs_plan(const ConvDesc& conv2, const ConvDesc& sc, int gn_blocks, bool fp16_handle);
+
 bool conv_reduce_stats_on();
 
 constexpr int kConvBK = 64;
diff --git a/ml-stable-diffusion_amd/csrc/igemm.hip b/ml-stable-diffusion_amd/csrc/igemm.hip
--- a/ml-stable-diffusion_amd/csrc/igemm.hip
+++ b/ml-stable-diffusion_amd/csrc/igemm.hip
@@ -724,7 +724,14 @@
   int silu, pix_per_block;
   int gx, gy;
   int n_gn_pad;
+  int side_tiles, side_stride;
 };
+
+template <int D>
+__device__ __forceinline__ void gn_side_gemm(const GnSideArgs& g, const IgemmArgs& a, int w) {
+  const int split = w / g.side_stride, tile = w - split * g.side_stride;
+  if (tile < g.side_tiles) gemm_pipe_body<64, 64, 2, 2, D, false>(a, tile, split);
+}
 
 template <int D>
 __global__ __launch_bounds__(256) void gn_apply_side_kernel(GnSideArgs g, IgemmArgs a) {
@@ -733,7 +740,7 @@
     groupnorm_apply_body(g.x0, g.C0, g.x1, g.C1, g.partial, g.slabs, g.gamma, g.beta, g.y, g.HW, g.G, g.eps, g.silu, g.pix_per_block,
                          v % g.gx, v / g.gx);
   } else if (v >= g.n_gn_pad) {
-    gemm_pipe_body<64, 64, 2, 2, D, false>(a, v - g.n_gn_pad, 0);
+    gn_side_gemm<D>(g, a, v - g.n_gn_pad);
   }
 }
 
@@ -743,14 +750,19 @@
   if (v < g.gx * g.gy) {
     groupnorm_fused_body<VW, 256>(g.x0, g.C0, g.x1, g.C1, g.gamma, g.beta, g.y, g.HW, g.G, g.eps, g.silu, v % g.gx, v / g.gx);
   } else if (v >= g.n_gn_pad) {
-    gemm_pipe_body<64, 64, 2, 2, D, false>(a, v - g.n_gn_pad, 0);
-  }
+    gn_side_gemm<D>(g, a, v - g.n_gn_pad);
+  }
+}
+
+__device__ __forceinline__ const float* combine_slab(const IgemmArgs& a, int z, size_t slab) {
+  return z < a.splitk ? a.partial + (size_t)z * slab : a.xpartial + (size_t)(z - a.splitk) * slab;
 }
 
 __global__ __launch_bounds__(256) void splitk_reduce_kernel(IgemmArgs a) {
   constexpr int SB = 8;
   const size_t total4 = (size_t)a.M * a.N / 4;
   const size_t slab = (size_t)a.M * a.N;
+  const int nslab = a.splitk + a.xsplitk;
   const floatx4 z4 = {0.f, 0.f, 0.f, 0.f};
   for (size_t idx = (size_t)blockIdx.x * blockDim.x + threadIdx.x; idx < total4;
        idx += (size_t)gridDim.x * blockDim.x) {
@@ -759,7 +771,7 @@
     const int n = (int)(e0 - (size_t)m * a.N);
     floatx4 p[SB];
 #pragma unroll
-    for (int z = 0; z < SB; ++z) p[z] = (z < a.splitk) ? *reinterpret_cast<const floatx4*>(a.partial + (size_t)z * slab + e0) : z4;
+    for (int z = 0; z < SB; ++z) p[z] = (z < nslab) ? *reinterpret_cast<const floatx4*>(combine_slab(a, z, slab) + e0) : z4;
     const floatx4 bv = a.bias ? *reinterpret_cast<const floatx4*>(a.bias + n) : z4;
     const floatx4 tv = a.temb ? *reinterpret_cast<const floatx4*>(a.temb + (size_t)(m / a.HoWo) * a.temb_stride + n) : z4;
     const half4 hz = {0, 0, 0, 0};
@@ -767,8 +779,8 @@
     floatx4 s = z4;
 #pragma unroll
     for (int z = 0; z < SB; ++z)
-      if (z < a.splitk) s += p[z];
-    for (int z = SB; z < a.splitk; ++z) s += *reinterpret_cast<const floatx4*>(a.partial + (size_t)z * slab + e0);
+      if (z < nslab) s += p[z];
+    for (int z = SB; z < nslab; ++z) s += *reinterpret_cast<const floatx4*>(combine_slab(a, z, slab) + e0);
     if (a.bias) s += bv;
     if (a.temb) s += tv;
     if (a.res) {
@@ -797,6 +809,7 @@
       const size_t e0 = (size_t)m * a.N + n;
       floatx4 s = {0.f, 0.f, 0.f, 0.f};
       for (int z = 0; z < a.splitk; ++z) s += *reinterpret_cast<const floatx4*>(a.partial + (size_t)z * a.M * a.N + e0);
+      for (int z = 0; z < a.xsplitk; ++z) s += *reinterpret_cast<const floatx4*>(a.xpartial + (size_t)z * a.M * a.N + e0);
       if (a.bias) s += *reinterpret_cast<const floatx4*>(a.bias + n);
       if (a.temb) s += *reinterpret_cast<const floatx4*>(a.temb + (size_t)b * a.temb_stride + n);
       if (a.res) {
@@ -1000,6 +1013,10 @@
   SD_REQUIRE(!d.vt_perm || (d.out_t && (d.Ho * d.Wo) % 16 == 0), kInvalidArgument, "permuted V^T needs the fused q|k|v epilogue and HoWo %% 16 == 0");
   SD_REQUIRE(d.q_cols == 0 || (d.out_t && d.q_cols % 4 == 0 && d.q_cols <= d.n_trans), kInvalidArgument, "pre-scaled queries need the fused q|k|v epilogue (q_cols %d)", d.q_cols);
   const ConvPlan p = conv_plan(d);
+  SD_REQUIRE(d.n_xslabs == 0 || (d.xslabs && d.n_xslabs > 0 && p.slab && d.n_twins == 0 && !d.res && d.out_mode == kOutHalf && !d.out_t && !d.debug &&
+                                 (p.kernel == ConvKernel::Igemm || p.kernel == ConvKernel::GemmPipe || p.kernel == ConvKernel::HaloKs ||
+                                  p.kernel == ConvKernel::Wstream || p.kernel == ConvKernel::WstreamPal)),
+             kInvalidArgument, "extra slabs (%d) on a conv whose plan '%s' has no slab combine for them", d.n_xslabs, conv_plan_kernel_name(p).c_str());
   switch (p.kernel) {
     case ConvKernel::Wsgemm: launch_wsgemm(d, s); return 0;
     case ConvKernel::Bvgemm: launch_bvgemm(d, p, s); return 0;
@@ -1056,6 +1073,8 @@
   if (twins) {
     launch_reduce_twin(a.partial, a.splitk, a.M, a.N, a.HoWo, a.bias, a.temb, a.temb_stride, a.res, a.out, d.n_twins, d.twin, s);
   } else if (a.slab) {
+    a.xpartial = d.xslabs;
+    a.xsplitk = d.n_xslabs;
     gn_entries = launch_slab_combine(d, a, s);
   }
   SD_HIP(hipGetLastError());
@@ -1067,18 +1086,34 @@
         !d.gn_partial && !d.temb && !d.debug && conv_fast_path_ok(d)))
     return false;
   const int M = d.B * d.Ho * d.Wo, c1 = d.x1 ? d.C1 : 0;
-  return gemm_pipe_ok(d.ksize, d.stride, d.up, M, d.N, d.C0 + c1, d.C0, c1) && M >= 256;
+  if (!gemm_pipe_ok(d.ksize, d.stride, d.up, M, d.N, d.C0 + c1, d.C0, c1)) return false;
+  if (d.n_xslabs == 0) return !d.xslabs && M >= 256;
+  const int steps = (d.C0 + c1) / BK;
+  return d.xslabs && !d.res && M >= 128 && d.n_xslabs >= 1 && d.n_xslabs <= 8 && (d.n_xslabs - 1) * cdiv(steps, d.n_xslabs) < steps;
 }
 
 namespace {
 constexpr int kSideD = 4;
 IgemmArgs side_args(const ConvDesc& d) {
-  SD_REQUIRE(gn_side_gemm_ok(d), kInvalidArgument, "side GEMM: not a plain 1x1 GEMM of the pipelined kernel (C0=%d C1=%d N=%d)", d.C0, d.C1, d.N);
+  SD_REQUIRE(gn_side_gemm_ok(d), kInvalidArgument, "side GEMM: not a plain 1x1 GEMM of the pipelined kernel (C0=%d C1=%d N=%d slabs=%d)", d.C0, d.C1, d.N, d.n_xslabs);
   IgemmArgs a = make_args(d);
   a.splitk = 1;
   a.slab = 0;
+  if (d.n_xslabs > 0) {
+    a.splitk = d.n_xslabs;
+    a.slab = 1;
+    a.partial = d.xslabs;
+    a.nk_per_split = cdiv(a.nk_total, a.splitk);
+    a.bias = nullptr;
+    a.out = nullptr;
+  }
   set_tile_order(a, 64, 64);
   return a;
+}
+int side_blocks(const IgemmArgs& a, GnSideArgs& g) {
+  g.side_tiles = cdiv(a.M, 64) * cdiv(a.N, 64);
+  g.side_stride = a.slab ? (g.side_tiles + 7) / 8 * 8 : g.side_tiles;
+  return g.side_stride * a.splitk;
 }
 constexpr size_t kSideLds = (size_t)kSideD * (64 + 64) * BK * sizeof(half_t) + 2 * 64 * sizeof(float);
 }
@@ -1092,7 +1127,8 @@
   auto k = gn_apply_side_kernel<kSideD>;
   static DynLdsOnce once;
   once.set(k, kSideLds);
-  hipLaunchKernelGGL(k, dim3(g.n_gn_pad + cdiv(a.M, 64) * cdiv(a.N, 64)), dim3(256), kSideLds, s, g, a);
+  const dim3 grid(g.n_gn_pad + side_blocks(a, g));
+  hipLaunchKernelGGL(k, grid, dim3(256), kSideLds, s, g, a);
   SD_HIP(hipGetLastError());
 }
 
@@ -1101,7 +1137,7 @@
   IgemmArgs a = side_args(side);
   GnSideArgs g{x0, x1, C0, x1 ? C1 : 0, nullptr, 0, gamma, beta, y, HW, G, eps, silu, 0, G, B, 0};
   g.n_gn_pad = (G * B + 7) / 8 * 8;
-  const dim3 grid(g.n_gn_pad + cdiv(a.M, 64) * cdiv(a.N, 64));
+  const dim3 grid(g.n_gn_pad + side_blocks(a, g));
   static DynLdsOnce o8, o4, o2;
   if (vw == 8) {
     auto k = gn_fused_side_kernel<8, kSideD>;
diff --git a/ml-stable-diffusion_amd/csrc/igemm_device.h b/ml-stable-diffusion_amd/csrc/igemm_device.h
--- a/ml-stable-diffusion_amd/csrc/igemm_device.h
+++ b/ml-stable-diffusion_amd/csrc/igemm_device.h
@@ -57,6 +57,8 @@
   int gnf_G, gnf_entries;
   float q_scale;
   int q_cols;
+  const float* xpartial;
+  int xsplitk;
 };
 
 constexpr int kGnScratchFloats = 256 * 17;
diff --git a/ml-stable-diffusion_amd/csrc/kernels.h b/ml-stable-diffusion_amd/csrc/kernels.h
--- a/ml-stable-diffusion_amd/csrc/kernels.h
+++ b/ml-stable-diffusion_amd/csrc/kernels.h
@@ -81,6 +81,8 @@
   GnTwin twin[2];
   int n_twins = 0;
   bool subpix = false;
+  float* xslabs = nullptr;
+  int n_xslabs = 0;
 };
 
 constexpr int kGnMaxSlabs = 256;
diff --git a/ml-stable-diffusion_amd/csrc/net.cpp b/ml-stable-diffusion_amd/csrc/net.cpp
--- a/ml-stable-diffusion_amd/csrc/net.cpp
+++ b/ml-stable-diffusion_amd/csrc/net.cpp
@@ -146,8 +146,15 @@
   if (f32_) return conv_f32(ops, name, x, a);
   const int cin = x.C + (a.x2 ? a.x2->C : 0);
   const bool geglu = a.out_mode == kOutGeglu;
-  const float* b = a.bias ? upload_vec(name + ".bias", a.cout, geglu) : nullptr;
+  const float* b = a.bias_dev ? a.bias_dev : a.bias ? upload_vec(name + ".bias", a.cout, geglu) : nullptr;
   const WeightPin pin = weight_plan(name, x, a, false);
+  observe_conv(ops, name, x, a);
+  if (pin.kind != WeightSource::Fp16) return conv_w(ops, name, upload_compressed(name, pin, cin, a), b, x, a);
+  if (a.subpix && !a.silu_out && subpixel_wanted(conv_shape(name, x, a))) return conv_w(ops, name, ConvWeights(upload_subpixel_weight(name, a.cout, cin), true), b, x, a);
+  return conv_w(ops, name, upload_conv_weight(name, a.cout, cin, a.k, geglu), b, x, a);
+}
+
+void Net::observe_conv(std::vector<Op>& ops, const std::string& name, const Tensor& x, const ConvArgs& a) {
   const WeightSource could = ws_->observe() && !ws_->palette(name + ".weight") && !a.silu_out
                                  ? conv_plan_weights(conv_shape(name, x, a), StoredWeights::W8A8, ws_->observe_gemms() && a.keep_compressed).kind
                                  : WeightSource::Fp16;
@@ -159,9 +166,6 @@
     ops.push_back([=](hipStream_t s) { launch_absmax_half(p0, n0, p1, n1, slot, s); });
     ops.back().label = "absmax " + name;
   }
-  if (pin.kind != WeightSource::Fp16) return conv_w(ops, name, upload_compressed(name, pin, cin, a), b, x, a);
-  if (a.subpix && !a.silu_out && subpixel_wanted(conv_shape(name, x, a))) return conv_w(ops, name, ConvWeights(upload_subpixel_weight(name, a.cout, cin), true), b, x, a);
-  return conv_w(ops, name, upload_conv_weight(name, a.cout, cin, a.k, geglu), b, x, a);
 }
 
 WeightPin Net::weight_plan(const std::string& name, const Tensor& x, const ConvArgs& a, bool ln) const {
@@ -357,6 +361,7 @@
   d.ldT = a.ldT;
   d.ln_colsum = a.ln_colsum;
   d.x0_i8 = a.x_i8;
+  d.n_xslabs = a.n_xslabs;
   if (ln || a.x_i8) {
     d.vt_perm = a.vt_perm ? 1 : 0;
     d.q_scale = a.q_scale;
@@ -434,12 +439,17 @@
       d.w_bv = wt;
     }
     ll_.ws_need = std::max(ll_.ws_need, conv_workspace_bytes(d));
-    ops.push_back([this, d, hook, with_hook](hipStream_t s) {
-      const int n = launch_conv(with_hook(d), ll_.ws_conv, s);
+    const size_t xoff = a.xslab_offset;
+    SD_REQUIRE(d.n_xslabs == 0 || (xoff >= conv_workspace_bytes(d) && xoff % 16 == 0), kInternal, "%s: extra slabs inside the conv's own workspace", name.c_str());
+    ops.push_back([this, d, hook, with_hook, xoff](hipStream_t s) {
+      ConvDesc dd = with_hook(d);
+      if (dd.n_xslabs > 0) dd.xslabs = ll_.ws_conv.partial + xoff / sizeof(float);
+      const int n = launch_conv(dd, ll_.ws_conv, s);
       if (hook) hook->produced(n);
     });
   } else {
     const int so = a.silu_out ? 1 : 0;
+    SD_REQUIRE(d.n_xslabs == 0, kInternal, "%s: extra slabs off the MFMA path", name.c_str());
     ops.push_back([d, so, hook, with_hook](hipStream_t s) {
       const int n = launch_conv_generic(with_hook(d), so, s);
       if (hook) hook->produced(n);
@@ -498,7 +508,7 @@
 }
 
 Tensor Net::group_norm(std::vector<Op>& ops, const std::string& name, const Tensor& x, const Tensor* x2, float eps,
-                       bool silu, const ConvDesc* side, const std::string& side_label, double side_flop) {
+                       bool silu, const ConvDesc* side, const std::string& side_label, double side_flop, size_t side_slab_offset) {
   SD_REQUIRE(!side || !f32_, kInternal, "%s: side GEMM on the fp32 path", name.c_str());
   const int C = x.C + (x2 ? x2->C : 0);
   const int G = cfg_.norm_num_groups;
@@ -527,7 +537,9 @@
   if (side) {
     const ConvDesc sd = *side;
     ops.push_back([=](hipStream_t s) {
-      launch_groupnorm(p0, C0, p1, C1, partial, gamma, beta, yp, B, HW, G, eps, si, s, hook ? hook->consume() : 0, &sd);
+      ConvDesc sl = sd;
+      if (sl.n_xslabs > 0) sl.xslabs = ll_.ws_conv.partial + side_slab_offset / sizeof(float);
+      launch_groupnorm(p0, C0, p1, C1, partial, gamma, beta, yp, B, HW, G, eps, si, s, hook ? hook->consume() : 0, &sl);
     });
     ops.back().label = label + " || " + side_label;
     ops.back().flop = side_flop;
@@ -557,6 +569,37 @@
     sd.Hi = sd.Ho = x.H;
     sd.Wi = sd.Wo = x.W;
     sd.N = cout;
+    static const int slab_mode = tune_env_int("SD_SHORTCUT_SLABS", 1);
+    if (slab_mode != 0 && !ws_->w8a8(p + ".conv2.weight") && !ws_->w8a8(p + ".conv_shortcut.weight")) {
+      Tensor hs = x;
+      hs.C = cout;
+      hs.gn.reset();
+      const ConvDesc c2 = conv_shape(p + ".conv2", hs, {.cout = cout, .k = 3});
+      const int G = cfg_.norm_num_groups, HW = x.H * x.W;
+      const int gn_blocks = groupnorm_wants_producer_stats(HW, cout, G) ? 512 : x.B * G;
+      const ShortcutSlabs ss = shortcut_slabs_plan(c2, sd, gn_blocks, true);
+      if (ss.splits > 0) {
+        t0 = group_norm(ops, p + ".norm1", x, x2, cfg_.norm_eps, true);
+        Tensor h = conv(ops, p + ".conv1", t0, {.cout = cout, .k = 3, .temb = temb});
+        if (!gn_side_gemm_ok(sd)) observe_conv(ops, p + ".conv_shortcut", x, {.x2 = x2, .cout = cout});
+        sd.w = upload_conv_weight(p + ".conv_shortcut", cout, cin, 1, false);
+        sd.n_xslabs = ss.splits;
+        char buf[256];
+        snprintf(buf, sizeof(buf), "gemm1x1 %d->%d @%dx%d M=%d K=%d slabs=%d %s.conv_shortcut", cin, cout, x.H, x.W, x.M(), cin, ss.splits, p.c_str());
+        Tensor t1 = group_norm(ops, p + ".norm2", h, nullptr, cfg_.norm_eps, true, &sd, buf, 2.0 * x.M() * (double)cout * cin, ss.slab_offset);
+        ll_.ws_need = std::max(ll_.ws_need, ss.workspace_bytes);
+        float* bsum = ll_.arena.alloc_n<float>(cout);
+        const std::string n2 = p + ".conv2.bias", ns = p + ".conv_shortcut.bias";
+        refill({n2, ns}, bsum, [=](const WeightStore& ws) {
+          const HostTensor &b2 = ws.get(n2), &bs = ws.get(ns);
+          SD_REQUIRE((int)b2.numel() == cout && (int)bs.numel() == cout, kInvalidArgument, "%s / %s: expected %d elements each", n2.c_str(), ns.c_str(), cout);
+          std::vector<float> host((size_t)cout);
+          sum_bias(b2.data.data(), bs.data.data(), cout, host.data());
+          SD_HIP(hipMemcpy(bsum, host.data(), (size_t)cout * sizeof(float), hipMemcpyHostToDevice));
+        });
+        return conv(ops, p + ".conv2", t1, {.cout = cout, .k = 3, .n_xslabs = ss.splits, .xslab_offset = ss.slab_offset, .bias_dev = bsum});
+      }
+    }
     if (gn_side_gemm_ok(sd)) {
       sd.w = upload_conv_weight(p + ".conv_shortcut", cout, cin, 1, false);
       sd.bias = upload_vec(p + ".conv_shortcut.bias", cout);
diff --git a/ml-stable-diffusion_amd/csrc/net.h b/ml-stable-diffusion_amd/csrc/net.h
--- a/ml-stable-diffusion_amd/csrc/net.h
+++ b/ml-stable-diffusion_amd/csrc/net.h
@@ -67,6 +67,9 @@
   const int8_t* x_i8 = nullptr;
   int8_t* out_q8 = nullptr;
   float out_inv_s = 0.f;
+  int n_xslabs = 0;
+  size_t xslab_offset = 0;
+  const float* bias_dev = nullptr;
 };
 
 struct ConvWeights {
@@ -126,7 +129,8 @@
   ConvWeights upload_qkv_i8(const std::vector<std::string>& parts, const WeightPin& pin, int cin, int cout_each);
   void conv_small_n(std::vector<Op>& ops, const std::string& name, const Tensor& x, int cout, half_t* out_nhwc, float* out_nchw);
   Tensor group_norm(std::vector<Op>& ops, const std::string& name, const Tensor& x, const Tensor* x2, float eps,
-                    bool silu, const ConvDesc* side = nullptr, const std::string& side_label = std::string(), double side_flop = 0);
+                    bool silu, const ConvDesc* side = nullptr, const std::string& side_label = std::string(), double side_flop = 0,
+                    size_t side_slab_offset = 0);
   Tensor resnet(std::vector<Op>& ops, const std::string& p, const Tensor& x, const Tensor* x2, int cout, const float* temb);
 
   using Fill = std::function<void(const WeightStore&)>;
@@ -150,6 +154,7 @@
 
  private:
   ConvDesc conv_shape(const std::string& name, const Tensor& x, const ConvArgs& a) const;
+  void observe_conv(std::vector<Op>& ops, const std::string& name, const Tensor& x, const ConvArgs& a);
   ConvDesc qkv_shape(const std::string& name, const Tensor& x, const ConvArgs& a) const;
   int pal_tensors_ = 0, pal_streamed_ = 0;
   size_t pal_stream_bytes_ = 0;
diff --git a/ml-stable-diffusion_amd/csrc/weight_prep.h b/ml-stable-diffusion_amd/csrc/weight_prep.h
--- a/ml-stable-diffusion_amd/csrc/weight_prep.h
+++ b/ml-stable-diffusion_amd/csrc/weight_prep.h
@@ -24,6 +24,10 @@
     for (int c = 0; c < cin; ++c)
       for (int t = 0; t < kk; ++t) dst[((size_t)dst_o * kk + t) * cin + c] = (D)src[((size_t)o * cin + c) * kk + t];
   }
+}
+
+inline void sum_bias(const float* b2, const float* bs, int n, float* dst) {
+  for (int i = 0; i < n; ++i) dst[i] = (float)((double)b2[i] + (double)bs[i]);
 }
 
 inline size_t subpixel_fold_halves(int cout, int cin) { return (size_t)16 * cout * cin; }
diff --git a/ml-stable-diffusion_amd/python_hip_stable_diffusion/_lib.py b/ml-stable-diffusion_amd/python_hip_stable_diffusion/_lib.py
--- a/ml-stable-diffusion_amd/python_hip_stable_diffusion/_lib.py
+++ b/ml-stable-diffusion_amd/python_hip_stable_diffusion/_lib.py
@@ -145,6 +145,10 @@
     ("sd_op_layernorm", _I, [_P, _FP, _FP, _P, _I, _I, _I, _F, _I, _FP]),
     ("sd_op_groupnorm", _I, [_P, _FP, _FP, _P, _I, _I, _I, _I, _I, _F, _I, _I, _FP]),
     ("sd_op_groupnorm_shortcut", _I, [_P, _P, _FP, _FP, _P, _FP, _P, _P, _I, _I, _I, _I, _I, _I, _I, _F, _I, _I, _I, _FP]),
+    ("sd_op_resnet_tail", _I, [_P, _P, _P, _FP, _FP, _P, _FP, _P, _FP, _P, _P, _I, _I, _I, _I, _I, _I, _I, _F, _I, _I, _I, _I, _I, C.POINTER(_I),
+                               _I, _FP]),
+    ("sd_op_shortcut_slabs_plan", _I, [_I, _I, _I, _I, _I, _I, _I, _I, C.POINTER(_I), C.POINTER(C.c_ulonglong), C.c_char_p, _I]),
+    ("sd_op_sum_bias", _I, [_FP, _FP, _I, _FP]),
     ("sd_op_conv2d", _I, [_P, _P, _FP, _P, _P, _I, _I, _I, _I, _I, _I, _I, _I, _I, _I, _I, _I, _FP]),
     ("sd_op_conv2d_ex", _I, [_P, _P, _P, _FP, _FP, _P, _P, _I, _I, _I, _I, _I, _I, _I, _I, _I, _I, _I, _FP, _FP, _F, _I, _P, _I, _I, _I,
                              C.POINTER(_I), _I, _FP]),
@@ -874,6 +878,47 @@
     return out_gn, out_sc, ms.value
 
 
+def resnet_tail(h, x0, x1, gn_weight, gn_bias, w2, b2, wsc, bsc, groups=32, eps=1e-5, silu=True, slabs=-1, conv2_tile=0, conv2_splitk=0,
+                stats_entries=0, iters=1):
+    h, x0, w2, wsc = f16(h), f16(x0), f16(w2), f16(wsc)
+    x1 = None if x1 is None else f16(x1)
+    B, Cn, H, W = h.shape
+    C0 = x0.shape[1]
+    C1 = 0 if x1 is None else x1.shape[1]
+    wsc = np.ascontiguousarray(wsc.reshape(Cn, -1))
+    if (w2.shape != (Cn, Cn, 3, 3) or wsc.shape[1] != C0 + C1 or x0.shape != (B, C0, H, W) or (x1 is not None and x1.shape != (B, C1, H, W))):
+        raise ValueError("resnet_tail: inconsistent shapes")
+    gn_weight, gn_bias, b2, bsc = f32(gn_weight), f32(gn_bias), f32(b2), f32(bsc)
+    if any(v.shape != (Cn,) for v in (gn_weight, gn_bias, b2, bsc)):
+        raise ValueError("resnet_tail: gn_weight, gn_bias, b2 and bsc must be (C,)")
+    out_gn = np.empty((B, Cn, H, W), np.float16)
+    out = np.empty((B, Cn, H, W), np.float16)
+    plan = (C.c_int * 6)()
+    ms = C.c_float(0)
+    check(lib().sd_op_resnet_tail(ptr(h), ptr(x0), ptr(x1), fptr(gn_weight), fptr(gn_bias), ptr(w2), fptr(b2), ptr(wsc), fptr(bsc), ptr(out_gn),
+                                  ptr(out), B, Cn, C0, C1, H, W, groups, eps, int(silu), slabs, conv2_tile, conv2_splitk, stats_entries, plan, iters,
+                                  C.byref(ms)))
+    return out_gn, out, {"tile": plan[0], "staging": plan[1], "splitk": plan[2], "slab": bool(plan[3]), "slabs": plan[4], "side": bool(plan[5])}, ms.value
+
+
+def shortcut_slabs_plan(B, H, W, C0, C1, N, gn_blocks=64, flags=0):
+    plan = (C.c_int * 3)()
+    nbytes = (C.c_ulonglong * 3)()
+    text = C.create_string_buffer(128)
+    check(lib().sd_op_shortcut_slabs_plan(B, H, W, C0, C1, N, gn_blocks, flags, plan, nbytes, text, len(text)))
+    return {"splits": plan[0], "conv2_tile": plan[1], "conv2_splits": plan[2], "slab_bytes": int(nbytes[0]), "slab_offset": int(nbytes[1]),
+            "workspace_bytes": int(nbytes[2]), "refusal": text.value.decode()}
+
+
+def sum_bias(b2, bs):
+    b2, bs = f32(b2), f32(bs)
+    if b2.shape != bs.shape or b2.ndim != 1:
+        raise ValueError("sum_bias: two vectors of one length")
+    out = np.empty_like(b2)
+    check(lib().sd_op_sum_bias(fptr(b2), fptr(bs), b2.size, fptr(out)))
+    return out
+
+
 def conv2d_groupnorm(x, w, gn_weight, gn_bias, bias=None, res=None, groups=32, eps=1e-5, silu=False, tile=0,
                      producer_stats=True, iters=1):
     x, w = f16(x), f16(w)
```

Measured after the change: 249.2 it/s (median of 6 runs). No clear change (+0.5%).
